# valida-xyz/valida

Measured on AMD Instinct MI355X. Metric: proofs/sec, 2^20-row Fibonacci trace, higher is better.
Workload: dtype u32; 1 GPU; C2: Fibonacci 2^20 cpu rows (mem 2^22), 14 chips, one proof per GPU; field=BabyBear / Ext5, mmcs=Keccak-256, fri_blowup=2, log_blowup=1, num_queries=40, pow_bits=8, parallelism=single GPU, proofs_in_flight_per_gpu=3, comm_stuck=False

## Files before the change

valida_amd/csrc/field.hpp:

```cpp
#pragma once
#include <cstdint>

#if defined(__HIPCC__)
#include <hip/hip_runtime.h>
#define VG_HD __host__ __device__ __forceinline__
#else
#define VG_HD inline
#endif

namespace vg {

constexpr uint32_t P = 0x78000001u;
constexpr uint32_t P_INV_NEG = 0x77ffffffu;
constexpr uint32_t R_MOD_P = 268435454u;
constexpr uint32_t R2_MOD_P = 1172168163u;
constexpr uint32_t GENERATOR = 31;
constexpr uint32_t TWO_ADIC_ROOT_27 = 0x1a427a41u;

#ifndef VG_MULHI_NOP
#define VG_MULHI_NOP 0
#endif
VG_HD uint32_t mul_lo_pinv(uint32_t lo) {
#if defined(__HIP_DEVICE_COMPILE__) && VG_MULHI_NOP == 2
    uint32_t o;
    asm("v_mul_lo_u32 %0, %1, %2\n\ts_nop 0" : "=v"(o) : "v"(lo), "v"(0x88000001u));
    return o;
#else
    return lo * 0x88000001u;
#endif
}
VG_HD uint32_t mul_hi_u32(uint32_t a, uint32_t b) {
#if defined(__HIP_DEVICE_COMPILE__) && VG_MULHI_NOP
    uint32_t o;
    asm("v_mul_hi_u32 %0, %1, %2\n\ts_nop 0" : "=v"(o) : "v"(a), "v"(b));
    return o;
#elif defined(__HIP_DEVICE_COMPILE__)
    return __umulhi(a, b);
#else
    return (uint32_t)(((uint64_t)a * b) >> 32);
#endif
}

#ifndef VG_CARRY_REDUCE
#define VG_CARRY_REDUCE 1
#endif
#if defined(__HIP_DEVICE_COMPILE__) && VG_CARRY_REDUCE == 2
VG_HD uint32_t reduce_once(uint32_t s) {
    uint32_t t, r;
    asm("v_subrev_co_u32_e32 %0, vcc, %3, %2\n\tv_cndmask_b32_e32 %1, %0, %2, vcc" : "=&v"(t), "=v"(r) : "v"(s), "v"(P) : "vcc");
    return r;
}
VG_HD uint32_t sub_mod(uint32_t a, uint32_t b) {
    uint32_t d, t, r;
    asm("v_sub_co_u32_e32 %0, vcc, %3, %4\n\tv_add_u32_e32 %1, %5, %0\n\tv_cndmask_b32_e32 %2, %0, %1, vcc" : "=&v"(d), "=&v"(t), "=v"(r) : "v"(a), "v"(b), "v"(P) : "vcc");
    return r;
}
#elif defined(__HIP_DEVICE_COMPILE__) && VG_CARRY_REDUCE
VG_HD uint32_t reduce_once(uint32_t s) {
    uint32_t t, r;
    unsigned long long borrow;
    asm("v_subrev_co_u32_e64 %0, %1, %4, %3\n\tv_cndmask_b32_e64 %2, %0, %3, %1" : "=&v"(t), "=&s"(borrow), "=v"(r) : "v"(s), "v"(P));
    return r;
}
VG_HD uint32_t sub_mod(uint32_t a, uint32_t b) {
    uint32_t d, t, r;
    unsigned long long borrow;
    asm("v_sub_co_u32_e64 %0, %1, %4, %5\n\tv_add_u32_e32 %2, %6, %0\n\tv_cndmask_b32_e64 %3, %0, %2, %1" : "=&v"(d), "=&s"(borrow), "=&v"(t), "=v"(r) : "v"(a), "v"(b), "v"(P));
    return r;
}
#else
VG_HD uint32_t reduce_once(uint32_t s) { uint32_t t = s - P; return s < t ? s : t; }
VG_HD uint32_t sub_mod(uint32_t a, uint32_t b) { uint32_t d = a - b, t = d + P; return d < t ? d : t; }
#endif

#ifndef VG_MONTY_ADD
#define VG_MONTY_ADD 0
#endif
VG_HD uint32_t monty_reduce(uint64_t t) {
#if VG_MONTY_ADD == 1
    const uint32_t m = (uint32_t)t * P_INV_NEG;
    return reduce_once((uint32_t)((t + (uint64_t)m * P) >> 32));
#else
    uint32_t lo = (uint32_t)t, hi = (uint32_t)(t >> 32);
    uint32_t m = mul_lo_pinv(lo);
    uint32_t u = mul_hi_u32(m, P);
    return sub_mod(hi, u);
#endif
}

VG_HD uint32_t monty_reduce_wide(uint64_t t) {
    uint32_t lo = (uint32_t)t, hi = reduce_once((uint32_t)(t >> 32));
    uint32_t m = mul_lo_pinv(lo);
    uint32_t u = mul_hi_u32(m, P);
    return sub_mod(hi, u);
}

struct Fp {
    uint32_t v;
    VG_HD static Fp raw(uint32_t m) { Fp r; r.v = m; return r; }
    VG_HD static Fp zero() { return raw(0); }
    VG_HD static Fp one() { return raw(R_MOD_P); }
    VG_HD static Fp from_canonical(uint32_t x) { return raw(monty_reduce((uint64_t)x * R2_MOD_P)); }
    VG_HD uint32_t canonical() const { return monty_reduce((uint64_t)v); }
    VG_HD bool is_zero() const { return v == 0; }
    VG_HD bool operator==(const Fp& o) const { return v == o.v; }
    VG_HD bool operator!=(const Fp& o) const { return v != o.v; }
    VG_HD Fp operator+(const Fp& o) const { return raw(reduce_once(v + o.v)); }
    VG_HD Fp operator-(const Fp& o) const { return raw(sub_mod(v, o.v)); }
    VG_HD Fp operator-() const { return raw(v ? P - v : 0); }
#if VG_MONTY_ADD == 2 && defined(__HIP_DEVICE_COMPILE__)
    VG_HD Fp operator*(const Fp& o) const {
        uint32_t lo, hi;
        asm("v_mul_lo_u32 %0, %2, %3\n\tv_mul_hi_u32 %1, %2, %3" : "=&v"(lo), "=v"(hi) : "v"(v), "v"(o.v));
        return raw(sub_mod(hi, mul_hi_u32(lo * 0x88000001u, P)));
    }
#else
    VG_HD Fp operator*(const Fp& o) const { return raw(monty_reduce((uint64_t)v * o.v)); }
#endif
    VG_HD Fp& operator+=(const Fp& o) { *this = *this + o; return *this; }
    VG_HD Fp& operator-=(const Fp& o) { *this = *this - o; return *this; }
    VG_HD Fp& operator*=(const Fp& o) { *this = *this * o; return *this; }
    VG_HD Fp square() const { return *this * *this; }
    VG_HD Fp pow(uint64_t e) const {
        Fp r = one(), b = *this;
        while (e) { if (e & 1) r *= b; b *= b; e >>= 1; }
        return r;
    }
    VG_HD Fp exp_power_of_2(unsigned k) const { Fp r = *this; for (unsigned i = 0; i < k; i++) r *= r; return r; }
    VG_HD Fp inv() const {
        const Fp x = *this;
        const Fp x3 = x.square() * x, x7 = x3.square() * x;
        const Fp a6 = x7.exp_power_of_2(3) * x7;
        const Fp a12 = a6.exp_power_of_2(6) * a6;
        const Fp a24 = a12.exp_power_of_2(12) * a12;
        const Fp t = a24.exp_power_of_2(3) * x7;
        const Fp w = t * x, w2 = w.square(), w4 = w2.square(), w8 = w4.square();
        return t * (w8 * w4 * w2);
    }
    VG_HD Fp halve() const { return raw((v & 1) ? (uint32_t)(((uint64_t)v + P) >> 1) : v >> 1); }
};

VG_HD Fp two_adic_generator(unsigned bits) {
    return Fp::from_canonical(TWO_ADIC_ROOT_27).exp_power_of_2(27 - bits);
}

struct Ext5 {
    Fp c[5];
    VG_HD static Ext5 zero() { Ext5 r; for (int i = 0; i < 5; i++) r.c[i] = Fp::zero(); return r; }
    VG_HD static Ext5 one() { Ext5 r = zero(); r.c[0] = Fp::one(); return r; }
    VG_HD static Ext5 from_base(Fp b) { Ext5 r = zero(); r.c[0] = b; return r; }
    VG_HD bool is_zero() const { return (c[0].v | c[1].v | c[2].v | c[3].v | c[4].v) == 0; }
    VG_HD bool operator==(const Ext5& o) const { for (int i = 0; i < 5; i++) if (c[i].v != o.c[i].v) return false; return true; }
    VG_HD bool operator!=(const Ext5& o) const { return !(*this == o); }
    VG_HD Ext5 operator+(const Ext5& o) const { Ext5 r; for (int i = 0; i < 5; i++) r.c[i] = c[i] + o.c[i]; return r; }
    VG_HD Ext5 operator-(const Ext5& o) const { Ext5 r; for (int i = 0; i < 5; i++) r.c[i] = c[i] - o.c[i]; return r; }
    VG_HD Ext5 operator-() const { Ext5 r; for (int i = 0; i < 5; i++) r.c[i] = -c[i]; return r; }
    VG_HD Ext5 operator*(const Fp& s) const { Ext5 r; for (int i = 0; i < 5; i++) r.c[i] = c[i] * s; return r; }
    VG_HD Ext5 operator+(const Fp& s) const { Ext5 r = *this; r.c[0] += s; return r; }
    VG_HD Ext5 operator-(const Fp& s) const { Ext5 r = *this; r.c[0] -= s; return r; }
    VG_HD Ext5 operator*(const Ext5& o) const {
        Fp d[5];
#pragma unroll
        for (int j = 0; j < 5; j++) d[j] = o.c[j] + o.c[j];
        Ext5 r;
#pragma unroll
        for (int k = 0; k < 5; k++) {
            uint32_t bb[5];
#pragma unroll
            for (int i = 0; i < 5; i++) bb[i] = i <= k ? o.c[k - i].v : d[k + 5 - i].v;
            uint64_t t0123 = (uint64_t)c[0].v * bb[0] + (uint64_t)c[1].v * bb[1] + (uint64_t)c[2].v * bb[2] + (uint64_t)c[3].v * bb[3];
            uint64_t t4 = (uint64_t)c[4].v * bb[4];
            r.c[k] = Fp::raw(monty_reduce_wide(t0123)) + Fp::raw(monty_reduce(t4));
        }
        return r;
    }
    VG_HD Ext5& operator+=(const Ext5& o) { *this = *this + o; return *this; }
    VG_HD Ext5& operator-=(const Ext5& o) { *this = *this - o; return *this; }
    VG_HD Ext5& operator*=(const Ext5& o) { *this = *this * o; return *this; }
    VG_HD Ext5 square() const { return *this * *this; }
    VG_HD Ext5 pow(uint64_t e) const {
        Ext5 r = one(), b = *this;
        while (e) { if (e & 1) r *= b; b *= b; e >>= 1; }
        return r;
    }
    VG_HD Ext5 exp_power_of_2(unsigned k) const { Ext5 r = *this; for (unsigned i = 0; i < k; i++) r *= r; return r; }
    template <int K> VG_HD Ext5 frobenius_k() const {
        constexpr uint32_t Z[5] = {0, 1079828539u, 847078768u, 1597816133u, 233372948u};
        Ext5 r;
        r.c[0] = c[0];
        r.c[1] = c[1] * Fp::raw(Z[(1 * K) % 5]);
        r.c[2] = c[2] * Fp::raw(Z[(2 * K) % 5]);
        r.c[3] = c[3] * Fp::raw(Z[(3 * K) % 5]);
        r.c[4] = c[4] * Fp::raw(Z[(4 * K) % 5]);
        return r;
    }
    VG_HD Ext5 frobenius() const { return frobenius_k<1>(); }
    VG_HD Ext5 inv() const {
        Ext5 f1 = frobenius_k<1>(), f2 = frobenius_k<2>(), f3 = frobenius_k<3>(), f4 = frobenius_k<4>();
        Ext5 prod = (f1 * f2) * (f3 * f4);
        Fp hi = c[1] * prod.c[4] + c[2] * prod.c[3] + c[3] * prod.c[2] + c[4] * prod.c[1];
        Fp norm = c[0] * prod.c[0] + hi + hi;
        return prod * norm.inv();
    }
};

VG_HD uint32_t reverse_bits_len(uint32_t x, unsigned bits) {
#if defined(__HIP_DEVICE_COMPILE__)
    return bits ? (__brev(x) >> (32 - bits)) : 0;
#else
    uint32_t r = 0;
    for (unsigned i = 0; i < bits; i++) r |= ((x >> i) & 1u) << (bits - 1 - i);
    return r;
#endif
}

inline unsigned log2_strict_u64(uint64_t n) { unsigned k = 0; while ((1ull << k) < n) k++; return k; }

}
```

valida_amd/csrc/host/prover.cpp:

```cpp
#include "prover.hpp"
#include "poseidon_opt.hpp"

namespace vhost {

using Clock = std::chrono::steady_clock;
static double ms_since(Clock::time_point t0) { return std::chrono::duration<double, std::milli>(Clock::now() - t0).count(); }

static Ext5 ext_from_canonical(const uint32_t* w) { Ext5 e; for (int k = 0; k < 5; k++) e.c[k] = Fp::from_canonical(w[k]); return e; }
static void ext_to_canonical(const Ext5& e, uint32_t* w) { for (int k = 0; k < 5; k++) w[k] = e.c[k].canonical(); }

Prover::Prover(int device, const MachineDesc& machine, const uint32_t* poseidon_rc480, const FriParams& fri)
    : ctx_(new DeviceCtx(device)), machine_(machine), fri_(fri), perm16_(poseidon_rc480) {
    for (auto& a : machine_.airs) {
        if (a.log_quotient_degree < 1 || a.log_quotient_degree > 3) throw std::invalid_argument("chip " + a.name + ": log_quotient_degree must be 1..3");
        if (a.native_chip != -2 && (a.native_chip < 0 || a.native_chip >= 14)) throw std::invalid_argument("chip " + a.name + ": native_chip must be a BasicMachine chip id (0..13) or -2 (captured AIR)");
        if (a.log_quotient_degree != 1 && a.native_chip >= 0) throw std::invalid_argument("chip " + a.name + ": the compiled chip kernels assume log_quotient_degree = 1");
        if (fri_.log_blowup < a.log_quotient_degree)
            throw std::invalid_argument("chip " + a.name + ": log_blowup must be >= log_quotient_degree (the quotient domain must lie inside the committed LDE)");
        std::vector<uint32_t> pw(a.program.instrs.size() * 2 + 2, 0);
        if (!a.program.instrs.empty()) memcpy(pw.data(), a.program.instrs.data(), a.program.instrs.size() * 8);
        prog_dev_.emplace_back(ctx_.get(), pw);
        iw_dev_.emplace_back(ctx_.get(), a.interaction_words);
    }
    bool sparse = false;
// ... 467 lines not shown
    ch.observe_digest(perm_pd->tree.root);
    read_cumulative_sums();
    perm_nat.clear();
    main_own.clear();
    tm.commit_perm = ms_since(t0);

    t0 = Clock::now();
    const Ext5 alpha = ch.sample_ext();
    std::vector<DMat> quot(NC);
    std::vector<char> quot_is_natural(NC, 0);
    std::vector<Fp> quot_shifts(NC);
    {
        std::vector<uint32_t> pool;
        std::vector<size_t> off(NC);
        std::vector<uint32_t> Ks(NC);
        uint32_t maxK = 0;
        for (size_t i = 0; i < NC; i++) maxK = std::max<uint32_t>(maxK, machine_.airs[i].program.num_asserts + (uint32_t)machine_.airs[i].interactions.size() + 3);
        std::vector<Ext5> apow_all(maxK);
        { Ext5 p = Ext5::one(); for (auto& e : apow_all) { e = p; p *= alpha; } }
        for (size_t i = 0; i < NC; i++) {
            auto& air = machine_.airs[i];
            uint32_t M = (uint32_t)air.interactions.size(), K = air.program.num_asserts + M + 3;
            Ks[i] = K;
            off[i] = pool.size();
            for (uint32_t k = 0; k < K; k++) put_ext(pool, apow_all[K - 1 - k]);
            for (auto& e : bus_alphas[i]) put_ext(pool, e);
            for (auto& e : betas[i]) put_ext(pool, e);
            put_ext(pool, cumulative_sums[i]);
        }
        DBuf pool_dev(&c, pool);
        Section quotient_section(&c);
        for (size_t i = 0; i < NC; i++) {
            auto& air = machine_.airs[i];
            vk::QuotientArgs a{};
            fill_quotient_args(a, (int)i, main_pd->ldes[i].view(), perm_pd->ldes[i].view(),
                               prep_slot[i] >= 0 ? prep_pd->ldes[prep_slot[i]].view() : vk::DMatView{nullptr, 0, 0, 0}, log_deg[i], pool_dev.data + off[i]);
            a.K = Ks[i];
            quot[i] = DMat(&c, 1ull << log_deg[i], 5ull << air.log_quotient_degree);
            a.out = quot[i].view();
            a.out_natural = air.log_quotient_degree == 1 ? 1 : 0;
            quot_is_natural[i] = a.out_natural != 0;
            vk::launch_quotient(c.stream_for(i, 1ull << log_deg[i]), a, c.tables);
            quot_shifts[i] = s.exp_power_of_2(air.log_quotient_degree);
        }
        quotient_section.join();
        c.check_launch("quotient");
    }
    tm.quotient = ms_since(t0);
    if (dbg && dbg->keep_matrices) {
        dbg->quotient_chunks.resize(NC);
        for (size_t i = 0; i < NC; i++) {
            auto& q = quot[i];
            DMat nat(&c, q.height, q.width);
            if (q.height > 1 && !quot_is_natural[i]) vk::launch_bitrev_rows(c.stream, q.view(), nat.view());
            else VG_HIP_CHECK(hipMemcpyAsync(nat.data, q.data, q.height * q.width * 4, hipMemcpyDeviceToDevice, c.stream));
            DBuf tmp(&c, (size_t)(q.height * q.width));
            vk::launch_export_rows(c.stream, nat.view(), 0, q.height, tmp.data);
            dbg->quotient_chunks[i].resize(q.height * q.width);
            c.download(dbg->quotient_chunks[i].data(), tmp.data, dbg->quotient_chunks[i].size() * 4);
        }
    }
    t0 = Clock::now();
    std::unique_ptr<ProverData> quot_pd;
    {
        std::vector<CommitInput> in;
        for (size_t i = 0; i < quot.size(); i++) in.push_back({&quot[i], !quot_is_natural[i], !quot_is_natural[i]});
        quot_pd = commit_batches(&c, in, &quot_shifts, fri_);
    }
    ch.observe_digest(quot_pd->tree.root);
    quot.clear();
    tm.commit_quotient = ms_since(t0);

    const Ext5 zeta = ch.sample_ext();
    std::vector<OpenRound> rounds(3);
    rounds[0].pd = main_pd.get(); rounds[1].pd = perm_pd.get(); rounds[2].pd = quot_pd.get();
    for (size_t i = 0; i < NC; i++) {
        Fp g = vg::two_adic_generator(log_deg[i]);
        rounds[0].points.push_back({zeta, zeta * g});
        rounds[1].points.push_back({zeta, zeta * g});
        rounds[2].points.push_back({zeta.exp_power_of_2(machine_.airs[i].log_quotient_degree)});
    }
    PcsOpening opening = open_multi_batches(rounds, ch);
    tm.open_values = opening.ms_values; tm.open_reduce = opening.ms_reduce; tm.fri = opening.ms_fri;
    t0 = Clock::now();
    const auto& opened = opening.opened;

    std::vector<uint32_t> pw;
    {
        size_t chip_words = 26;
        for (size_t i = 0; i < NC; i++) chip_words += 11 + 5 * (2 * machine_.airs[i].width + 10 * (machine_.airs[i].interactions.size() + 1) + 10);
        pw.reserve(chip_words + opening.proof_words.size());
    }
    pw.push_back(PROOF_MAGIC);
    pw.push_back((uint32_t)NC);
    for (int k = 0; k < 8; k++) pw.push_back(main_pd->tree.root[k]);
    for (int k = 0; k < 8; k++) pw.push_back(perm_pd->tree.root[k]);
    for (int k = 0; k < 8; k++) pw.push_back(quot_pd->tree.root[k]);
    auto put_vec = [&](const std::vector<Ext5>& v) {
        pw.push_back((uint32_t)v.size());
        for (auto& e : v) { uint32_t w5[5]; ext_to_canonical(e, w5); pw.insert(pw.end(), w5, w5 + 5); }
    };
    for (size_t i = 0; i < NC; i++) {
        pw.push_back(log_deg[i]);
        put_vec(opened[0][i][0]); put_vec(opened[0][i][1]);
        put_vec(opened[1][i][0]); put_vec(opened[1][i][1]);
        put_vec(opened[2][i][0]);
        uint32_t w5[5]; ext_to_canonical(cumulative_sums[i], w5); pw.insert(pw.end(), w5, w5 + 5);
    }
    pw.insert(pw.end(), opening.proof_words.begin(), opening.proof_words.end());
    tm.queries = opening.ms_queries + ms_since(t0);
    c.profiler.collect();
    tm.total = ms_since(t_total);
    if (times) *times = tm;
    if (dbg) {
        if (prep_pd) memcpy(dbg->prep_root, prep_pd->tree.root, 32); else memset(dbg->prep_root, 0, 32);
        for (int i = 0; i < 3; i++) ext_to_canonical(rnd[i], dbg->perm_challenges + 5 * i);
        ext_to_canonical(alpha, dbg->alpha);
        ext_to_canonical(zeta, dbg->zeta);
    }
    return pw;
}

void put_min_poly(std::vector<uint32_t>& w, const Ext5& z) {
    Ext5 g[5] = {Ext5::one(), Ext5::zero(), Ext5::zero(), Ext5::zero(), Ext5::zero()};
    Ext5 conj = z;
    for (int i = 1; i <= 4; i++) {
        conj = conj.frobenius();
        for (int k = i; k >= 1; k--) g[k] = g[k - 1] - conj * g[k];
        g[0] = Ext5::zero() - conj * g[0];
    }
    Ext5 m[5];
    for (int k = 0; k < 5; k++) m[k] = (k ? g[k - 1] : Ext5::zero()) - z * g[k];
    for (int k = 0; k < 5; k++) {
        for (int l = 1; l < 5; l++) if (!m[k].c[l].is_zero()) throw std::logic_error("open: minimal polynomial coefficient outside the base field");
        w.push_back(m[k].c[0].v);
    }
    for (int k = 0; k < 4; k++) put_ext(w, g[k]);
}

PcsOpening Prover::open_multi_batches(const std::vector<OpenRound>& rounds, Challenger& ch) {
    DeviceCtx& c = *ctx_;
    c.activate();
    const Fp s = Fp::from_canonical(vg::GENERATOR);
    const unsigned lb = fri_.log_blowup;
    const size_t NR = rounds.size();
    if (!NR) throw std::invalid_argument("open: no rounds");
    for (auto& r : rounds) {
        if (!r.pd || r.pd->ldes.empty()) throw std::invalid_argument("open: empty round");
        if (r.points.size() != r.pd->ldes.size()) throw std::invalid_argument("open: one point list per committed matrix is required");
    }
    PcsOpening res;
    auto t0 = Clock::now();
    const Ext5 alpha_b = ch.sample_ext();
    struct MatEntry { const DMat* lde; std::vector<std::tuple<uint32_t, Ext5, Ext5>> pts; size_t r, i; };
    struct Group { std::vector<Ext5> zs; std::map<PointKey, uint32_t> slot; std::vector<MatEntry> mats; uint64_t num_reduced = 0; Ext5 offset = Ext5::one(); };
    std::map<unsigned, Group> groups;
    std::vector<Ext5> apow;
    auto prepare_groups = [&]() {
        size_t max_width = 0;
        for (auto& r : rounds) for (auto& l : r.pd->ldes) max_width = std::max<size_t>(max_width, l.width);
        apow.resize(max_width);
        { Ext5 p = Ext5::one(); for (auto& a : apow) { a = p; p *= alpha_b; } }
        for (size_t r = 0; r < NR; r++)
            for (size_t i = 0; i < rounds[r].pd->ldes.size(); i++) {
                const DMat& lde = rounds[r].pd->ldes[i];
                unsigned lh = vg::log2_strict_u64(lde.height);
                Group& g = groups[lh];
                MatEntry me{&lde, {}, r, i};
                for (size_t p = 0; p < rounds[r].points[i].size(); p++) {
                    const Ext5& z = rounds[r].points[i][p];
                    auto key = key_of(z);
                    auto it = g.slot.find(key);
                    uint32_t slot;
                    if (it == g.slot.end()) { slot = (uint32_t)g.zs.size(); g.slot[key] = slot; g.zs.push_back(z); } else slot = it->second;
                    me.pts.emplace_back(slot, g.offset, Ext5::zero());
                    g.num_reduced += lde.width;
                    if (lde.width) g.offset *= apow[lde.width - 1] * alpha_b;
                }
                g.mats.push_back(std::move(me));
            }
    };

    res.opened.resize(NR);
    struct Job { size_t r, i; int p0, np; uint64_t c0, cw; size_t w[2]; size_t scale_off, out_off; };
    std::vector<Job> jobs;
    size_t out_words = 0;
    struct RLaunch { unsigned lh; size_t off; bool accumulate; uint64_t total_width; int n_points; bool vec_ok; };
    std::vector<RLaunch> launches;
    DBuf reduce_pool_dev;
    size_t apw_at = 0, ydesc_at = 0, yoff_at = 0, n_y_slots = 0;
    DBuf out_dev;
    uint32_t* out_host = nullptr;
    {
        std::map<std::pair<unsigned, PointKey>, size_t> wkey;
        std::map<unsigned, Fp> den_inv;
        std::map<PointKey, std::vector<Ext5>> zpow2;
        struct WEntry { unsigned log_n; Ext5 z; size_t pool_off; DBuf buf; };
        std::vector<WEntry> wlist;
        std::vector<uint32_t> pool;
        for (size_t r = 0; r < NR; r++) {
            res.opened[r].resize(rounds[r].pd->ldes.size());
            for (size_t i = 0; i < rounds[r].pd->ldes.size(); i++) {
                const DMat& lde = rounds[r].pd->ldes[i];
                const unsigned ln = vg::log2_strict_u64(lde.height) - lb;
                const uint64_t n = 1ull << ln;
                const auto& pts = rounds[r].points[i];
                res.opened[r][i].assign(pts.size(), std::vector<Ext5>(lde.width));
                for (size_t p0 = 0; p0 < pts.size(); p0 += 2) {
                    const int np = (int)std::min<size_t>(2, pts.size() - p0);
                    size_t widx[2] = {0, 0};
                    const size_t scale_off = pool.size();
                    for (int p = 0; p < np; p++) {
                        const Ext5& z = pts[p0 + p];
                        auto dit = den_inv.find(ln);
                        if (dit == den_inv.end()) dit = den_inv.emplace(ln, (Fp::from_canonical((uint32_t)(n % vg::P)) * s.pow(n - 1)).inv()).first;
                        std::vector<Ext5>& zp = zpow2[key_of(z)];
                        if (zp.empty()) zp.push_back(z);
                        while (zp.size() <= ln) zp.push_back(zp.back().square());
                        Ext5 zer = zp[ln] - s.exp_power_of_2(ln);
                        put_ext(pool, zer * dit->second);
                    }
                    for (int p = 0; p < np; p++) {
                        const Ext5& z = pts[p0 + p];
                        auto key = std::make_pair(ln, key_of(z));
                        auto it = wkey.find(key);
                        if (it == wkey.end()) { wkey[key] = wlist.size(); widx[p] = wlist.size(); wlist.push_back(WEntry{ln, z, 0, DBuf()}); }
                        else widx[p] = it->second;
                    }
                    const uint64_t max_cols = vk::col_dot_max_columns(np);
                    for (uint64_t c0 = 0; c0 < lde.width; c0 += max_cols) {
                        const uint64_t cw = std::min<uint64_t>(max_cols, lde.width - c0);
                        jobs.push_back(Job{r, i, (int)p0, np, c0, cw, {widx[0], widx[np - 1]}, scale_off, out_words});
                        out_words += cw * np * 5;
                    }
                }
            }
        }
        for (auto& w : wlist) { w.pool_off = pool.size(); put_min_poly(pool, w.z); }
        pool.push_back(0);
        DBuf pool_dev(&c, pool);
        {
            std::vector<uint32_t> jobs;
            uint32_t blocks = 0;
            double rows = 0;
            for (auto& w : wlist) {
                const uint64_t n = 1ull << w.log_n;
                w.buf = DBuf(&c, (size_t)vk::bary_buffer_words(n));
                jobs.push_back(blocks); jobs.push_back(0);
                put_u64(jobs, n);
                put_ptr(jobs, pool_dev.data + w.pool_off);
                put_ptr(jobs, w.buf.data);
                put_ptr(jobs, vk::bary_weights_has_image(n) ? w.buf.data + 5 * n : nullptr);
                blocks += vk::bary_weights_blocks(n);
                rows += (double)n;
            }
            if (!wlist.empty()) {
                DBuf jobs_dev(&c, jobs);
                vk::launch_bary_weights_batch(c.stream, jobs_dev.data, (uint32_t)wlist.size(), blocks, rows, s, c.tables);
            }
        }
        prepare_groups();
        {
            struct YSlot { size_t pool_off, r, i, p; };
            std::vector<YSlot> y_slots;
            std::vector<uint32_t> pool;
            for (auto& kv : groups) {
                Group& g = kv.second;
                for (uint32_t s0 = 0; s0 < g.zs.size() || s0 == 0; s0 += vk::MAX_OPEN_POINTS_PER_LAUNCH) {
                    const uint32_t s1 = std::min<uint32_t>((uint32_t)g.zs.size(), s0 + vk::MAX_OPEN_POINTS_PER_LAUNCH);
                    std::vector<const MatEntry*> live;
                    size_t max_w = 0;
                    uint64_t total_width = 0;
                    bool vec_ok = true;
                    for (auto& me : g.mats) {
                        bool any = false;
                        for (auto& t : me.pts) any |= std::get<0>(t) >= s0 && std::get<0>(t) < s1;
                        if (any) { live.push_back(&me); max_w = std::max<size_t>(max_w, me.lde->width); total_width += me.lde->width; vec_ok &= vk::reduce_vec_ok(me.lde->data, me.lde->height); }
                    }
                    launches.push_back({kv.first, pool.size(), s0 != 0, total_width, (int)(s1 - s0), vec_ok});
                    pool.push_back((uint32_t)live.size());
                    pool.push_back(s1 - s0);
                    pool.push_back((uint32_t)max_w);
                    for (uint32_t q = s0; q < s1; q++) put_min_poly(pool, g.zs[q]);
                    for (size_t col = 0; col < max_w; col++) put_ext(pool, apow[col]);
                    for (auto* me : live) {
                        put_ptr(pool, me->lde->data);
                        put_u64(pool, me->lde->height);
                        pool.push_back((uint32_t)me->lde->width);
                        uint32_t cnt = 0;
                        for (auto& t : me->pts) cnt += std::get<0>(t) >= s0 && std::get<0>(t) < s1;
                        pool.push_back(cnt);
                        for (size_t pi = 0; pi < me->pts.size(); pi++) {
                            auto& t = me->pts[pi];
                            if (std::get<0>(t) >= s0 && std::get<0>(t) < s1) {
                                pool.push_back(std::get<0>(t) - s0);
                                put_ext(pool, std::get<1>(t));
                                y_slots.push_back({pool.size(), me->r, me->i, pi});
                                put_ext(pool, Ext5::zero());
                            }
                        }
                    }
                    if (g.zs.size() <= s1) break;
                }
            }
            apw_at = pool.size();
            for (auto& a : apow) put_ext(pool, a);
            std::vector<uint32_t> ydesc, yoff;
            for (auto& ys : y_slots) {
                yoff.push_back((uint32_t)ydesc.size());
                ydesc.push_back((uint32_t)ys.pool_off);
                const size_t n_seg_at = ydesc.size();
                ydesc.push_back(0);
                for (auto& j : jobs)
                    if (j.r == ys.r && j.i == ys.i && (size_t)j.p0 <= ys.p && ys.p < (size_t)(j.p0 + j.np)) {
                        ydesc.push_back((uint32_t)j.out_off); ydesc.push_back((uint32_t)j.np); ydesc.push_back((uint32_t)(ys.p - (size_t)j.p0));
                        ydesc.push_back((uint32_t)j.c0); ydesc.push_back((uint32_t)j.cw);
                        ydesc[n_seg_at]++;
                    }
            }
            ydesc_at = pool.size();
            pool.insert(pool.end(), ydesc.begin(), ydesc.end());
            yoff_at = pool.size();
            pool.insert(pool.end(), yoff.begin(), yoff.end());
            pool.push_back(0);
            n_y_slots = y_slots.size();
            reduce_pool_dev = DBuf(&c, pool);
        }
        out_dev = DBuf(&c, out_words + 4);
        std::vector<DBuf> partials;
        std::vector<uint32_t> fin_jobs;
        uint32_t fin_blocks = 0;
        for (auto& j : jobs) {
            const DMat& lde = rounds[j.r].pd->ldes[j.i];
            const uint64_t n = lde.height >> lb;
            partials.emplace_back(&c, (size_t)(vk::col_dot_slots(n) * j.cw * j.np * 5));
            fin_blocks = vk::col_dot_finish_job(fin_jobs, fin_blocks, n, j.cw, j.np, partials.back().data, pool_dev.data + j.scale_off, out_dev.data + j.out_off);
        }
        DBuf fin_dev;
        if (!fin_jobs.empty()) fin_dev = DBuf(&c, fin_jobs);
        Section open_section(&c);
        size_t job_idx = 0;
        for (auto& j : jobs) {
            const DMat& lde = rounds[j.r].pd->ldes[j.i];
            const uint64_t n = lde.height >> lb;
            vk::DMatView sub{lde.data + j.c0 * lde.height, lde.height, j.cw, lde.height};
            vk::launch_col_dot(c.stream_for(job_idx, n), sub, n, j.np, wlist[j.w[0]].buf.data, wlist[j.w[1]].buf.data, partials[job_idx].data,
                               pool_dev.data + j.scale_off, out_dev.data + j.out_off, false);
            job_idx++;
        }
        open_section.join();
        if (!fin_jobs.empty()) vk::launch_col_dot_finish_batch(c.stream, fin_dev.data, (uint32_t)jobs.size(), fin_blocks);
        c.check_launch("opened values");
        {
            std::lock_guard<std::recursive_mutex> lk(c.host_mu);
            if (open_pinned_words_ < out_words + 4) {
                if (open_pinned_) { VG_HIP_CHECK(hipStreamSynchronize(c.stream)); VG_HIP_CHECK(hipHostFree(open_pinned_)); open_pinned_ = nullptr; open_pinned_words_ = 0; }
                VG_HIP_CHECK(hipHostMalloc((void**)&open_pinned_, (out_words + 4) * 4));
                open_pinned_words_ = out_words + 4;
            }
            out_host = open_pinned_;
        }
    }
    res.ms_values = ms_since(t0);

    t0 = Clock::now();
    std::map<unsigned, DBuf> ro;
    unsigned log_max = 0;
    {
        DBuf& pool_dev = reduce_pool_dev;
        vk::launch_open_y(c.stream, out_dev.data, pool_dev.data + apw_at, pool_dev.data + ydesc_at, pool_dev.data + yoff_at, (uint32_t)n_y_slots, pool_dev.data);
        for (auto& kv : groups) { ro[kv.first] = DBuf(&c, (size_t)(5ull << kv.first)); log_max = std::max(log_max, kv.first); }
        Section reduce_section(&c);
        std::map<unsigned, hipStream_t> stream_of;
        size_t grp_idx = 0;
        for (auto& l : launches) {
            const uint64_t L = 1ull << l.lh;
            if (!stream_of.count(l.lh)) stream_of[l.lh] = c.stream_for(grp_idx++, L);
            vk::launch_reduce_openings(stream_of[l.lh], pool_dev.data + l.off, L, s, c.tables, ro[l.lh].data, l.total_width, l.accumulate, l.n_points, l.vec_ok);
        }
        reduce_section.join();
        c.check_launch("reduce openings");
        if (out_words) VG_HIP_CHECK(hipMemcpyAsync(out_host, out_dev.data, out_words * 4, hipMemcpyDeviceToHost, c.stream));
    }
    res.ms_reduce = ms_since(t0);
    if (log_max < lb + 0u) throw std::invalid_argument("open: nothing to open");

    t0 = Clock::now();
    std::vector<DBuf> layer_bufs;
    std::vector<DeviceTree> layer_trees;
    std::vector<std::array<uint32_t, 8>> commit_phase_commits;
    DBuf cur = std::move(ro[log_max]);
    ro.erase(log_max);
    const unsigned n_layers = log_max - lb;
    std::vector<uint32_t> chw(vk::DEV_CHALLENGER_WORDS, 0);
    for (int i = 0; i < 16; i++) chw[i] = ch.state[i].v;
    for (size_t i = 0; i < ch.in.size(); i++) chw[16 + i] = ch.in[i].v;
    chw[32] = (uint32_t)ch.in.size();
    for (size_t i = 0; i < ch.out.size(); i++) chw[33 + i] = ch.out[i].v;
    chw[49] = (uint32_t)ch.out.size();
    DBuf ch_dev(&c, chw), betas_dev(&c, (size_t)(5 * n_layers + 8)), commits_dev(&c, (size_t)(8 * n_layers + 8));
    unsigned li = 0;
    for (unsigned lf = log_max; lf-- > lb; li++) {
        uint64_t L = 2ull << lf, half = L >> 1;
        layer_trees.emplace_back();
        layer_trees.back().drop_bottom = true;
        const DeviceTree::TopChallenger step{pow_pos_.data, ch_dev.data, betas_dev.data + 5 * li, commits_dev.data + 8 * li};
        layer_trees.back().build(&c, {vk::DMatView{cur.data, half, 10, half}}, false, nullptr, &step);
        DBuf next(&c, (size_t)(5 * half));
        auto it = ro.find(lf);
        vk::launch_fri_fold(c.stream, cur.data, L, betas_dev.data + 5 * li, it != ro.end() ? it->second.data : nullptr, c.tables, next.data);
        if (it != ro.end()) ro.erase(it);
        layer_bufs.push_back(std::move(cur));
        cur = std::move(next);
    }
    c.check_launch("fri fold");
    const size_t NQ = fri_.num_queries, NL = layer_trees.size();
    if (NQ > 256) throw std::invalid_argument("open: at most 256 queries");
    std::vector<uint32_t> templ, bottom_jobs;
    std::vector<std::pair<uint32_t, uint32_t>> fix;
    size_t fix_roots_at = 0, fix_final_at = 0;
    uint32_t tail_pos = 0;
    {
        size_t n_desc = 0, n_fix = 8 * NL + 16;
        for (size_t l = 0; l < NL; l++) n_desc += 1 + layer_trees[l].log_max_height;
        for (size_t r = 0; r < NR; r++) n_desc += rounds[r].pd->ldes.size() + rounds[r].pd->tree.log_max_height;
        n_desc *= NQ;
        n_fix += NQ * (2 + 2 * NL + NR * 2);
        for (size_t r = 0; r < NR; r++) n_fix += NQ * rounds[r].pd->ldes.size();
        templ.reserve(8 * n_desc + 8);
        fix.reserve(n_fix);
        uint32_t& pos = tail_pos;
        auto host_word = [&](uint32_t v) { fix.emplace_back(pos++, v); };
        auto gather = [&](const uint32_t* base, uint64_t stride, uint32_t count, uint32_t kind, size_t q, uint32_t mode, uint32_t shift, uint32_t aux) {
            const uint64_t pv = (uint64_t)base;
            const uint32_t d8[8] = {(uint32_t)pv, (uint32_t)(pv >> 32), (uint32_t)stride, (uint32_t)(stride >> 32), count | (kind << 28), pos, (uint32_t)q | (mode << 8) | (shift << 16), aux};
            templ.insert(templ.end(), d8, d8 + 8);
            pos += count;
        };
        auto gather_path = [&](const DeviceTree& t, size_t q, uint32_t shift0) {
            host_word(t.log_max_height);
            for (unsigned l = 0; l < t.log_max_height; l++) {
                if (l < t.dropped) {
                    const uint64_t pv = (uint64_t)t.leaf_ptr;
                    const uint32_t j8[8] = {(uint32_t)pv, (uint32_t)(pv >> 32), (uint32_t)t.leaf_stride, (uint32_t)(t.leaf_stride >> 32), (uint32_t)t.leaf_elems, pos, (uint32_t)q | (l << 8) | (shift0 << 16), 0};
                    bottom_jobs.insert(bottom_jobs.end(), j8, j8 + 8);
                    pos += 8;
                } else gather(t.layers[l].data, 1, 8, 1, q, 1, shift0 + l, 0);
            }
        };
        host_word((uint32_t)NL);
        fix_roots_at = fix.size();
        for (size_t l = 0; l < NL; l++) for (int w = 0; w < 8; w++) host_word(0);
        host_word((uint32_t)NQ);
        for (size_t q = 0; q < NQ; q++) {
            host_word((uint32_t)NL);
            for (size_t l = 0; l < NL; l++) {
                const uint64_t half = 1ull << (log_max - 1 - l);
                gather(layer_bufs[l].data, half, 5, 0, q, 2, (uint32_t)l, (uint32_t)(5 * half));
                gather_path(layer_trees[l], q, (uint32_t)l + 1);
            }
        }
        fix_final_at = fix.size();
        for (int k = 0; k < 6; k++) host_word(0);
        host_word((uint32_t)NQ);
        for (size_t q = 0; q < NQ; q++) {
            host_word((uint32_t)NR);
            for (size_t r = 0; r < NR; r++) {
                const DeviceTree& t = rounds[r].pd->tree;
                const uint32_t shift_r = log_max - t.log_max_height;
                host_word((uint32_t)rounds[r].pd->ldes.size());
                for (auto& lde : rounds[r].pd->ldes) {
// ... 77 lines not shown
```

valida_amd/csrc/host/sharded_prover.cpp:

```cpp
#include "sharded_prover.hpp"
#include <algorithm>
#include <array>
#include <tuple>

namespace vhost {

namespace {

Ext5 sp_ext_from_canonical(const uint32_t* w) { Ext5 e; for (int k = 0; k < 5; k++) e.c[k] = Fp::from_canonical(w[k]); return e; }
void sp_ext_to_canonical(const Ext5& e, uint32_t* w) { for (int k = 0; k < 5; k++) w[k] = e.c[k].canonical(); }

struct SpPointKey {
    uint32_t w[5];
    bool operator<(const SpPointKey& o) const { return memcmp(w, o.w, 20) < 0; }
};
SpPointKey sp_key_of(const Ext5& e) { SpPointKey k; for (int i = 0; i < 5; i++) k.w[i] = e.c[i].v; return k; }

int owner_of(uint64_t global_col, int W) { return (int)(global_col % (uint64_t)W); }

struct ShTree {
    bool sharded = false;
    DeviceTree tree;
    std::vector<std::vector<uint32_t>> top;
    unsigned log_total = 0, log_local = 0;
// ... 667 lines not shown
        std::vector<uint32_t> out;
        Ext5 alpha_b;
        std::map<unsigned, DBuf> ro;
        std::vector<FriLayer> layers;
        std::vector<std::array<uint32_t, 8>> commits;
        DBuf cur;
        bool cur_sharded = false;
        uint32_t fpw[5];
        uint32_t pow_witness = 0;
        std::vector<uint32_t> tail;
    };
    std::vector<Opening> op((size_t)NH);
    std::vector<std::vector<std::vector<std::vector<Ext5>>>> points((size_t)NH);
    for (int k = 0; k < NH; k++) {
        Rank& R = rk[k];
        const Ext5 zeta = R.ch->sample_ext();
        points[k].resize(NR);
        for (size_t i = 0; i < NC; i++) {
            const Fp g = vg::two_adic_generator(log_deg[i]);
            points[k][0].push_back({zeta, zeta * g});
            points[k][1].push_back({zeta, zeta * g});
            points[k][2].push_back({zeta.exp_power_of_2(1)});
        }
    }
    auto round_of = [&](Rank& R, size_t r) -> ShRound& { return r == 0 ? R.main_rs : r == 1 ? R.perm_rs : R.quot_rs; };

    struct Job { size_t r, i; int p0, np; uint64_t c0, cw; size_t w[2]; size_t scale_off, out_off; bool big; };
    std::vector<Job> jobs0;
    size_t out_words = 0;
    for (int k = 0; k < NH; k++) {
        Rank& R = rk[k];
        DeviceCtx& c = *R.c;
        c.activate();
        Opening& O = op[k];
        O.opened.resize(NR);
        struct WEntry { bool big; unsigned logL; uint64_t rows; Fp shift; Ext5 z; size_t pool_off; DBuf buf; };
        std::map<std::tuple<int, unsigned, SpPointKey>, size_t> wkey;
        std::vector<WEntry> wlist;
        std::vector<uint32_t> pool;
        std::vector<Job> jobs;
        size_t ow = 0;
        for (size_t r = 0; r < NR; r++) {
            ShRound& rs = round_of(R, r);
            O.opened[r].resize(rs.mats.size());
            for (size_t i = 0; i < rs.mats.size(); i++) {
                const ShMat& m = rs.mats[i];
                const unsigned logL = vg::log2_strict_u64(m.L), ln = logL - lb;
                const uint64_t n = 1ull << ln;
                const auto& pts = points[k][r][i];
                O.opened[r][i].assign(pts.size(), std::vector<Ext5>(m.width));
                const Fp rho = m.big ? rho_of(R, logL) : Fp::one();
                for (size_t p0 = 0; p0 < pts.size(); p0 += 2) {
                    const int np = (int)std::min<size_t>(2, pts.size() - p0);
                    size_t widx[2] = {0, 0};
                    const size_t scale_off = pool.size();
                    for (int p = 0; p < np; p++) {
                        const Ext5& z = pts[p0 + p];
                        if (m.big) {
                            Ext5 zer = z.exp_power_of_2(logL) - s.exp_power_of_2(logL);
                            Fp den = Fp::from_canonical((uint32_t)(m.L % vg::P)) * s.pow(m.L - 1);
                            put_ext(pool, zer * (den.inv() * rho));
                        } else {
                            Ext5 zer = z.exp_power_of_2(ln) - s.exp_power_of_2(ln);
                            Fp den = Fp::from_canonical((uint32_t)(n % vg::P)) * s.pow(n - 1);
                            put_ext(pool, zer * den.inv());
                        }
                    }
                    for (int p = 0; p < np; p++) {
                        const Ext5& z = pts[p0 + p];
                        auto key = std::make_tuple(m.big ? 1 : 0, m.big ? logL : ln, sp_key_of(z));
                        auto it = wkey.find(key);
                        if (it == wkey.end()) {
                            wkey[key] = wlist.size(); widx[p] = wlist.size();
                            wlist.push_back(WEntry{m.big, logL, m.big ? m.L / W : n, m.big ? s * rho : s, z, 0, DBuf()});
                        } else widx[p] = it->second;
                    }
                    const uint64_t max_cols = vk::col_dot_max_columns(np);
                    for (uint64_t c0 = 0; c0 < m.width; c0 += max_cols) {
                        const uint64_t cw = std::min<uint64_t>(max_cols, m.width - c0);
                        jobs.push_back(Job{r, i, (int)p0, np, c0, cw, {widx[0], widx[np - 1]}, scale_off, ow, m.big});
                        ow += cw * np * 5;
                    }
                }
            }
        }
        for (auto& w : wlist) { w.pool_off = pool.size(); put_min_poly(pool, w.z); }
        pool.push_back(0);
        DBuf pool_dev(&c, pool);
        {
            std::vector<uint32_t> bj;
            uint32_t blocks = 0;
            double rows = 0;
            auto put64 = [&](uint64_t v) { bj.push_back((uint32_t)v); bj.push_back((uint32_t)(v >> 32)); };
            for (auto& w : wlist) {
                w.buf = DBuf(&c, (size_t)vk::bary_buffer_words(w.rows));
                bj.push_back(blocks); bj.push_back(w.shift.v);
                put64(w.rows);
                put64((uint64_t)(pool_dev.data + w.pool_off));
                put64((uint64_t)w.buf.data);
                put64((uint64_t)(vk::bary_weights_has_image(w.rows) ? w.buf.data + 5 * w.rows : nullptr));
                blocks += vk::bary_weights_blocks(w.rows);
                rows += (double)w.rows;
            }
            if (!wlist.empty()) {
                DBuf jobs_dev(&c, bj);
                vk::launch_bary_weights_batch(c.stream, jobs_dev.data, (uint32_t)wlist.size(), blocks, rows, s, c.tables);
            }
        }
        DBuf out_dev(&c, ow + 4);
        std::vector<DBuf> partials;
        for (auto& j : jobs) {
            const ShMat& m = round_of(R, j.r).mats[j.i];
            const DMat& lde = m.big ? m.shard : m.lde;
            const uint64_t rows = m.big ? lde.height : (lde.height >> lb);
            partials.emplace_back(&c, (size_t)(vk::col_dot_slots(rows) * j.cw * j.np * 5));
            vk::DMatView sub{lde.data + j.c0 * lde.height, lde.height, j.cw, lde.height};
            vk::launch_col_dot(c.stream, sub, rows, j.np, wlist[j.w[0]].buf.data, wlist[j.w[1]].buf.data, partials.back().data, pool_dev.data + j.scale_off, out_dev.data + j.out_off);
        }
        c.check_launch("opened values");
        O.out.assign(ow, 0);
        if (ow) c.download_small(O.out.data(), out_dev.data, ow * 4); else c.sync();
        if (k == 0) { jobs0 = jobs; out_words = ow; }
        else if (ow != out_words) throw std::logic_error("sharded open: ranks disagree on the layout of the opened values");
    }
    {
        std::vector<const uint32_t*> contrib;
        for (auto& O : op) contrib.push_back(O.out.data());
        std::vector<uint32_t> all;
        f.all_gather(contrib, out_words, all);
        for (int k = 0; k < NH; k++) {
            Opening& O = op[k];
            for (auto& j : jobs0)
                for (uint64_t col = 0; col < j.cw; col++)
                    for (int p = 0; p < j.np; p++) {
                        const size_t at = j.out_off + (col * j.np + p) * 5;
                        Ext5 v;
                        if (j.big) {
                            v = Ext5::zero();
                            for (int r = 0; r < W; r++) v += sp_ext_from_canonical(&all[(size_t)r * out_words + at]);
                        } else v = sp_ext_from_canonical(&O.out[at]);
                        O.opened[j.r][j.i][j.p0 + p][j.c0 + col] = v;
                    }
        }
    }

    unsigned log_max = 0;
    for (int k = 0; k < NH; k++) {
        Rank& R = rk[k];
        DeviceCtx& c = *R.c;
        c.activate();
        Opening& O = op[k];
        O.alpha_b = R.ch->sample_ext();
        const Ext5& alpha_b = O.alpha_b;
        struct MatEntry { const uint32_t* data; uint64_t stride; uint64_t width; std::vector<std::tuple<uint32_t, Ext5, Ext5>> pts; };
        struct Group { std::vector<Ext5> zs; std::map<SpPointKey, uint32_t> slot; std::vector<MatEntry> mats; uint64_t num_reduced = 0; Ext5 offset = Ext5::one(); };
        std::map<unsigned, Group> groups;
        size_t max_width = 0;
        for (size_t r = 0; r < NR; r++) for (auto& m : round_of(R, r).mats) max_width = std::max<size_t>(max_width, m.width);
        std::vector<Ext5> apow(max_width);
        { Ext5 pw = Ext5::one(); for (auto& a : apow) { a = pw; pw *= alpha_b; } }
        for (size_t r = 0; r < NR; r++) {
            ShRound& rs = round_of(R, r);
            for (size_t i = 0; i < rs.mats.size(); i++) {
                const ShMat& m = rs.mats[i];
                const unsigned lh = vg::log2_strict_u64(m.L);
                Group& g = groups[lh];
                MatEntry me{m.big ? m.shard.data : m.lde.data, m.big ? m.shard.height : m.lde.height, m.width, {}};
                for (size_t p = 0; p < points[k][r][i].size(); p++) {
                    const Ext5& z = points[k][r][i][p];
                    auto key = sp_key_of(z);
                    auto it = g.slot.find(key);
                    uint32_t slot;
                    if (it == g.slot.end()) { slot = (uint32_t)g.zs.size(); g.slot[key] = slot; g.zs.push_back(z); } else slot = it->second;
                    Ext5 Y = Ext5::zero();
                    auto& ys = O.opened[r][i][p];
                    for (size_t col = 0; col < ys.size(); col++) Y += apow[col] * ys[col];
                    me.pts.emplace_back(slot, g.offset, Y);
                    g.num_reduced += m.width;
                    if (m.width) g.offset *= apow[m.width - 1] * alpha_b;
                }
                g.mats.push_back(std::move(me));
            }
        }
        struct Launch { unsigned lh; size_t off; bool accumulate; uint64_t total_width; int n_points; bool vec_ok; };
        std::vector<Launch> launches;
        std::vector<uint32_t> pool;
        for (auto& kv : groups) {
            Group& g = kv.second;
            for (uint32_t s0 = 0; s0 < g.zs.size() || s0 == 0; s0 += vk::MAX_OPEN_POINTS_PER_LAUNCH) {
                const uint32_t s1 = std::min<uint32_t>((uint32_t)g.zs.size(), s0 + vk::MAX_OPEN_POINTS_PER_LAUNCH);
                std::vector<const MatEntry*> live;
                size_t max_w = 0;
                uint64_t total_width = 0;
                bool vec_ok = true;
                for (auto& me : g.mats) {
                    bool any = false;
                    for (auto& t : me.pts) any |= std::get<0>(t) >= s0 && std::get<0>(t) < s1;
                    if (any) { live.push_back(&me); max_w = std::max<size_t>(max_w, me.width); total_width += me.width; vec_ok &= vk::reduce_vec_ok(me.data, me.stride); }
                }
                launches.push_back({kv.first, pool.size(), s0 != 0, total_width, (int)(s1 - s0), vec_ok});
                pool.push_back((uint32_t)live.size());
                pool.push_back(s1 - s0);
                pool.push_back((uint32_t)max_w);
                for (uint32_t q = s0; q < s1; q++) put_min_poly(pool, g.zs[q]);
                for (size_t col = 0; col < max_w; col++) put_ext(pool, apow[col]);
                for (auto* me : live) {
                    put_ptr(pool, me->data);
                    put_u64(pool, me->stride);
                    pool.push_back((uint32_t)me->width);
                    uint32_t cnt = 0;
                    for (auto& t : me->pts) cnt += std::get<0>(t) >= s0 && std::get<0>(t) < s1;
                    pool.push_back(cnt);
                    for (auto& t : me->pts)
                        if (std::get<0>(t) >= s0 && std::get<0>(t) < s1) { pool.push_back(std::get<0>(t) - s0); put_ext(pool, std::get<1>(t)); put_ext(pool, std::get<2>(t)); }
                }
                if (g.zs.size() <= s1) break;
            }
        }
        DBuf pool_dev(&c, pool);
        for (auto& kv : groups) {
            const uint64_t L = 1ull << kv.first, rows = L >= min_big ? L / W : L;
            O.ro[kv.first] = DBuf(&c, (size_t)(5 * rows));
            log_max = std::max(log_max, kv.first);
        }
        for (auto& l : launches) {
            const uint64_t L = 1ull << l.lh;
            const bool big = L >= min_big;
            vk::launch_reduce_openings(c.stream, pool_dev.data + l.off, big ? L / W : L, big ? s * rho_of(R, l.lh) : s, c.tables, O.ro[l.lh].data, l.total_width, l.accumulate, l.n_points, l.vec_ok);
        }
        c.check_launch("reduce openings");
    }
    if (log_max < lb) throw std::invalid_argument("sharded open: nothing to open");

    const bool multi = W > 1;
    for (auto& O : op) {
        O.cur = std::move(O.ro[log_max]);
        O.ro.erase(log_max);
        O.cur_sharded = multi && (1ull << log_max) >= min_big;
    }
    struct DevFri { bool on = false; unsigned count = 0; size_t first_layer = 0; DBuf ch_dev, betas_dev, commits_dev; };
    std::vector<DevFri> dev((size_t)NH);
    for (unsigned lf = log_max; lf-- > lb;) {
        const uint64_t len = 2ull << lf, half = len >> 1;
        const bool sharded = multi && len >= min_big, next_sharded = multi && half >= min_big;
        if (!sharded) {
            for (int k = 0; k < NH; k++) {
                Rank& R = rk[k];
                DeviceCtx& c = *R.c;
                c.activate();
                Opening& O = op[k];
                DevFri& D = dev[(size_t)k];
                if (O.cur_sharded) throw std::logic_error("sharded fri: layer state out of step");
                if (!D.on) {
                    const unsigned remaining = lf - lb + 1;
                    std::vector<uint32_t> chw(vk::DEV_CHALLENGER_WORDS, 0);
                    const Challenger& ch = *R.ch;
                    for (int i = 0; i < 16; i++) chw[i] = ch.state[i].v;
                    for (size_t i = 0; i < ch.in.size(); i++) chw[16 + i] = ch.in[i].v;
                    chw[32] = (uint32_t)ch.in.size();
                    for (size_t i = 0; i < ch.out.size(); i++) chw[33 + i] = ch.out[i].v;
                    chw[49] = (uint32_t)ch.out.size();
                    D.ch_dev = DBuf(&c, chw);
                    D.betas_dev = DBuf(&c, (size_t)(5 * remaining + 8));
                    D.commits_dev = DBuf(&c, (size_t)(8 * remaining + 8));
                    D.first_layer = O.layers.size();
                    D.on = true;
                }
                O.layers.emplace_back();
                FriLayer& ly = O.layers.back();
                ly.sharded = false; ly.len = len;
                ly.t.sharded = false;
                ly.t.log_total = ly.t.log_local = vg::log2_strict_u64(half);
                const DeviceTree::TopChallenger step{R.p->pow_pos_.data, D.ch_dev.data, D.betas_dev.data + 5 * D.count, D.commits_dev.data + 8 * D.count};
                ly.t.tree.build(&c, {vk::DMatView{O.cur.data, half, 10, half}}, false, nullptr, &step);
                DBuf next(&c, (size_t)(5 * half));
                auto it = O.ro.find(lf);
                vk::launch_fri_fold(c.stream, O.cur.data, len, D.betas_dev.data + 5 * D.count, it != O.ro.end() ? it->second.data : nullptr, c.tables, next.data);
                c.check_launch("fri fold");
                D.count++;
                ly.buf = std::move(O.cur);
                O.cur = std::move(next);
                O.cur_sharded = false;
            }
            continue;
        }
        for (int k = 0; k < NH; k++) {
            Rank& R = rk[k];
            DeviceCtx& c = *R.c;
            c.activate();
            Opening& O = op[k];
            if (O.cur_sharded != sharded) throw std::logic_error("sharded fri: layer state out of step");
            O.layers.emplace_back();
            FriLayer& ly = O.layers.back();
            ly.sharded = sharded; ly.len = len;
            const uint64_t prow = sharded ? half / W : half;
            ly.t.sharded = sharded;
            ly.t.log_total = vg::log2_strict_u64(half);
            ly.t.log_local = vg::log2_strict_u64(prow);
            ly.t.tree.build(&c, {vk::DMatView{O.cur.data, prow, 10, prow}}, true);
            if (!sharded) memcpy(ly.t.root, ly.t.tree.root, 32);
        }
        if (sharded) {
            std::vector<ShTree*> trees;
            for (auto& O : op) trees.push_back(&O.layers.back().t);
            std::vector<uint32_t> roots;
            gather_subtree_roots(trees, roots);
            for (int k = 0; k < NH; k++) finish_top(rk[k], op[k].layers.back().t, roots, nullptr);
        }
        std::vector<std::vector<uint32_t>> next_host((size_t)NH);
        for (int k = 0; k < NH; k++) {
            Rank& R = rk[k];
            DeviceCtx& c = *R.c;
            c.activate();
            Opening& O = op[k];
            FriLayer& ly = O.layers.back();
            R.ch->observe_digest(ly.t.root);
            std::array<uint32_t, 8> root;
            memcpy(root.data(), ly.t.root, 32);
            O.commits.push_back(root);
            Ext5 beta = R.ch->sample_ext();
            if (sharded) beta = beta * rho_of(R, lf + 1).inv();
            std::vector<uint32_t> bw;
            put_ext(bw, beta);
            bw.resize(8, 0);
            DBuf beta_dev(&c, bw);
            const uint64_t my_len = sharded ? len / W : len;
            DBuf next(&c, (size_t)(5 * (my_len / 2)));
            auto it = O.ro.find(lf);
            const uint32_t* add = (it != O.ro.end() && sharded == next_sharded) ? it->second.data : nullptr;
            vk::launch_fri_fold(c.stream, O.cur.data, my_len, beta_dev.data, add, c.tables, next.data);
            c.check_launch("fri fold");
            if (sharded && !next_sharded) {
                next_host[k].resize((size_t)(5 * (my_len / 2)));
                c.download(next_host[k].data(), next.data, next_host[k].size() * 4);
            } else c.sync();
            ly.buf = std::move(O.cur);
            O.cur = std::move(next);
            O.cur_sharded = next_sharded;
        }
        if (sharded && !next_sharded) {
            const uint64_t my_half = half / W, qloc = my_half / 2, q = half / 2;
            std::vector<const uint32_t*> contrib;
            for (auto& v : next_host) contrib.push_back(v.data());
            std::vector<uint32_t> all;
            f.all_gather(contrib, (size_t)(10 * qloc), all);
            for (int k = 0; k < NH; k++) {
                Rank& R = rk[k];
                DeviceCtx& c = *R.c;
                c.activate();
                Opening& O = op[k];
                std::vector<uint32_t> full((size_t)(10 * q));
                for (int r = 0; r < W; r++)
                    for (uint64_t col = 0; col < 10; col++)
                        memcpy(&full[(size_t)(col * q + (uint64_t)r * qloc)], &all[(size_t)r * 10 * qloc + (size_t)(col * qloc)], (size_t)qloc * 4);
                auto it = O.ro.find(lf);
                if (it != O.ro.end()) {
                    std::vector<uint32_t> add((size_t)(10 * q));
                    c.download(add.data(), it->second.data, add.size() * 4);
                    for (size_t x = 0; x < full.size(); x++) full[x] = (Fp::raw(full[x]) + Fp::raw(add[x])).v;
                }
                O.cur = DBuf(&c, full);
            }
        }
    }
    for (int k = 0; k < NH; k++) {
        DevFri& D = dev[(size_t)k];
        if (!D.on) continue;
// ... 179 lines not shown
```

valida_amd/csrc/kernels/launch.hpp:

```cpp
#pragma once
#include <vector>
#include "device_common.hpp"
#include "profiler.hpp"
#include "../air/symbolic.hpp"
#include "verify_args.hpp"

namespace vk {

struct QuotientArgs {
    DMatView main_lde, perm_lde, prep_lde;
    int log_n;
    const vair::Instr* prog;
    uint32_t n_instrs, n_regs, n_air_asserts;
    const uint32_t* iw;
    const uint32_t* consts;
    uint32_t K;
    uint32_t coset_shift, coset_shift_inv;
    int lqd;
    uint32_t zh_inv[8];
    uint32_t zh[8];
    uint32_t g_inv;
    DMatView out;
    int out_natural;
    static constexpr int INTERPRET = -2;
    int native_chip;
    const uint32_t* main_nx;
    const uint32_t* perm_nx;
    const uint32_t* prep_nx;
    uint32_t next_step_p1;
    QuotientArgs normalised() const {
        QuotientArgs b = *this;
        if (!b.main_nx) b.main_nx = b.main_lde.data;
        if (!b.perm_nx) b.perm_nx = b.perm_lde.data;
        if (!b.prep_nx) b.prep_nx = b.prep_lde.data;
        if (!b.next_step_p1) b.next_step_p1 = 1u + (1u << (b.lqd > 0 ? b.lqd : 1));
        return b;
    }
};


void launch_ingest(hipStream_t st, const uint32_t* src_dev, DMatView dst, bool bitrev);
void launch_bitrev_rows(hipStream_t st, DMatView src, DMatView dst);
void launch_clock_probe(hipStream_t st, uint64_t* out3, uint32_t iters);
void launch_interleave_blocks(hipStream_t st, const uint32_t* src, uint32_t* dst, uint64_t rows, uint32_t log_wq, uint64_t n_cols);
void launch_export_rows(hipStream_t st, DMatView src, uint64_t row0, uint64_t nrows, uint32_t* dst_dev);
void launch_intt(hipStream_t st, DMatView m, const DeviceTables& tb);
void launch_coset_ntt(hipStream_t st, DMatView coeffs, DMatView dst, uint64_t dst_row0, Fp shift, const DeviceTables& tb);
void launch_lde_natural(hipStream_t st, DMatView nat, DMatView lde, int log_blowup, const DeviceTables& tb, const LdeTables& lt, DMatView s1, DMatView s2);
void launch_verify_chunk(hipStream_t st, const VerifyChunkArgs& a);
void launch_keccak_leaves(hipStream_t st, const uint32_t* const* cols_dev, int n_elems, uint64_t n_rows, uint32_t* digests);
void launch_keccak_leaves_strided(hipStream_t st, const uint32_t* base, uint64_t stride, int n_elems, uint64_t n_rows, uint32_t* digests);
void launch_keccak_compress(hipStream_t st, const uint32_t* prev, const uint32_t* const* cols_dev, int n_elems, uint64_t n_out, uint32_t* next);
void launch_keccak_bottom_q(hipStream_t st, const uint32_t* jobs_dev, uint32_t n_jobs, const uint32_t* indices_dev, uint32_t* dst);
void launch_poseidon_bottom_q(hipStream_t st, const uint32_t* pos_dev, bool sparse, const uint32_t* jobs_dev, uint32_t n_jobs, const uint32_t* indices_dev, uint32_t* dst);
constexpr int KECCAK_TOP_MAX_LEVELS = 11;
struct KeccakTopArgs {
    const uint32_t* prev;
    uint64_t first_len;
    int levels;
    uint32_t* out[KECCAK_TOP_MAX_LEVELS];
    const uint32_t* const* cols[KECCAK_TOP_MAX_LEVELS];
    int n_elems[KECCAK_TOP_MAX_LEVELS];
    const uint32_t* leaf_base = nullptr;
    uint64_t leaf_stride = 0;
    int leaf_elems = 0;
    uint64_t leaf_rows = 0;
    uint64_t block_len = 0;
    const uint32_t* ch_pos = nullptr;
    uint32_t* ch_state = nullptr;
    uint32_t* ch_beta5 = nullptr;
    uint32_t* ch_commit8 = nullptr;
};
void launch_keccak_top(hipStream_t st, const KeccakTopArgs& a);
constexpr uint64_t KECCAK_LEVELS_BLOCK_LEN = 64;
void launch_keccak_levels(hipStream_t st, const KeccakTopArgs& a);
bool keccak_levels_fused(uint64_t len);
bool keccak_levels_take_leaves(uint64_t n_rows);
bool keccak_top_takes_leaves(uint64_t n_rows);
void launch_poseidon_leaves(hipStream_t st, const uint32_t* pos_dev, bool sparse, const uint32_t* const* cols_dev, int n_elems, uint64_t n_rows, uint32_t* digests);
void launch_poseidon_leaves_strided(hipStream_t st, const uint32_t* pos_dev, bool sparse, const uint32_t* base, uint64_t stride, int n_elems, uint64_t n_rows, uint32_t* digests);
void launch_poseidon_compress(hipStream_t st, const uint32_t* pos_dev, bool sparse, const uint32_t* prev, const uint32_t* const* cols_dev, int n_elems, uint64_t n_out, uint32_t* next);
bool poseidon_levels_take(uint64_t parents);
int poseidon_levels_group(uint64_t parents);
void launch_poseidon_levels(hipStream_t st, const uint32_t* pos_dev, bool sparse, const KeccakTopArgs& a);
void launch_poseidon_top(hipStream_t st, const uint32_t* pos_dev, bool sparse, const KeccakTopArgs& a);
uint64_t perm_scratch_words(uint64_t n);
void launch_add_ext_const(hipStream_t st, uint32_t* data, uint64_t stride, uint64_t n, const uint32_t* off5_dev);
void launch_perm_trace(hipStream_t st, DMatView main, DMatView prep, const uint32_t* iw_dev, const uint32_t* chal_dev, uint32_t M, DMatView perm,
                       uint32_t* scratch, int native_chip = -2);
void launch_quotient(hipStream_t st, const QuotientArgs& a, const DeviceTables& tb);
void launch_check_constraints(hipStream_t st, const QuotientArgs& a, unsigned long long* first_bad_dev);
struct TgCpuOp { uint32_t pc, fp, opcode; int32_t operands[5]; uint32_t kind, has_imm, imm, mem_first; };
struct TgMemOp { uint32_t clk, addr, value, is_write; };
struct TgAluOp { uint32_t opcode, a, b, c; };
struct TgOutOp { uint32_t clk, byte; };
enum { TG_CPU_STORE32 = 0, TG_CPU_LOAD32, TG_CPU_JAL, TG_CPU_JALV, TG_CPU_BEQ, TG_CPU_BNE, TG_CPU_IMM32, TG_CPU_BUS, TG_CPU_BUS_LEFT_IMM, TG_CPU_STOP,
       TG_CPU_LOADFP, TG_CPU_LOAD_U8, TG_CPU_LOAD_S8, TG_CPU_STORE_U8, TG_CPU_READ_ADVICE };
void launch_tracegen_cpu(hipStream_t st, const TgCpuOp* ops, uint64_t n, const TgMemOp* mem, uint64_t n_mem, DMatView t);
size_t tracegen_mem_sort_scratch_bytes(uint64_t n);
hipError_t launch_tracegen_mem(hipStream_t st, const TgMemOp* mem, uint64_t n, const uint32_t* static_cells, uint64_t n_static, uint32_t* keys2, uint32_t* idx2,
                               void* sort_tmp, size_t sort_tmp_bytes, DMatView t);
void launch_tracegen_alu(hipStream_t st, int chip, const TgAluOp* ops, uint64_t n, DMatView t);
void launch_tracegen_idle(hipStream_t st, int mode, const uint32_t* static_cells, uint64_t n_static, DMatView t);
hipError_t launch_tracegen_range(hipStream_t st, const TgCpuOp* ops, uint64_t n, const TgMemOp* mem, uint64_t n_mem, uint32_t* counts, DMatView t);
void launch_tracegen_alu2(hipStream_t st, int chip, const TgAluOp* ops, uint64_t n, DMatView t);
void launch_tracegen_output(hipStream_t st, const TgOutOp* vals, const uint32_t* row0, uint64_t n, uint64_t n_rows, DMatView t);
hipError_t launch_tracegen_program(hipStream_t st, const TgCpuOp* ops, uint64_t n, uint64_t padded_n, uint32_t rom_len, uint32_t* counts, DMatView t);
void launch_bary_weights(hipStream_t st, uint64_t n, const uint32_t* min_poly_dev, Fp shift, const DeviceTables& tb, uint32_t* w);
void launch_bary_weights_batch(hipStream_t st, const uint32_t* jobs_dev, uint32_t n_jobs, uint32_t total_blocks, double total_rows, Fp shift, const DeviceTables& tb);
uint32_t bary_weights_blocks(uint64_t n);
bool bary_weights_has_image(uint64_t n);
uint64_t col_dot_slots(uint64_t n);
uint64_t bary_buffer_words(uint64_t n);
uint64_t col_dot_max_columns(int np);
void launch_col_dot(hipStream_t st, DMatView m, uint64_t n, int np, const uint32_t* w0, const uint32_t* w1, uint32_t* partial,
                    const uint32_t* scale5_dev, uint32_t* out_dev, bool finish = true);
uint32_t col_dot_finish_job(std::vector<uint32_t>& jobs, uint32_t first_block, uint64_t n, uint64_t width, int np, const uint32_t* partial, const uint32_t* scale5_dev, uint32_t* out_dev);
void launch_col_dot_finish_batch(hipStream_t st, const uint32_t* jobs_dev, uint32_t n_jobs, uint32_t total_blocks);
constexpr int MAX_OPEN_POINTS_PER_LAUNCH = 4;
void launch_open_y(hipStream_t st, const uint32_t* vals_dev, const uint32_t* apow_dev, const uint32_t* desc_dev, const uint32_t* entry_off_dev, uint32_t n_entries, uint32_t* pool_dev);
inline bool reduce_vec_ok(const void* col0, uint64_t stride_words) { return ((uintptr_t)col0 & 15) == 0 && (stride_words & 3) == 0; }
void launch_reduce_openings(hipStream_t st, const uint32_t* desc_dev, uint64_t L, Fp shift, const DeviceTables& tb, uint32_t* out, uint64_t total_width,
                            bool accumulate, int n_points, bool vec_ok);
void launch_fri_fold(hipStream_t st, const uint32_t* in, uint64_t L, const uint32_t* beta5_dev, const uint32_t* add, const DeviceTables& tb, uint32_t* out);
constexpr int DEV_CHALLENGER_WORDS = 50;
void launch_fri_challenge(hipStream_t st, const uint32_t* pos_dev, uint32_t* ch_dev, const uint32_t* digest8_dev, uint32_t* beta5_dev, uint32_t* commit8_dev);
void launch_pow_grind(hipStream_t st, const uint32_t* pos_dev, bool sparse, uint32_t k_pending, uint32_t first, uint32_t count, uint32_t bits, uint32_t* best_dev);
void launch_gather(hipStream_t st, const uint32_t* desc_dev, uint64_t n_desc, uint32_t* dst);
void launch_gather_q(hipStream_t st, const uint32_t* templ_dev, uint64_t n_desc, const uint32_t* indices_dev, uint32_t* dst);

}
```

valida_amd/csrc/kernels/merkle.hip:

```cpp
#include "launch.hpp"
#include "keccak.hpp"
#include "keccak_pair.hpp"
#include "challenger_dev.hpp"
#include <cstdlib>
#include <stdexcept>

namespace vk {

__device__ __forceinline__ uint32_t wrap_mod_p(uint32_t w) {
    if (w >= vg::P) w -= vg::P;
    if (w >= vg::P) w -= vg::P;
    return w;
}

__device__ __forceinline__ void squeeze_digest(const KState& a, uint32_t (&out)[8]) {
#pragma unroll
    for (int i = 0; i < 4; i++) { out[2 * i] = wrap_mod_p(a.lo[i]); out[2 * i + 1] = wrap_mod_p(a.hi[i]); }
}

struct PtrCols {
    const uint32_t* const* p;
    __device__ __forceinline__ const uint32_t* operator[](int k) const { return p[k]; }
};
struct StridedCols {
    const uint32_t* base;
    uint64_t stride;
    __device__ __forceinline__ const uint32_t* operator[](int k) const { return base + (uint64_t)k * stride; }
};
template <class Cols>
__device__ __forceinline__ void hash_row(const Cols cols, int n_elems, uint64_t r, uint32_t (&out)[8]) {
    KState a;
    kstate_zero(a);
    int base = 0;
    for (; base + 34 <= n_elems; base += 34) {
#pragma unroll
        for (int k = 0; k < 34; k++) absorb_word(a, k, Fp::raw(cols[base + k][r]).canonical());
        keccak_f1600<false>(a);
    }
    const int rem = n_elems - base;
#pragma unroll
    for (int k = 0; k < 34; k++) {
        if (k < rem) absorb_word(a, k, Fp::raw(cols[base + k][r]).canonical());
        if (k == rem) absorb_word(a, k, 0x01u);
    }
    absorb_word(a, 33, 0x80000000u);
    keccak_f1600<true>(a);
    squeeze_digest(a, out);
}

__device__ __forceinline__ void compress2(const uint32_t (&l)[8], const uint32_t (&r)[8], uint32_t (&out)[8]) {
    KState a;
    kstate_zero(a);
#pragma unroll
    for (int i = 0; i < 4; i++) { a.lo[i] = l[2 * i]; a.hi[i] = l[2 * i + 1]; a.lo[4 + i] = r[2 * i]; a.hi[4 + i] = r[2 * i + 1]; }
    a.lo[8] = 0x01u;
    a.hi[16] = 0x80000000u;
    keccak_f1600<true>(a);
    squeeze_digest(a, out);
}

__device__ __forceinline__ void load_digest(const uint32_t* p, uint32_t (&d)[8]) {
    const uint4* q = reinterpret_cast<const uint4*>(p);
    uint4 lo = q[0], hi = q[1];
    d[0] = lo.x; d[1] = lo.y; d[2] = lo.z; d[3] = lo.w; d[4] = hi.x; d[5] = hi.y; d[6] = hi.z; d[7] = hi.w;
}
__device__ __forceinline__ void store_digest(uint32_t* p, const uint32_t (&d)[8]) {
    uint4* q = reinterpret_cast<uint4*>(p);
    q[0] = make_uint4(d[0], d[1], d[2], d[3]);
    q[1] = make_uint4(d[4], d[5], d[6], d[7]);
}

template <class Cols>
__global__ void __launch_bounds__(256) k_keccak_leaves(const Cols cols, int n_elems, uint64_t n_rows, uint32_t* __restrict__ digests) {
    uint64_t r = (uint64_t)blockIdx.x * blockDim.x + threadIdx.x;
    if (r >= n_rows) return;
    uint32_t d[8];
    hash_row(cols, n_elems, r, d);
    store_digest(digests + 8 * r, d);
}

__global__ void __launch_bounds__(256) k_keccak_compress(const uint32_t* __restrict__ prev, const uint32_t* const* __restrict__ cols, int n_elems, uint64_t n_out,
                                  uint32_t* __restrict__ next) {
    uint64_t i = (uint64_t)blockIdx.x * blockDim.x + threadIdx.x;
    if (i >= n_out) return;
    uint32_t l[8], r[8], d[8];
    load_digest(prev + 16 * i, l);
    load_digest(prev + 16 * i + 8, r);
    compress2(l, r, d);
    if (n_elems > 0) {
        uint32_t h[8], d2[8];
        hash_row(PtrCols{cols}, n_elems, i, h);
        compress2(d, h, d2);
        store_digest(next + 8 * i, d2);
    } else {
        store_digest(next + 8 * i, d);
    }
}

template <class Cols>
__device__ __forceinline__ void hash_row_pair(const Cols cols, int n_elems, uint64_t r, int h, uint32_t (&out)[4]) {
    KHalf a;
#pragma unroll
    for (int i = 0; i < 25; i++) a.s[i] = 0;
    int base = 0;
    for (; base + 34 <= n_elems; base += 34) {
#pragma unroll
        for (int l = 0; l < 17; l++) a.s[l] ^= Fp::raw(cols[base + 2 * l + h][r]).canonical();
        keccak_f1600_pair<false>(a, h);
    }
    const int rem = n_elems - base;
#pragma unroll
    for (int l = 0; l < 17; l++) {
        const int k = 2 * l + h;
        if (k < rem) a.s[l] ^= Fp::raw(cols[base + k][r]).canonical();
        if (k == rem) a.s[l] ^= 0x01u;
    }
    if (h) a.s[16] ^= 0x80000000u;
    keccak_f1600_pair<true>(a, h);
#pragma unroll
    for (int i = 0; i < 4; i++) out[i] = wrap_mod_p(a.s[i]);
}
__device__ __forceinline__ void compress2_pair(const uint32_t (&l)[4], const uint32_t (&r)[4], int h, uint32_t (&out)[4]) {
    KHalf a;
#pragma unroll
    for (int i = 0; i < 25; i++) a.s[i] = 0;
#pragma unroll
    for (int i = 0; i < 4; i++) { a.s[i] = l[i]; a.s[4 + i] = r[i]; }
    if (!h) a.s[8] = 0x01u;
    else a.s[16] = 0x80000000u;
    keccak_f1600_pair<true>(a, h);
#pragma unroll
    for (int i = 0; i < 4; i++) out[i] = wrap_mod_p(a.s[i]);
}
__device__ __forceinline__ void load_digest_half(const uint32_t* p, int h, uint32_t (&d)[4]) {
#pragma unroll
    for (int i = 0; i < 4; i++) d[i] = p[2 * i + h];
}
__device__ __forceinline__ void store_digest_half(uint32_t* p, int h, const uint32_t (&d)[4]) {
#pragma unroll
    for (int i = 0; i < 4; i++) p[2 * i + h] = d[i];
}
__device__ __forceinline__ void node_pair(const uint32_t* prev, const uint32_t* const* cols, int n_elems, uint64_t i, int h, uint32_t* out) {
    uint32_t l[4], r[4], d[4];
    load_digest_half(prev + 16 * i, h, l);
    load_digest_half(prev + 16 * i + 8, h, r);
    compress2_pair(l, r, h, d);
    if (n_elems > 0) {
        uint32_t hr[4], d2[4];
        hash_row_pair(PtrCols{cols}, n_elems, i, h, hr);
        compress2_pair(d, hr, h, d2);
        store_digest_half(out + 8 * i, h, d2);
    } else {
        store_digest_half(out + 8 * i, h, d);
    }
}
template <class Cols>
__global__ void __launch_bounds__(256) k_keccak_leaves_pair(const Cols cols, int n_elems, uint64_t n_rows, uint32_t* __restrict__ digests) {
    const uint64_t t = (uint64_t)blockIdx.x * blockDim.x + threadIdx.x, r = t >> 1;
    if (r >= n_rows) return;
    uint32_t d[4];
    hash_row_pair(cols, n_elems, r, (int)(t & 1), d);
    store_digest_half(digests + 8 * r, (int)(t & 1), d);
}
__global__ void __launch_bounds__(256) k_keccak_compress_pair(const uint32_t* __restrict__ prev, const uint32_t* const* __restrict__ cols, int n_elems, uint64_t n_out,
                                                             uint32_t* __restrict__ next) {
    const uint64_t t = (uint64_t)blockIdx.x * blockDim.x + threadIdx.x, i = t >> 1;
    if (i >= n_out) return;
    node_pair(prev, cols, n_elems, i, (int)(t & 1), next);
}
__global__ void __launch_bounds__(1024) k_keccak_top_pair(KeccakTopArgs a) {
    const uint32_t* prev = a.prev;
    if (a.leaf_rows) {
        if ((threadIdx.x >> 1) < a.leaf_rows) {
            uint32_t d[4];
            hash_row_pair(StridedCols{a.leaf_base, a.leaf_stride}, a.leaf_elems, threadIdx.x >> 1, (int)(threadIdx.x & 1), d);
            store_digest_half(const_cast<uint32_t*>(a.prev) + 8 * (threadIdx.x >> 1), (int)(threadIdx.x & 1), d);
        }
        __threadfence_block();
        __syncthreads();
    }
    for (int l = 0; l < a.levels; l++) {
        const uint64_t len = a.first_len >> l;
        if ((threadIdx.x >> 1) < len) node_pair(prev, a.cols[l], a.n_elems[l], threadIdx.x >> 1, (int)(threadIdx.x & 1), a.out[l]);
        __threadfence_block();
        __syncthreads();
        prev = a.out[l];
    }
    if (a.ch_pos && threadIdx.x < 64) fri_challenge_step((int)threadIdx.x, a.ch_pos, a.ch_state, prev, a.ch_beta5, a.ch_commit8);
}

constexpr int LEVELS_LDS_X = 512, LEVELS_LDS_Y = 256;
__device__ __forceinline__ void lds_barrier() {
#ifdef __HIPCC__
    asm volatile("s_waitcnt lgkmcnt(0)\n\ts_barrier" ::: "memory");
#else
    __syncthreads();
#endif
}
__global__ void __launch_bounds__(1024) k_keccak_levels_pair(KeccakTopArgs a) {
    __shared__ uint32_t lds[(LEVELS_LDS_X + LEVELS_LDS_Y) * 8];
    const int h = (int)(threadIdx.x & 1);
    const uint32_t t = threadIdx.x >> 1;
    const uint64_t b0 = a.block_len, first = (uint64_t)blockIdx.x * b0;
    bool in_lds = false;
    if (a.leaf_rows) {
        if (t < 2 * b0) {
            uint32_t d[4];
            const uint64_t row = 2 * first + t;
            hash_row_pair(StridedCols{a.leaf_base, a.leaf_stride}, a.leaf_elems, row, h, d);
            store_digest_half(const_cast<uint32_t*>(a.prev) + 8 * row, h, d);
            store_digest_half(lds + 8 * t, h, d);
        }
        lds_barrier();
        in_lds = true;
    }
    for (int l = 0; l < a.levels; l++) {
        const uint32_t* in = lds + ((l & 1) ? LEVELS_LDS_X * 8 : 0);
        uint32_t* out = lds + ((l & 1) ? 0 : LEVELS_LDS_X * 8);
        if (t < (b0 >> l)) {
            const uint64_t i = (first >> l) + t;
            uint32_t lf[4], rg[4], d[4];
            if (in_lds) { load_digest_half(in + 16 * t, h, lf); load_digest_half(in + 16 * t + 8, h, rg); }
            else { load_digest_half(a.prev + 16 * i, h, lf); load_digest_half(a.prev + 16 * i + 8, h, rg); }
            compress2_pair(lf, rg, h, d);
            if (a.n_elems[l] > 0) {
                uint32_t hr[4], d2[4];
                hash_row_pair(PtrCols{a.cols[l]}, a.n_elems[l], i, h, hr);
                compress2_pair(d, hr, h, d2);
#pragma unroll
                for (int k = 0; k < 4; k++) d[k] = d2[k];
            }
            store_digest_half(a.out[l] + 8 * i, h, d);
            store_digest_half(out + 8 * t, h, d);
        }
        in_lds = true;
        if (l + 1 < a.levels) lds_barrier();
    }
    if (a.ch_pos) {
        __threadfence_block();
        __syncthreads();
        if (threadIdx.x < 64) fri_challenge_step((int)threadIdx.x, a.ch_pos, a.ch_state, a.out[a.levels - 1], a.ch_beta5, a.ch_commit8);
    }
}

__global__ void __launch_bounds__(1024) k_keccak_top(KeccakTopArgs a) {
    const uint32_t* prev = a.prev;
    for (int l = 0; l < a.levels; l++) {
        const uint64_t len = a.first_len >> l;
        if (threadIdx.x < len) {
            const uint64_t i = threadIdx.x;
            uint32_t lft[8], rgt[8], d[8];
            load_digest(prev + 16 * i, lft);
            load_digest(prev + 16 * i + 8, rgt);
            compress2(lft, rgt, d);
            if (a.n_elems[l] > 0) {
                uint32_t h[8], d2[8];
                hash_row(PtrCols{a.cols[l]}, a.n_elems[l], i, h);
                compress2(d, h, d2);
                store_digest(a.out[l] + 8 * i, d2);
            } else {
                store_digest(a.out[l] + 8 * i, d);
            }
        }
        __threadfence_block();
        __syncthreads();
        prev = a.out[l];
    }
    if (a.ch_pos && threadIdx.x < 64) fri_challenge_step((int)threadIdx.x, a.ch_pos, a.ch_state, prev, a.ch_beta5, a.ch_commit8);
}

constexpr double KECCAK_VALU_PER_PERM = 23 * 178.0 + 58.0;
constexpr uint64_t KECCAK_PAIR_MAX_NODES = 32768;
static bool keccak_pairs_enabled() {
    static const bool on = [] { const char* e = getenv("VGPU_KECCAK_PAIRS"); return !(e && e[0] == '0'); }();
    return on;
}
static double row_perms(int n_elems) { return (double)(n_elems / 34 + 1); }
static double node_perms(int n_inject) { return n_inject > 0 ? 2.0 + row_perms(n_inject) : 1.0; }

bool keccak_top_takes_leaves(uint64_t n_rows) { return keccak_pairs_enabled() && n_rows >= 2 && n_rows <= 512; }
static bool keccak_levels_enabled() {
    static const bool on = [] { const char* e = getenv("VGPU_KECCAK_LEVELS"); return !(e && e[0] == '0'); }();
    return on && keccak_pairs_enabled();
}
bool keccak_levels_fused(uint64_t len) { return keccak_levels_enabled() && len >= KECCAK_LEVELS_BLOCK_LEN && len <= KECCAK_PAIR_MAX_NODES; }
bool keccak_levels_take_leaves(uint64_t n_rows) { return n_rows >= 2 * KECCAK_LEVELS_BLOCK_LEN && keccak_levels_fused(n_rows / 2); }

void launch_keccak_levels(hipStream_t st, const KeccakTopArgs& a0) {
    KeccakTopArgs a = a0;
    if (!a.block_len) a.block_len = a.first_len;
    const uint64_t b0 = a.block_len;
    if (!keccak_levels_enabled() || !b0 || (b0 & (b0 - 1)) || b0 > (uint64_t)LEVELS_LDS_Y || a.first_len % b0 || a.levels < 1 || a.levels > KECCAK_TOP_MAX_LEVELS ||
        (b0 >> (a.levels - 1)) == 0 || (a.leaf_rows && a.leaf_rows != 2 * a.first_len) || (a.ch_pos && a.first_len != b0))
        throw std::logic_error("keccak levels: a launch this kernel does not fit");
    double bytes = 0, perms = 0;
    for (int l = 0; l < a.levels; l++) {
        bytes += (double)(a.first_len >> l) * (96.0 + 4.0 * a.n_elems[l]);
        perms += (double)(a.first_len >> l) * node_perms(a.n_elems[l]);
    }
    if (a.leaf_rows) {
        bytes += (double)a.leaf_rows * (4.0 * a.leaf_elems + 32.0);
        perms += (double)a.leaf_rows * row_perms(a.leaf_elems);
    }
    unsigned threads = (unsigned)((a.leaf_rows ? 4 : 2) * b0);
    if (threads < 64) threads = 64;
    ProfScope ps("k_keccak_levels_pair", st, bytes, perms * KECCAK_VALU_PER_PERM / 64.0);
    VK_LAUNCH(k_keccak_levels_pair, dim3((unsigned)(a.first_len / b0)), dim3(threads), 0, st, a);
}

void launch_keccak_top(hipStream_t st, const KeccakTopArgs& a) {
    double bytes = 0, perms = 0;
    for (int l = 0; l < a.levels; l++) {
        bytes += (double)(a.first_len >> l) * (96.0 + 4.0 * a.n_elems[l]);
        perms += (double)(a.first_len >> l) * node_perms(a.n_elems[l]);
    }
    const bool pairs = keccak_pairs_enabled() && a.first_len <= 512;
    if (a.leaf_rows) {
        if (!pairs || a.leaf_rows != 2 * a.first_len || !keccak_top_takes_leaves(a.leaf_rows)) throw std::logic_error("keccak top: leaf prologue on a tree it does not fit");
        bytes += (double)a.leaf_rows * (4.0 * a.leaf_elems + 32.0);
        perms += (double)a.leaf_rows * row_perms(a.leaf_elems);
    }
    if (pairs && keccak_levels_enabled() && a.first_len <= (uint64_t)LEVELS_LDS_Y) { launch_keccak_levels(st, a); return; }
    ProfScope ps(pairs ? "k_keccak_top_pair" : "k_keccak_top", st, bytes, perms * KECCAK_VALU_PER_PERM / 64.0);
    if (pairs) { VK_LAUNCH(k_keccak_top_pair, dim3(1), dim3(1024), 0, st, a); return; }
    VK_LAUNCH(k_keccak_top, dim3(1), dim3(1024), 0, st, a);
}

template <class Cols> __device__ __forceinline__ void bottom_digest_quad(const Cols cols, int n_elems, uint64_t node, uint32_t level, int pair, int h, uint32_t (&d)[4]) {
    uint32_t own[4];
    hash_row_pair(cols, n_elems, level ? 2 * node + (uint64_t)pair : node, h, own);
    if (level == 0) {
#pragma unroll
        for (int i = 0; i < 4; i++) d[i] = own[i];
        return;
    }
    uint32_t right[4];
#pragma unroll
    for (int i = 0; i < 4; i++) right[i] = (uint32_t)__builtin_amdgcn_update_dpp(0, (int)own[i], 0xEE, 0xF, 0xF, true);
    compress2_pair(own, right, h, d);
}
__global__ void __launch_bounds__(256) k_keccak_bottom_q(const uint32_t* __restrict__ jobs, uint32_t n_jobs, const uint32_t* __restrict__ indices, uint32_t* __restrict__ dst) {
    const uint32_t t = blockIdx.x * blockDim.x + threadIdx.x, j = t >> 2;
    if (j >= n_jobs) return;
    const int pair = (int)((t >> 1) & 1u), h = (int)(t & 1u);
    const uint32_t* e = jobs + 8 * j;
    const uint64_t ptr = ((uint64_t)e[1] << 32) | e[0], stride = ((uint64_t)e[3] << 32) | e[2];
    const uint32_t q = e[6] & 0xffu, level = (e[6] >> 8) & 0xffu, shift = e[6] >> 16;
    const uint64_t node = (((uint64_t)indices[q] >> shift) >> level) ^ 1u;
    uint32_t d[4];
    if (stride) bottom_digest_quad(StridedCols{reinterpret_cast<const uint32_t*>(ptr), stride}, (int)e[4], node, level, pair, h, d);
    else bottom_digest_quad(PtrCols{reinterpret_cast<const uint32_t* const*>(ptr)}, (int)e[4], node, level, pair, h, d);
    if (pair == 0) store_digest_half(dst + e[5], h, d);
}
void launch_keccak_bottom_q(hipStream_t st, const uint32_t* jobs_dev, uint32_t n_jobs, const uint32_t* indices_dev, uint32_t* dst) {
    if (!n_jobs) return;
    ProfScope ps("k_gather", st, 0.0);
    VK_LAUNCH(k_keccak_bottom_q, dim3((4 * n_jobs + 255) / 256), dim3(256), 0, st, jobs_dev, n_jobs, indices_dev, dst);
}

void launch_keccak_leaves(hipStream_t st, const uint32_t* const* cols_dev, int n_elems, uint64_t n_rows, uint32_t* digests) {
    unsigned blocks = (unsigned)((n_rows + 255) / 256);
    const bool pairs = keccak_pairs_enabled() && n_rows <= KECCAK_PAIR_MAX_NODES;
    ProfScope ps(pairs ? "k_keccak_leaves_pair" : "k_keccak_leaves", st, (double)n_rows * (4.0 * n_elems + 32.0), (double)n_rows * row_perms(n_elems) * KECCAK_VALU_PER_PERM / 64.0);
    if (pairs) {
        VK_LAUNCH(k_keccak_leaves_pair<PtrCols>, dim3((unsigned)((2 * n_rows + 255) / 256)), dim3(256), 0, st, PtrCols{cols_dev}, n_elems, n_rows, digests);
        return;
    }
    VK_LAUNCH(k_keccak_leaves<PtrCols>, dim3(blocks), dim3(256), 0, st, PtrCols{cols_dev}, n_elems, n_rows, digests);
}
void launch_keccak_leaves_strided(hipStream_t st, const uint32_t* base, uint64_t stride, int n_elems, uint64_t n_rows, uint32_t* digests) {
    unsigned blocks = (unsigned)((n_rows + 255) / 256);
    const bool pairs = keccak_pairs_enabled() && n_rows <= KECCAK_PAIR_MAX_NODES;
    ProfScope ps(pairs ? "k_keccak_leaves_pair" : "k_keccak_leaves", st, (double)n_rows * (4.0 * n_elems + 32.0), (double)n_rows * row_perms(n_elems) * KECCAK_VALU_PER_PERM / 64.0);
    if (pairs) {
        VK_LAUNCH(k_keccak_leaves_pair<StridedCols>, dim3((unsigned)((2 * n_rows + 255) / 256)), dim3(256), 0, st, StridedCols{base, stride}, n_elems, n_rows, digests);
        return;
    }
    VK_LAUNCH(k_keccak_leaves<StridedCols>, dim3(blocks), dim3(256), 0, st, StridedCols{base, stride}, n_elems, n_rows, digests);
}
void launch_keccak_compress(hipStream_t st, const uint32_t* prev, const uint32_t* const* cols_dev, int n_elems, uint64_t n_out, uint32_t* next) {
    unsigned blocks = (unsigned)((n_out + 255) / 256);
    const bool pairs = keccak_pairs_enabled() && n_out <= KECCAK_PAIR_MAX_NODES;
    ProfScope ps(pairs ? "k_keccak_compress_pair" : "k_keccak_compress", st, (double)n_out * (96.0 + 4.0 * n_elems), (double)n_out * node_perms(n_elems) * KECCAK_VALU_PER_PERM / 64.0);
    if (pairs) {
        VK_LAUNCH(k_keccak_compress_pair, dim3((unsigned)((2 * n_out + 255) / 256)), dim3(256), 0, st, prev, cols_dev, n_elems, n_out, next);
        return;
    }
    VK_LAUNCH(k_keccak_compress, dim3(blocks), dim3(256), 0, st, prev, cols_dev, n_elems, n_out, next);
}

}
```

valida_amd/csrc/kernels/ntt.hip:

```cpp
#include "launch.hpp"
#include "butterfly.hpp"

namespace vk {

template <bool PAD> __device__ __forceinline__ int tile_addr(int i, int c, int LD) { return PAD ? i + (i >> 4) : i * LD + c; }

template <int R>
__device__ __forceinline__ void load_round_twiddles(Fp (&held)[(1 << R) - 1], const uint32_t* tw, int low, int lowbits) {
#pragma unroll
    for (int st = 0; st < R; st++) {
        const uint32_t* t = tw + ((1 << (lowbits + st)) - 1) + low;
#pragma unroll
        for (int k = 0; k < (1 << st); k++) held[(1 << st) - 1 + k] = Fp::raw(t[k << lowbits]);
    }
}

template <int R, bool DIT, bool PAD, int LB>
__device__ __forceinline__ void ntt_round(uint32_t* buf, const uint32_t* tw, int logn, int s_lo, int logT, int LD) {
    constexpr int G = 1 << R;
    const int n_items = (1 << (logn - R)) << logT;
    const int maskT = (1 << logT) - 1, lowbits = LB >= 0 ? LB : s_lo - 1, lowmask = (1 << lowbits) - 1;
    const bool linear = !PAD || lowbits >= 4 || lowbits + R <= 4;
    const int gs = PAD ? (lowbits >= 4 ? (1 << lowbits) + (1 << (lowbits - 4)) : (1 << lowbits)) : (LD << lowbits);
    for (int w = threadIdx.x; w < n_items; w += blockDim.x) {
        const int c = w & maskT, q = w >> logT;
        const int low = q & lowmask, base = ((q >> lowbits) << (lowbits + R)) | low;
        uint32_t* p0 = buf + tile_addr<PAD>(base, c, LD);
        Fp x[G];
        if (linear) {
#pragma unroll
            for (int g = 0; g < G; g++) x[g] = Fp::raw(p0[g * gs]);
        } else {
#pragma unroll
            for (int g = 0; g < G; g++) x[g] = Fp::raw(buf[tile_addr<PAD>(base | (g << lowbits), c, LD)]);
        }
        butterflies<R, DIT, LB == 0>(x, tw, low, lowbits);
        if (linear) {
#pragma unroll
            for (int g = 0; g < G; g++) p0[g * gs] = x[g].v;
        } else {
#pragma unroll
            for (int g = 0; g < G; g++) buf[tile_addr<PAD>(base | (g << lowbits), c, LD)] = x[g].v;
        }
    }
    __syncthreads();
}

template <bool DIT, bool PAD>
__device__ __forceinline__ void ntt_round_dispatch(int R, uint32_t* buf, const uint32_t* tw, int logn, int s_lo, int logT, int LD) {
    if (s_lo == 1) {
        switch (R) {
            case 1: ntt_round<1, DIT, PAD, 0>(buf, tw, logn, 1, logT, LD); break;
            case 2: ntt_round<2, DIT, PAD, 0>(buf, tw, logn, 1, logT, LD); break;
            case 3: ntt_round<3, DIT, PAD, 0>(buf, tw, logn, 1, logT, LD); break;
            default: ntt_round<4, DIT, PAD, 0>(buf, tw, logn, 1, logT, LD); break;
        }
        return;
    }
    switch (R) {
        case 1: ntt_round<1, DIT, PAD, -1>(buf, tw, logn, s_lo, logT, LD); break;
        case 2: ntt_round<2, DIT, PAD, -1>(buf, tw, logn, s_lo, logT, LD); break;
        case 3: ntt_round<3, DIT, PAD, -1>(buf, tw, logn, s_lo, logT, LD); break;
        default: ntt_round<4, DIT, PAD, -1>(buf, tw, logn, s_lo, logT, LD); break;
    }
}

template <bool DIT, bool PAD>
__device__ __forceinline__ void tile_transform(uint32_t* buf, const uint32_t* tw, int logn, int logT, int LD) {
    if (logn == 0) return;
    if (PAD && logn == 12) {
        if (DIT) {
            ntt_round<4, true, PAD, 0>(buf, tw, 12, 1, 0, LD);
            ntt_round<4, true, PAD, 4>(buf, tw, 12, 5, 0, LD);
            ntt_round<4, true, PAD, 8>(buf, tw, 12, 9, 0, LD);
        } else {
            ntt_round<4, false, PAD, 8>(buf, tw, 12, 9, 0, LD);
            ntt_round<4, false, PAD, 4>(buf, tw, 12, 5, 0, LD);
            ntt_round<4, false, PAD, 0>(buf, tw, 12, 1, 0, LD);
        }
        return;
    }
    if (PAD && logn == 14) {
        if (DIT) {
            ntt_round<4, true, PAD, 0>(buf, tw, 14, 1, 0, LD);
            ntt_round<4, true, PAD, 4>(buf, tw, 14, 5, 0, LD);
            ntt_round<4, true, PAD, 8>(buf, tw, 14, 9, 0, LD);
            ntt_round<2, true, PAD, 12>(buf, tw, 14, 13, 0, LD);
        } else {
            ntt_round<2, false, PAD, 12>(buf, tw, 14, 13, 0, LD);
            ntt_round<4, false, PAD, 8>(buf, tw, 14, 9, 0, LD);
            ntt_round<4, false, PAD, 4>(buf, tw, 14, 5, 0, LD);
            ntt_round<4, false, PAD, 0>(buf, tw, 14, 1, 0, LD);
        }
        return;
    }
    const int rounds = (logn + 3) >> 2, small = logn / rounds, extra = logn - small * rounds;
    if (DIT) {
        int s_lo = 1;
        for (int i = 0; i < rounds; i++) { int R = small + (i < extra ? 1 : 0); ntt_round_dispatch<true, PAD>(R, buf, tw, logn, s_lo, logT, LD); s_lo += R; }
    } else {
        int s_top = logn;
        for (int i = 0; i < rounds; i++) { int R = small + (i < extra ? 1 : 0); ntt_round_dispatch<false, PAD>(R, buf, tw, logn, s_top - R + 1, logT, LD); s_top -= R; }
    }
}

template <int R, bool DIT, int LB, int LOGT>
__device__ __forceinline__ void ntt_round_strided(uint32_t* buf, const uint32_t* tw, int logn) {
    constexpr int G = 1 << R, T = 1 << LOGT, LD = T + 1, gs = LD << LB;
    const int n_items = (1 << (logn - R)) << LOGT;
    for (int w = threadIdx.x; w < n_items; w += blockDim.x) {
        const int c = w & (T - 1), q = w >> LOGT;
        const int low = q & ((1 << LB) - 1), base = ((q >> LB) << (LB + R)) | low;
        uint32_t* p0 = buf + base * LD + c;
        Fp x[G];
#pragma unroll
        for (int g = 0; g < G; g++) x[g] = Fp::raw(p0[g * gs]);
        butterflies<R, DIT, LB == 0>(x, tw, low, LB);
#pragma unroll
        for (int g = 0; g < G; g++) p0[g * gs] = x[g].v;
    }
    __syncthreads();
}
template <bool DIT, int K_HI, int LOGT>
__device__ __forceinline__ void strided_transform(uint32_t* buf, const uint32_t* tw) {
    static_assert(K_HI == 8 || K_HI == 10, "hot shapes only");
    if (DIT) {
        ntt_round_strided<4, true, 0, LOGT>(buf, tw, K_HI);
        ntt_round_strided<4, true, 4, LOGT>(buf, tw, K_HI);
        if (K_HI == 10) ntt_round_strided<2, true, 8, LOGT>(buf, tw, K_HI);
    } else {
        if (K_HI == 10) ntt_round_strided<2, false, 8, LOGT>(buf, tw, K_HI);
        ntt_round_strided<4, false, 4, LOGT>(buf, tw, K_HI);
        ntt_round_strided<4, false, 0, LOGT>(buf, tw, K_HI);
    }
}
#ifndef VGPU_STRIDED_FIXED
#define VGPU_STRIDED_FIXED 1
#endif
template <bool DIT>
__device__ __forceinline__ void strided_tile_transform(uint32_t* buf, const uint32_t* tw, int k_hi, int logT, int LD) {
    if (VGPU_STRIDED_FIXED && k_hi == 8 && logT == 6) strided_transform<DIT, 8, 6>(buf, tw);
    else if (VGPU_STRIDED_FIXED && k_hi == 10 && logT == 4) strided_transform<DIT, 10, 4>(buf, tw);
    else tile_transform<DIT, false>(buf, tw, k_hi, logT, LD);
}

__device__ __forceinline__ void stage_twiddles(uint32_t* dst, const uint32_t* __restrict__ compact, int logn) {
    const int count = (1 << logn) - 1;
    for (int i = threadIdx.x; i < count; i += blockDim.x) dst[i] = compact[i];
}

__device__ __forceinline__ Fp root_pow(const DeviceTables& tb, int m, uint32_t x) { return domain_point(tb, m ? __brev(x) >> (32 - m) : 0u); }
__device__ __forceinline__ Fp inv_root_pow(const DeviceTables& tb, int m, uint32_t x) { return inv_domain_point(tb, m ? __brev(x) >> (32 - m) : 0u); }

__host__ __device__ inline int padded_words(int n) { return n + (n >> 4); }

constexpr int CONTIG_MAX_PER_THREAD = 16;
__device__ __forceinline__ void prefetch_tile(uint32_t (&pre)[CONTIG_MAX_PER_THREAD], const uint32_t* __restrict__ src, int n_lo) {
#pragma unroll
    for (int u = 0; u < CONTIG_MAX_PER_THREAD; u++) {
        const int i = threadIdx.x + u * blockDim.x;
        if (i < n_lo) pre[u] = src[i];
    }
}
__device__ __forceinline__ void commit_tile(const uint32_t (&pre)[CONTIG_MAX_PER_THREAD], uint32_t* lds, int n_lo) {
#pragma unroll
    for (int u = 0; u < CONTIG_MAX_PER_THREAD; u++) {
        const int i = threadIdx.x + u * blockDim.x;
        if (i < n_lo) lds[tile_addr<true>(i, 0, 0)] = pre[u];
    }
}

__global__ void k_intt_contig(DMatView m, int k, int k_lo, DeviceTables tb, uint32_t n_inv_mont) {
    extern __shared__ uint32_t lds[];
    const int n_lo = 1 << k_lo, k_hi = k - k_lo;
    const uint32_t* tw = tb.itwc;
    const uint64_t tiles_per_col = m.height >> k_lo, total = tiles_per_col * m.width;
    auto tile_ptr = [&](uint64_t t) { const uint64_t cidx = t >> k_hi; return m.col(cidx) + (t & (tiles_per_col - 1)) * n_lo; };
    uint32_t pre[CONTIG_MAX_PER_THREAD];
    if (blockIdx.x < total) prefetch_tile(pre, tile_ptr(blockIdx.x), n_lo);
    for (uint64_t t = blockIdx.x; t < total; t += gridDim.x) {
        const uint64_t h = t & (tiles_per_col - 1);
        uint32_t* col = tile_ptr(t);
        commit_tile(pre, lds, n_lo);
        __syncthreads();
        if (t + gridDim.x < total) prefetch_tile(pre, tile_ptr(t + gridDim.x), n_lo);
        tile_transform<true, true>(lds, tw, k_lo, 0, 0);
        if (k_hi > 0) {
            const uint32_t e = __brev((uint32_t)h) >> (32 - k_hi), nmask = (1u << k) - 1u;
            Fp step = inv_root_pow(tb, k, (e * blockDim.x) & nmask), cur = inv_root_pow(tb, k, (e * threadIdx.x) & nmask);
            for (int i = threadIdx.x; i < n_lo; i += blockDim.x) { col[i] = (Fp::raw(lds[tile_addr<true>(i, 0, 0)]) * cur).v; cur *= step; }
        } else {
            Fp ninv = Fp::raw(n_inv_mont);
            for (int i = threadIdx.x; i < n_lo; i += blockDim.x) col[i] = (Fp::raw(lds[tile_addr<true>(i, 0, 0)]) * ninv).v;
        }
        __syncthreads();
    }
}

__device__ __forceinline__ unsigned strided_tile_of_block(unsigned x, unsigned n_tiles) {
    if (n_tiles & 15u) return x;
    return (x & ~15u) | ((x & 7u) << 1) | ((x >> 3) & 1u);
}

__global__ void k_intt_strided(DMatView m, int k, int k_lo, int logT, DeviceTables tb, uint32_t n_inv_mont) {
    extern __shared__ uint32_t lds[];
    const int k_hi = k - k_lo, n_hi = 1 << k_hi, T = 1 << logT, LD = T + 1;
    const uint64_t n_lo = 1ull << k_lo;
    uint32_t* tw = lds + n_hi * LD;
    uint32_t* col = m.col(blockIdx.y) + (uint64_t)strided_tile_of_block(blockIdx.x, gridDim.x) * T;
    const int total = n_hi << logT;
    {
        int e = threadIdx.x;
        for (; e + 7 * (int)blockDim.x < total; e += 8 * blockDim.x) {
            uint32_t v[8];
#pragma unroll
            for (int u = 0; u < 8; u++) { const int eu = e + u * (int)blockDim.x; v[u] = col[(uint64_t)(eu >> logT) * n_lo + (eu & (T - 1))]; }
#pragma unroll
            for (int u = 0; u < 8; u++) { const int eu = e + u * (int)blockDim.x; lds[(eu >> logT) * LD + (eu & (T - 1))] = v[u]; }
        }
        for (; e < total; e += blockDim.x) { int c = e & (T - 1), h = e >> logT; lds[h * LD + c] = col[h * n_lo + c]; }
    }
    stage_twiddles(tw, tb.itwc, k_hi);
    __syncthreads();
    strided_tile_transform<true>(lds, tw, k_hi, logT, LD);
    Fp ninv = Fp::raw(n_inv_mont);
    for (int e = threadIdx.x; e < total; e += blockDim.x) { int c = e & (T - 1), h = e >> logT; col[h * n_lo + c] = (Fp::raw(lds[h * LD + c]) * ninv).v; }
}

struct CosetPowers { uint32_t lo[64], hi[256], hp[128], step; };

__global__ void k_ntt_strided(DMatView src, DMatView dst, uint64_t dst_row0, int k, int k_lo, int logT, DeviceTables tb, CosetPowers cp) {
    extern __shared__ uint32_t lds[];
    const int k_hi = k - k_lo, n_hi = 1 << k_hi, T = 1 << logT, LD = T + 1;
    const uint64_t n_lo = 1ull << k_lo, r0 = (uint64_t)strided_tile_of_block(blockIdx.x, gridDim.x) * T;
    uint32_t* tw = lds + n_hi * LD;
    const uint32_t* in = src.col(blockIdx.y) + r0;
    uint32_t* out = dst.col(blockIdx.y) + dst_row0 + r0;
    const int total = n_hi << logT;
    {
        int c = threadIdx.x & (T - 1), h0 = threadIdx.x >> logT, hstep = blockDim.x >> logT;
        const uint32_t r = (uint32_t)r0 + c;
        Fp cur = Fp::raw(cp.lo[r & 63]) * Fp::raw(cp.hi[r >> 6]) * Fp::raw(cp.hp[h0]), step = Fp::raw(cp.step);
        int h = h0;
        for (; h + 7 * hstep < n_hi; h += 8 * hstep) {
            uint32_t v[8];
#pragma unroll
            for (int u = 0; u < 8; u++) v[u] = in[(uint64_t)(h + u * hstep) * n_lo + c];
#pragma unroll
            for (int u = 0; u < 8; u++) { lds[(h + u * hstep) * LD + c] = (Fp::raw(v[u]) * cur).v; cur *= step; }
        }
        for (; h < n_hi; h += hstep) { lds[h * LD + c] = (Fp::raw(in[h * n_lo + c]) * cur).v; cur *= step; }
    }
    stage_twiddles(tw, tb.twc, k_hi);
    __syncthreads();
    strided_tile_transform<false>(lds, tw, k_hi, logT, LD);
    for (int h = threadIdx.x; h < n_hi; h += blockDim.x) {
        const uint32_t e = __brev((uint32_t)h) >> (32 - k_hi);
        Fp base = root_pow(tb, k, e);
        Fp cur = root_pow(tb, k, (uint32_t)(((uint64_t)e * r0) & ((1ull << k) - 1)));
        for (int c = 0; c < T; c++) { lds[h * LD + c] = (Fp::raw(lds[h * LD + c]) * cur).v; cur *= base; }
    }
    __syncthreads();
    for (int e = threadIdx.x; e < total; e += blockDim.x) { int c = e & (T - 1), h = e >> logT; out[h * n_lo + c] = lds[h * LD + c]; }
}

__global__ void k_ntt_contig(DMatView src, DMatView dst, uint64_t dst_row0, int k, int k_lo, DeviceTables tb, uint32_t shift_mont,
                             int from_src
                             ) {
    extern __shared__ uint32_t lds[];
    const int n_lo = 1 << k_lo;
    const uint32_t* tw = tb.twc;
    const uint64_t tiles_per_col = src.height >> k_lo, total = tiles_per_col * src.width;
    auto tile_ptr = [&](uint64_t t) { const uint64_t cidx = t >> (k - k_lo); return dst.col(cidx) + dst_row0 + (t & (tiles_per_col - 1)) * n_lo; };
    Fp cur0 = Fp::one(), step = Fp::one();
    if (from_src) { Fp shift = Fp::raw(shift_mont); cur0 = shift.pow(threadIdx.x); step = shift.pow(blockDim.x); }
    uint32_t pre[CONTIG_MAX_PER_THREAD];
    if (!from_src && blockIdx.x < total) prefetch_tile(pre, tile_ptr(blockIdx.x), n_lo);
    for (uint64_t t = blockIdx.x; t < total; t += gridDim.x) {
        uint32_t* out = tile_ptr(t);
        if (from_src) {
            const uint32_t* in = src.col(t);
            Fp cur = cur0;
            for (int i = threadIdx.x; i < n_lo; i += blockDim.x) { lds[tile_addr<true>(i, 0, 0)] = (Fp::raw(in[i]) * cur).v; cur *= step; }
        } else {
            commit_tile(pre, lds, n_lo);
        }
        __syncthreads();
        if (!from_src && t + gridDim.x < total) prefetch_tile(pre, tile_ptr(t + gridDim.x), n_lo);
        tile_transform<false, true>(lds, tw, k_lo, 0, 0);
        for (int i = threadIdx.x; i < n_lo; i += blockDim.x) out[i] = lds[tile_addr<true>(i, 0, 0)];
        __syncthreads();
    }
}


#ifndef VGPU_STRIDED_IO
#define VGPU_STRIDED_IO 1
#endif
#if defined(__HIP_DEVICE_COMPILE__)
#define VGPU_OPAQUE_S(x) asm volatile("" : "+s"(x))
#else
#define VGPU_OPAQUE_S(x) ((void)0)
#endif
__host__ __device__ constexpr uint32_t brev_c(uint32_t x, int bits) { uint32_t r = 0; for (int i = 0; i < bits; i++) r |= ((x >> i) & 1u) << (bits - 1 - i); return r; }
template <int K_HI, int LOGT> struct StridedShape {
    static constexpr int NT = 512, T = 1 << LOGT, LD = T + 1, NH = 1 << K_HI, LH = 9 - LOGT , HSTEP = 1 << LH, U = NH >> LH;
    static_assert(U == 32 && (K_HI - LH) == 5, "512 threads x 32 elements");
};
template <int K_HI, int LOGT, bool SRC_BITREV>
__device__ __forceinline__ void strided_tile_load(const uint32_t* col0, uint32_t n_lo, uint32_t* lds) {
    using S = StridedShape<K_HI, LOGT>;
    const uint32_t tid = threadIdx.x, c = tid & (S::T - 1), h0 = tid >> LOGT;
    const uint32_t blk0 = SRC_BITREV ? (__brev(h0) >> (32 - S::LH)) << 5 : h0;
    const uint32_t voff = (blk0 * n_lo + c) * 4u;
    uint32_t* l0 = lds + h0 * S::LD + c;
    const uint32_t step = (uint32_t)S::HSTEP * n_lo * 4u;
    uint32_t run = 0;
#pragma unroll
    for (int u0 = 0; u0 < S::U; u0 += 8) {
        uint32_t v[8];
#pragma unroll
        for (int k = 0; k < 8; k++) {
            const uint32_t u = (uint32_t)(u0 + k);
            if (SRC_BITREV) v[k] = load_at(col0, voff, brev_c(u, 5) * n_lo * 4u);
            else { v[k] = load_at(col0, voff, run); run += step; VGPU_OPAQUE_S(run); }
        }
#pragma unroll
        for (int k = 0; k < 8; k++) l0[(u0 + k) * S::HSTEP * S::LD] = v[k];
    }
}
template <int K_HI, int LOGT>
__device__ __forceinline__ void strided_tile_store(uint32_t* col0, uint32_t n_lo, const uint32_t* lds) {
    using S = StridedShape<K_HI, LOGT>;
    const uint32_t tid = threadIdx.x, c = tid & (S::T - 1), h0 = tid >> LOGT;
    const uint32_t voff = (h0 * n_lo + c) * 4u;
    const uint32_t* l0 = lds + h0 * S::LD + c;
    const uint32_t step = (uint32_t)S::HSTEP * n_lo * 4u;
    uint32_t run = 0;
#pragma unroll
    for (int u = 0; u < S::U; u++) { store_at(col0, voff, run, l0[u * S::HSTEP * S::LD]); run += step; VGPU_OPAQUE_S(run); }
}
template <int K_HI, int LOGT>
__device__ __forceinline__ void strided_tile_store_transposed(uint32_t* out_col, uint32_t tile, int k_lo, const uint32_t* lds) {
    using S = StridedShape<K_HI, LOGT>;
    const uint32_t tid = threadIdx.x, kq = (uint32_t)(k_lo - LOGT);
    const uint32_t qb_tile = kq ? __brev(tile) >> (32 - kq) : 0u;
    if (K_HI == 8) {
        const uint32_t p2 = tid & 255u, c0 = tid >> 8;
        uint32_t* base = out_col + ((uint64_t)qb_tile << K_HI);
        const uint32_t voff = ((((c0 << 5) << kq) << K_HI) + p2) * 4u;
        const uint32_t* l0 = lds + p2 * S::LD + c0;
#pragma unroll
        for (int i = 0; i < 32; i++) store_at(base, voff, ((brev_c((uint32_t)i, 5) << kq) << K_HI) * 4u, l0[2 * i]);
    } else {
        uint32_t* base = out_col + ((uint64_t)qb_tile << K_HI);
        const uint32_t* l0 = lds + tid * S::LD;
#pragma unroll
        for (int i = 0; i < 32; i++) {
            const uint32_t c = (uint32_t)(i >> 1), half = (uint32_t)(i & 1);
            store_at(base, (tid + 512u * half) * 4u, ((brev_c(c, LOGT) << kq) << K_HI) * 4u, l0[512 * half * S::LD + c]);
        }
    }
}

template <int FK_HI, int FLOGT>
__global__ void __launch_bounds__(FK_HI ? 512 : 1024) k_lde_a(DMatView src, DMatView dst, int k, int k_lo, int logT_arg, DeviceTables tb) {
    extern __shared__ uint32_t lds[];
    const int k_hi = FK_HI ? FK_HI : k - k_lo, logT = FK_HI ? FLOGT : logT_arg, n_hi = 1 << k_hi, T = 1 << logT, LD = T + 1;
    const uint64_t n_lo = 1ull << k_lo, r0 = (uint64_t)strided_tile_of_block(blockIdx.x, gridDim.x) * T;
    uint32_t* tw = lds + n_hi * LD;
    const uint32_t* in = src.col(blockIdx.y) + r0;
    uint32_t* out = dst.col(blockIdx.y) + r0;
    const int total = n_hi << logT;
    if constexpr (FK_HI != 0) strided_tile_load<FK_HI, FLOGT, false>(in, (uint32_t)n_lo, lds);
    else {
        int e = threadIdx.x;
        for (; e + 7 * (int)blockDim.x < total; e += 8 * blockDim.x) {
            uint32_t v[8];
#pragma unroll
            for (int u = 0; u < 8; u++) { const int eu = e + u * (int)blockDim.x; v[u] = in[(uint64_t)(eu >> logT) * n_lo + (eu & (T - 1))]; }
#pragma unroll
            for (int u = 0; u < 8; u++) { const int eu = e + u * (int)blockDim.x; lds[(eu >> logT) * LD + (eu & (T - 1))] = v[u]; }
        }
        for (; e < total; e += blockDim.x) { int c = e & (T - 1), h = e >> logT; lds[h * LD + c] = in[(uint64_t)h * n_lo + c]; }
    }
    stage_twiddles(tw, tb.itwc, k_hi);
    __syncthreads();
    if constexpr (FK_HI != 0) strided_transform<false, FK_HI, FLOGT>(lds, tw);
    else tile_transform<false, false>(lds, tw, k_hi, logT, LD);
    for (int p = threadIdx.x; p < n_hi; p += blockDim.x) {
        const uint32_t ca = __brev((uint32_t)p) >> (32 - k_hi);
        const Fp base = inv_root_pow(tb, k, ca);
        Fp cur = inv_root_pow(tb, k, (uint32_t)(((uint64_t)ca * r0) & ((1ull << k) - 1)));
        for (int c = 0; c < T; c++) { lds[p * LD + c] = (Fp::raw(lds[p * LD + c]) * cur).v; cur *= base; }
    }
    __syncthreads();
    if constexpr (FK_HI != 0) strided_tile_store<FK_HI, FLOGT>(out, (uint32_t)n_lo, lds);
    else
        for (int e = threadIdx.x; e < total; e += blockDim.x) { int c = e & (T - 1), h = e >> logT; out[(uint64_t)h * n_lo + c] = lds[h * LD + c]; }
}

template <int MAXT>
__global__ void __launch_bounds__(MAXT) k_lde_mid(DMatView src, DMatView dst, int k, int k_lo, int lb, DeviceTables tb, LdeTables lt) {
    extern __shared__ uint32_t lds[];
    const int n_lo = 1 << k_lo, k_hi = k - k_lo, n_hi = 1 << k_hi, b = 1 << lb;
    uint32_t* A = lds;
    uint32_t* W = lds + padded_words(n_lo);
    const uint64_t N = 1ull << k, tiles_per_col = (uint64_t)n_hi, total = tiles_per_col * src.width;
    const uint32_t nmask = (uint32_t)(N - 1);
    auto tile_ptr = [&](uint64_t t) { const uint64_t cidx = t >> k_hi; return src.col(cidx) + (t & (tiles_per_col - 1)) * n_lo; };
    uint32_t pre[CONTIG_MAX_PER_THREAD];
    if (blockIdx.x < total) prefetch_tile(pre, tile_ptr(blockIdx.x), n_lo);
    for (uint64_t t = blockIdx.x; t < total; t += gridDim.x) {
        const uint64_t cidx = t >> k_hi, p = t & (tiles_per_col - 1);
        commit_tile(pre, A, n_lo);
        __syncthreads();
        if (t + gridDim.x < total) prefetch_tile(pre, tile_ptr(t + gridDim.x), n_lo);
        tile_transform<false, true>(A, tb.itwc, k_lo, 0, 0);
        const uint32_t ca = k_hi ? __brev((uint32_t)p) >> (32 - k_hi) : 0u;
        for (int tc = 0; tc < b; tc++) {
            const uint32_t* fac = lt.fac + (size_t)tc * n_lo;
            for (int i = threadIdx.x; i < n_lo; i += blockDim.x) W[tile_addr<true>(i, 0, 0)] = (Fp::raw(A[tile_addr<true>(i, 0, 0)]) * Fp::raw(fac[i])).v;
            __syncthreads();
            tile_transform<true, true>(W, tb.twc, k_lo, 0, 0);
            if (k_hi > 0) {
                uint32_t* out = dst.col(cidx) + (uint64_t)tc * N + p * n_lo;
                const Fp step = root_pow(tb, k, (ca * blockDim.x) & nmask);
                Fp cur = Fp::raw(lt.sig[(size_t)tc * n_hi + ca]) * root_pow(tb, k, (ca * threadIdx.x) & nmask);
                for (int q = threadIdx.x; q < n_lo; q += blockDim.x) { out[q] = (Fp::raw(W[tile_addr<true>(q, 0, 0)]) * cur).v; cur *= step; }
            } else {
                const uint32_t blk = lb ? __brev((uint32_t)tc) >> (32 - lb) : 0u;
                uint32_t* out = dst.col(cidx) + (uint64_t)blk * N;
                for (int j = threadIdx.x; j < n_lo; j += blockDim.x) {
                    const int q = k ? (int)(__brev((uint32_t)j) >> (32 - k)) : 0;
                    out[j] = W[tile_addr<true>(q, 0, 0)];
                }
            }
            __syncthreads();
        }
    }
}

__global__ void __launch_bounds__(256) k_lde_mid12(DMatView src, DMatView dst, int k, int lb, DeviceTables tb, LdeTables lt) {
    extern __shared__ uint32_t lds[];
    constexpr int K_LO = 12, N_LO = 1 << K_LO;
    const int k_hi = k - K_LO, n_hi = 1 << k_hi, b = 1 << lb, tid = threadIdx.x;
    const uint64_t N = 1ull << k, tiles_per_col = (uint64_t)n_hi, total = tiles_per_col * src.width;
    const uint32_t nmask = (uint32_t)(N - 1);
    auto tile_ptr = [&](uint64_t t) { const uint64_t cidx = t >> k_hi; return src.col(cidx) + (t & (tiles_per_col - 1)) * N_LO; };
    Fp tw_in[15], tw_out[15];
    load_round_twiddles<4>(tw_in, tb.itwc, tid, 8);
    load_round_twiddles<4>(tw_out, tb.twc, tid, 8);
    const Fp* const held_in = tw_in;
    const Fp* const held_out = tw_out;
    uint32_t pre[16];
    if (blockIdx.x < total) {
        const uint32_t* sp = tile_ptr(blockIdx.x);
#pragma unroll
        for (int g = 0; g < 16; g++) pre[g] = sp[tid + 256 * g];
    }
    for (uint64_t t = blockIdx.x; t < total; t += gridDim.x) {
        const uint64_t cidx = t >> k_hi, p = t & (tiles_per_col - 1);
        Fp x[16];
#pragma unroll
        for (int g = 0; g < 16; g++) x[g] = Fp::raw(pre[g]);
        if (t + gridDim.x < total) {
            const uint32_t* sp = tile_ptr(t + gridDim.x);
#pragma unroll
            for (int g = 0; g < 16; g++) pre[g] = sp[tid + 256 * g];
        }
        butterflies<4, false, false>(x, tb.itwc, tid, 8, held_in);
        {
            uint32_t* p0 = lds + tile_addr<true>(tid, 0, 0);
#pragma unroll
            for (int g = 0; g < 16; g++) p0[g * 272] = x[g].v;
        }
        __syncthreads();
        ntt_round<4, false, true, 4>(lds, tb.itwc, 12, 5, 0, 0);
        {
            const uint32_t* p0 = lds + 17 * tid;
#pragma unroll
            for (int g = 0; g < 16; g++) x[g] = Fp::raw(p0[g]);
        }
        butterflies<4, false, true>(x, tb.itwc, 0, 0);
        const uint32_t ca = __brev((uint32_t)p) >> (32 - k_hi);
        const Fp step = root_pow(tb, k, (ca * 256u) & nmask), tw0 = root_pow(tb, k, (ca * (uint32_t)tid) & nmask);
        for (int tc = 0; tc < b; tc++) {
            Fp y[16];
            {
                const uint32_t* fac = lt.fac + (size_t)tc * N_LO + 16 * tid;
#pragma unroll
                for (int g = 0; g < 16; g++) y[g] = x[g] * Fp::raw(fac[g]);
            }
            butterflies<4, true, true>(y, tb.twc, 0, 0);
            {
                uint32_t* p0 = lds + 17 * tid;
#pragma unroll
                for (int g = 0; g < 16; g++) p0[g] = y[g].v;
            }
            __syncthreads();
            ntt_round<4, true, true, 4>(lds, tb.twc, 12, 5, 0, 0);
            {
                const uint32_t* p0 = lds + tile_addr<true>(tid, 0, 0);
#pragma unroll
                for (int g = 0; g < 16; g++) y[g] = Fp::raw(p0[g * 272]);
            }
            butterflies<4, true, false>(y, tb.twc, tid, 8, held_out);
            uint32_t* out = dst.col(cidx) + (uint64_t)tc * N + p * N_LO + tid;
            Fp cur = Fp::raw(lt.sig[(size_t)tc * n_hi + ca]) * tw0;
#pragma unroll
            for (int g = 0; g < 16; g++) { out[256 * g] = (y[g] * cur).v; cur *= step; }
            __syncthreads();
        }
    }
}

__global__ void __launch_bounds__(1024) k_lde_mid14(DMatView src, DMatView dst, int k, int lb, DeviceTables tb, LdeTables lt) {
    extern __shared__ uint32_t lds[];
    constexpr int K_LO = 14, N_LO = 1 << K_LO, NT = 1024;
    uint32_t* const coef = lds + (N_LO + (N_LO >> 4));
    const int k_hi = k - K_LO, n_hi = 1 << k_hi, b = 1 << lb, tid = threadIdx.x;
    const uint64_t N = 1ull << k, tiles_per_col = (uint64_t)n_hi, total = tiles_per_col * src.width;
    const uint32_t nmask = (uint32_t)(N - 1);
    for (uint64_t t = blockIdx.x; t < total; t += gridDim.x) {
        const uint64_t cidx = t >> k_hi, p = t & (tiles_per_col - 1);
        const uint32_t* sp = src.col(cidx) + p * N_LO;
#pragma unroll
        for (int j = 0; j < 4; j++) {
            const int w = tid + NT * j;
            Fp x4[4];
#pragma unroll
            for (int g = 0; g < 4; g++) x4[g] = Fp::raw(sp[w + 4096 * g]);
            butterflies<2, false, false>(x4, tb.itwc, w, 12);
#pragma unroll
            for (int g = 0; g < 4; g++) lds[tile_addr<true>(w + 4096 * g, 0, 0)] = x4[g].v;
        }
        __syncthreads();
        ntt_round<4, false, true, 8>(lds, tb.itwc, 14, 9, 0, 0);
        ntt_round<4, false, true, 4>(lds, tb.itwc, 14, 5, 0, 0);
        {
            Fp x[16];
            const uint32_t* p0 = lds + 17 * tid;
#pragma unroll
            for (int g = 0; g < 16; g++) x[g] = Fp::raw(p0[g]);
            butterflies<4, false, true>(x, tb.itwc, 0, 0);
            uint32_t* c0 = coef + 17 * tid;
#pragma unroll
            for (int g = 0; g < 16; g++) c0[g] = x[g].v;
        }
        const uint32_t ca = k_hi ? __brev((uint32_t)p) >> (32 - k_hi) : 0u;
        const Fp step = root_pow(tb, k, (ca * 4096u) & nmask);
        for (int tc = 0; tc < b; tc++) {
            Fp y[16];
            {
                const uint32_t* fac = lt.fac + (size_t)tc * N_LO + 16 * tid;
                const uint32_t* c0 = coef + 17 * tid;
#pragma unroll
                for (int g = 0; g < 16; g++) y[g] = Fp::raw(c0[g]) * Fp::raw(fac[g]);
            }
            butterflies<4, true, true>(y, tb.twc, 0, 0);
            {
                uint32_t* p0 = lds + 17 * tid;
#pragma unroll
                for (int g = 0; g < 16; g++) p0[g] = y[g].v;
            }
            __syncthreads();
            ntt_round<4, true, true, 4>(lds, tb.twc, 14, 5, 0, 0);
            ntt_round<4, true, true, 8>(lds, tb.twc, 14, 9, 0, 0);
            uint32_t* out = dst.col(cidx) + (uint64_t)tc * N + p * N_LO;
            const Fp sg = Fp::raw(lt.sig[(size_t)tc * n_hi + ca]);
#pragma unroll 1
            for (int j = 0; j < 4; j++) {
                const int w = tid + NT * j;
                Fp y4[4];
#pragma unroll
                for (int g = 0; g < 4; g++) y4[g] = Fp::raw(lds[tile_addr<true>(w + 4096 * g, 0, 0)]);
                butterflies<2, true, false>(y4, tb.twc, w, 12);
                Fp cur = sg * root_pow(tb, k, (ca * (uint32_t)w) & nmask);
#pragma unroll
                for (int g = 0; g < 4; g++) { out[w + 4096 * g] = (y4[g] * cur).v; cur *= step; }
            }
            __syncthreads();
        }
    }
}

template <int FK_HI, int FLOGT>
__global__ void __launch_bounds__(FK_HI ? 512 : 1024) k_lde_c(DMatView src, DMatView dst, int k, int k_lo, int lb, int logT_arg, DeviceTables tb
                        ) {
    extern __shared__ uint32_t lds[];
    const int k_hi = FK_HI ? FK_HI : k - k_lo, logT = FK_HI ? FLOGT : logT_arg, n_hi = 1 << k_hi, T = 1 << logT, LD = T + 1;
    const uint64_t n_lo = 1ull << k_lo, N = 1ull << k, q0 = (uint64_t)strided_tile_of_block(blockIdx.x, gridDim.x) * T;
    const uint32_t tc = blockIdx.z, blk = lb ? __brev(tc) >> (32 - lb) : 0u;
    uint32_t* tw = lds + n_hi * LD;
    const uint32_t* in = src.col(blockIdx.y) + (uint64_t)tc * N + q0;
    uint32_t* out = dst.col(blockIdx.y) + (uint64_t)blk * N;
    const int total = n_hi << logT;
    if constexpr (FK_HI != 0) strided_tile_load<FK_HI, FLOGT, true>(in, (uint32_t)n_lo, lds);
    else {
        int e = threadIdx.x;
        for (; e + 7 * (int)blockDim.x < total; e += 8 * blockDim.x) {
            uint32_t v[8];
#pragma unroll
            for (int u = 0; u < 8; u++) {
                const int eu = e + u * (int)blockDim.x;
                const uint32_t h = (uint32_t)(eu >> logT), pb = __brev(h) >> (32 - k_hi);
                v[u] = in[(uint64_t)pb * n_lo + (eu & (T - 1))];
            }
#pragma unroll
            for (int u = 0; u < 8; u++) { const int eu = e + u * (int)blockDim.x; lds[(eu >> logT) * LD + (eu & (T - 1))] = v[u]; }
        }
        for (; e < total; e += blockDim.x) {
            const int c = e & (T - 1);
            const uint32_t h = (uint32_t)(e >> logT), pb = __brev(h) >> (32 - k_hi);
            lds[h * LD + c] = in[(uint64_t)pb * n_lo + c];
        }
    }
    stage_twiddles(tw, tb.twc, k_hi);
    __syncthreads();
    if constexpr (FK_HI != 0) strided_transform<false, FK_HI, FLOGT>(lds, tw);
    else tile_transform<false, false>(lds, tw, k_hi, logT, LD);
    const uint32_t tile = strided_tile_of_block(blockIdx.x, gridDim.x);
    if constexpr (FK_HI != 0) strided_tile_store_transposed<FK_HI, FLOGT>(out, tile, k_lo, lds);
    else
    for (int e = threadIdx.x; e < total; e += blockDim.x) {
        const int p2 = e & (n_hi - 1), c = e >> k_hi;
        const uint32_t qb = __brev((uint32_t)(q0 + c)) >> (32 - k_lo);
        out[(uint64_t)qb * n_hi + p2] = lds[p2 * LD + c];
    }
}

struct NttPlan { int k, k_lo, k_hi, logT; unsigned threads_contig, threads_strided; size_t lds_contig, lds_strided; };
static NttPlan make_plan(int k) {
    NttPlan p;
    p.k = k; p.k_lo = k < 12 ? k : (k >= 23 ? 14 : 12); p.k_hi = k - p.k_lo;
    int t = 16384 >> p.k_hi; if (t > 64) t = 64; if (t < 8) t = 8;
    if ((1 << p.k_lo) < t) t = 1 << p.k_lo;
    p.logT = 0; while ((1 << p.logT) < t) p.logT++;
    unsigned n_lo = 1u << p.k_lo;
    p.threads_contig = n_lo / 16 < 64 ? 64 : (n_lo / 16 > 1024 ? 1024 : n_lo / 16);
    unsigned tile = (1u << p.k_hi) << p.logT;
    p.threads_strided = tile / 32 < 64 ? 64 : (tile / 32 > 1024 ? 1024 : tile / 32);
    if (p.threads_strided < (1u << p.logT)) p.threads_strided = 1u << p.logT;
    p.lds_contig = (size_t)padded_words((int)n_lo) * 4;
    p.lds_strided = ((size_t)(1u << p.k_hi) * ((1u << p.logT) + 1) + (1u << p.k_hi)) * 4;
    return p;
}

static void set_lds_limit() {
    static bool done = false;
    if (done) return;
    const int lim = 160 * 1024;
    (void)hipFuncSetAttribute((const void*)k_intt_strided, hipFuncAttributeMaxDynamicSharedMemorySize, lim);
    (void)hipFuncSetAttribute((const void*)k_ntt_strided, hipFuncAttributeMaxDynamicSharedMemorySize, lim);
    (void)hipFuncSetAttribute((const void*)k_intt_contig, hipFuncAttributeMaxDynamicSharedMemorySize, lim);
    (void)hipFuncSetAttribute((const void*)k_ntt_contig, hipFuncAttributeMaxDynamicSharedMemorySize, lim);
    (void)hipFuncSetAttribute((const void*)k_lde_a<0, 0>, hipFuncAttributeMaxDynamicSharedMemorySize, lim);
    (void)hipFuncSetAttribute((const void*)k_lde_a<8, 6>, hipFuncAttributeMaxDynamicSharedMemorySize, lim);
    (void)hipFuncSetAttribute((const void*)k_lde_a<10, 4>, hipFuncAttributeMaxDynamicSharedMemorySize, lim);
    (void)hipFuncSetAttribute((const void*)k_lde_mid<256>, hipFuncAttributeMaxDynamicSharedMemorySize, lim);
    (void)hipFuncSetAttribute((const void*)k_lde_mid<1024>, hipFuncAttributeMaxDynamicSharedMemorySize, lim);
    (void)hipFuncSetAttribute((const void*)k_lde_c<0, 0>, hipFuncAttributeMaxDynamicSharedMemorySize, lim);
    (void)hipFuncSetAttribute((const void*)k_lde_c<8, 6>, hipFuncAttributeMaxDynamicSharedMemorySize, lim);
    (void)hipFuncSetAttribute((const void*)k_lde_c<10, 4>, hipFuncAttributeMaxDynamicSharedMemorySize, lim);
    (void)hipFuncSetAttribute((const void*)k_lde_mid12, hipFuncAttributeMaxDynamicSharedMemorySize, lim);
    (void)hipFuncSetAttribute((const void*)k_lde_mid14, hipFuncAttributeMaxDynamicSharedMemorySize, lim);
    done = true;
}

void launch_intt(hipStream_t st, DMatView m, const DeviceTables& tb) {
    set_lds_limit();
    int k = (int)vg::log2_strict_u64(m.height);
    NttPlan p = make_plan(k);
    uint32_t ninv = Fp::from_canonical((uint32_t)(m.height % vg::P)).inv().v;
    const uint64_t tiles_c = (m.height >> p.k_lo) * m.width;
    dim3 gc((unsigned)(tiles_c < 4096 ? tiles_c : 4096));
    const double pass_bytes = 8.0 * m.height * m.width;
    {
        ProfScope ps("k_intt_contig", st, pass_bytes);
        VK_LAUNCH(k_intt_contig, gc, dim3(p.threads_contig), p.lds_contig, st, m, k, p.k_lo, tb, ninv);
    }
    if (p.k_hi > 0) {
        dim3 gs((unsigned)((1u << p.k_lo) >> p.logT), (unsigned)m.width);
        ProfScope ps("k_intt_strided", st, pass_bytes);
        VK_LAUNCH(k_intt_strided, gs, dim3(p.threads_strided), p.lds_strided, st, m, k, p.k_lo, p.logT, tb, ninv);
    }
}

void launch_coset_ntt(hipStream_t st, DMatView coeffs, DMatView dst, uint64_t dst_row0, Fp shift, const DeviceTables& tb) {
    set_lds_limit();
    int k = (int)vg::log2_strict_u64(coeffs.height);
    NttPlan p = make_plan(k);
    const uint64_t tiles_c = (coeffs.height >> p.k_lo) * coeffs.width;
    dim3 gc((unsigned)(tiles_c < 4096 ? tiles_c : 4096));
    const double pass_bytes = 8.0 * coeffs.height * coeffs.width;
    if (p.k_hi > 0) {
        dim3 gs((unsigned)((1u << p.k_lo) >> p.logT), (unsigned)coeffs.width);
        {
            CosetPowers cp;
            const unsigned hstep = p.threads_strided >> p.logT;
            Fp a = Fp::one(), s64 = shift.pow(64), sn = shift.pow(1ull << p.k_lo);
            for (int i = 0; i < 64; i++) { cp.lo[i] = a.v; a *= shift; }
            a = Fp::one();
            for (int i = 0; i < 256; i++) { cp.hi[i] = a.v; a *= s64; }
            a = Fp::one();
            cp.step = 0;
            for (unsigned i = 0; i < 128; i++) { cp.hp[i] = a.v; a *= sn; if (i + 1 == hstep) cp.step = a.v; }
            ProfScope ps("k_ntt_strided", st, pass_bytes);
            VK_LAUNCH(k_ntt_strided, gs, dim3(p.threads_strided), p.lds_strided, st, coeffs, dst, dst_row0, k, p.k_lo, p.logT, tb, cp);
        }
        ProfScope ps("k_ntt_contig", st, pass_bytes);
        VK_LAUNCH(k_ntt_contig, gc, dim3(p.threads_contig), p.lds_contig, st, coeffs, dst, dst_row0, k, p.k_lo, tb, shift.v, 0);
    } else {
        ProfScope ps("k_ntt_contig", st, pass_bytes);
        VK_LAUNCH(k_ntt_contig, gc, dim3(p.threads_contig), p.lds_contig, st, coeffs, dst, dst_row0, k, p.k_lo, tb, shift.v, 1);
    }
}

void launch_lde_natural(hipStream_t st, DMatView nat, DMatView lde, int log_blowup, const DeviceTables& tb, const LdeTables& lt, DMatView s1, DMatView s2) {
    set_lds_limit();
    const int k = (int)vg::log2_strict_u64(nat.height);
    NttPlan p = make_plan(k);
    const uint64_t tiles = ((uint64_t)1 << p.k_hi) * nat.width;
    dim3 gm((unsigned)(tiles < 4096 ? tiles : 4096));
    const size_t lds_mid = 2 * (size_t)padded_words(1 << p.k_lo) * 4;
    const double nw = 4.0 * nat.height * nat.width, b = (double)(1u << log_blowup);
    if (p.k_hi == 0) {
        ProfScope ps("k_lde_mid", st, nw * (1.0 + b));
        VK_LAUNCH(k_lde_mid<256>, gm, dim3(p.threads_contig), lds_mid, st, nat, lde, k, p.k_lo, log_blowup, tb, lt);
        return;
    }
    dim3 gs((unsigned)((1u << p.k_lo) >> p.logT), (unsigned)nat.width);
    {
        ProfScope ps("k_lde_a", st, 2.0 * nw);
        const int shape = VGPU_STRIDED_IO && VGPU_STRIDED_FIXED && p.threads_strided == 512 ? (p.k_hi == 8 && p.logT == 6 ? 8 : (p.k_hi == 10 && p.logT == 4 ? 10 : 0)) : 0;
        if (shape == 8) VK_LAUNCH((k_lde_a<8, 6>), gs, dim3(512), p.lds_strided, st, nat, s1, k, p.k_lo, p.logT, tb);
        else if (shape == 10) VK_LAUNCH((k_lde_a<10, 4>), gs, dim3(512), p.lds_strided, st, nat, s1, k, p.k_lo, p.logT, tb);
        else VK_LAUNCH((k_lde_a<0, 0>), gs, dim3(p.threads_strided), p.lds_strided, st, nat, s1, k, p.k_lo, p.logT, tb);
    }
    if (p.k_lo == 12) {
        if (gm.x > 4096u) gm.x = 4096u;
        ProfScope ps("k_lde_mid12", st, nw * (1.0 + b));
        VK_LAUNCH(k_lde_mid12, gm, dim3(256), (size_t)padded_words(4096) * 4, st, s1, s2, k, log_blowup, tb, lt);
    } else if (p.k_lo == 14) {
        ProfScope ps("k_lde_mid14", st, nw * (1.0 + b));
        VK_LAUNCH(k_lde_mid14, gm, dim3(1024), 2 * (size_t)padded_words(16384) * 4, st, s1, s2, k, log_blowup, tb, lt);
    } else {
        ProfScope ps("k_lde_mid", st, nw * (1.0 + b));
        if (p.threads_contig <= 256) VK_LAUNCH(k_lde_mid<256>, gm, dim3(p.threads_contig), lds_mid, st, s1, s2, k, p.k_lo, log_blowup, tb, lt);
        else VK_LAUNCH(k_lde_mid<1024>, gm, dim3(p.threads_contig), lds_mid, st, s1, s2, k, p.k_lo, log_blowup, tb, lt);
    }
    dim3 gc((unsigned)((1u << p.k_lo) >> p.logT), (unsigned)nat.width, 1u << log_blowup);
    ProfScope ps("k_lde_c", st, 2.0 * nw * b);
    const int shape_c = VGPU_STRIDED_IO && VGPU_STRIDED_FIXED && p.threads_strided == 512 ? (p.k_hi == 8 && p.logT == 6 ? 8 : (p.k_hi == 10 && p.logT == 4 ? 10 : 0)) : 0;
#define VG_LDE_C(A, B, THREADS) VK_LAUNCH((k_lde_c<A, B>), gc, dim3(THREADS), p.lds_strided, st, s2, lde, k, p.k_lo, log_blowup, p.logT, tb)
    if (shape_c == 8) VG_LDE_C(8, 6, 512);
    else if (shape_c == 10) VG_LDE_C(10, 4, 512);
    else VG_LDE_C(0, 0, p.threads_strided);
#undef VG_LDE_C
}

}
```

valida_amd/csrc/kernels/open.hip:

```cpp
#include <cstdlib>
#include <stdexcept>
#include <type_traits>
#include <vector>
#include <string>
#include "launch.hpp"
#include "poseidon_perm.hpp"
#include "challenger_dev.hpp"

namespace vk {

constexpr int BARY_ROWS = 4;
__device__ __forceinline__ void bary_weights_block(uint64_t block, uint64_t n, const uint32_t* __restrict__ mg, uint32_t shift, const DeviceTables& tb, uint32_t* __restrict__ w,
                                                   uint32_t* __restrict__ img) {
    const uint64_t j0 = (block * blockDim.x + threadIdx.x) * BARY_ROWS;
    if (j0 >= n) return;
    const uint32_t* g = mg + 5;
    Fp r[BARY_ROWS], mx[BARY_ROWS], pre[BARY_ROWS];
    Ext5 gx[BARY_ROWS];
    Fp run = Fp::one();
#pragma unroll
    for (int q = 0; q < BARY_ROWS; q++) {
        const bool live = j0 + q < n;
        r[q] = live ? domain_point(tb, (uint32_t)(j0 + q)) : Fp::one();
        const Fp x = Fp::raw(shift) * r[q], x2 = x * x, x3 = x2 * x, x4 = x2 * x2, x5 = x4 * x;
        const uint64_t tm = (uint64_t)mg[1] * x.v + (uint64_t)mg[2] * x2.v + (uint64_t)mg[3] * x3.v + (uint64_t)mg[4] * x4.v;
        mx[q] = Fp::raw(vg::monty_reduce_wide(tm)) + Fp::raw(mg[0]) + x5;
#pragma unroll
        for (int k = 0; k < 5; k++) {
            const uint64_t tg = (uint64_t)g[5 + k] * x.v + (uint64_t)g[10 + k] * x2.v + (uint64_t)g[15 + k] * x3.v;
            gx[q].c[k] = Fp::raw(vg::monty_reduce_wide(tg)) + Fp::raw(g[k]);
        }
        gx[q].c[0] += x4;
        pre[q] = run;
        run = run * mx[q];
    }
    Fp inv = run.inv();
    Ext5 res[BARY_ROWS];
#pragma unroll
    for (int q = BARY_ROWS - 1; q >= 0; q--) {
        const Fp minv = inv * pre[q];
        inv = inv * mx[q];
        res[q] = gx[q] * (-(minv * r[q]));
    }
    if (img) {
        const uint64_t slab = j0 >> 6, gg = (j0 >> 4) & 3, qq = (j0 >> 2) & 3;
#pragma unroll
        for (int k = 0; k < 5; k++)
#pragma unroll
            for (int a = 0; a < 5; a++) {
                uint32_t word = 0;
#pragma unroll
                for (int q = 0; q < BARY_ROWS; q++) word |= ((res[q].c[k].v >> (7 * a)) & 0x7fu) << (8 * q);
                img[((((slab * 5 + a) * 4 + gg) * 5 + k) << 2) + qq] = word;
            }
    }
    if (j0 + BARY_ROWS <= n) {
#pragma unroll
        for (int k = 0; k < 5; k++) *reinterpret_cast<uint4*>(w + (uint64_t)k * n + j0) = make_uint4(res[0].c[k].v, res[1].c[k].v, res[2].c[k].v, res[3].c[k].v);
    } else {
#pragma unroll
        for (int q = 0; q < BARY_ROWS; q++) if (j0 + q < n) store_ext(w, n, j0 + q, res[q]);
    }
}

__global__ void __launch_bounds__(256) k_bary_weights(uint64_t n, const uint32_t* __restrict__ mg, uint32_t shift, DeviceTables tb, uint32_t* __restrict__ w,
                                                      uint32_t* __restrict__ img) {
    bary_weights_block(blockIdx.x, n, mg, shift, tb, w, img);
}
struct BaryJob { uint32_t first_block, shift; uint64_t n; const uint32_t* mg; uint32_t* w; uint32_t* img; };
__global__ void __launch_bounds__(256) k_bary_weights_batch(const BaryJob* __restrict__ jobs, uint32_t n_jobs, uint32_t shift, DeviceTables tb) {
    uint32_t lo = 0, hi = n_jobs - 1;
    while (lo < hi) { const uint32_t mid = (lo + hi + 1) >> 1; if (jobs[mid].first_block <= blockIdx.x) lo = mid; else hi = mid - 1; }
    const BaryJob j = jobs[lo];
    bary_weights_block(blockIdx.x - j.first_block, j.n, j.mg, j.shift ? j.shift : shift, tb, j.w, j.img);
}

constexpr int DOT_THREADS = 256, DOT_TR = 128, DOT_TRP = DOT_TR + 4, DOT_MAX_PASSES = 4, DOT_MAX_BLOCKS = 1024;

__device__ __forceinline__ Fp wave_sum(Fp v) {
#pragma unroll
    for (int off = 32; off >= 1; off >>= 1) v += Fp::raw((uint32_t)__shfl_xor((int)v.v, off, 64));
    return v;
}

struct Acc96 {
    uint32_t lo, mid, hi;
    __device__ __forceinline__ void add(uint64_t t) {
        const uint64_t s = (uint64_t)lo + (uint32_t)t;
        lo = (uint32_t)s;
        const uint64_t m = (uint64_t)mid + (uint32_t)(t >> 32) + (uint32_t)(s >> 32);
        mid = (uint32_t)m;
        hi += (uint32_t)(m >> 32);
    }
    __device__ __forceinline__ Fp reduce() const {
        uint32_t m = mid;
        if (m >= vg::P) m -= vg::P;
        if (m >= vg::P) m -= vg::P;
        return Fp::raw(vg::monty_reduce((uint64_t)lo)) + Fp::raw(m) + Fp::from_canonical(hi);
    }
};

template <int NP>
__global__ void __launch_bounds__(DOT_THREADS) k_col_dot(DMatView m, uint64_t n, const uint32_t* __restrict__ w0, const uint32_t* __restrict__ w1, uint32_t* __restrict__ partial) {
    extern __shared__ uint32_t lds[];
    constexpr int PK = NP * 5;
    const int C = (int)m.width, n_out = C * PK;
    uint32_t* Mt = lds;
    uint32_t* Wt = lds + C * DOT_TRP;
    Acc96 acc[DOT_MAX_PASSES];
#pragma unroll
    for (int q = 0; q < DOT_MAX_PASSES; q++) acc[q] = Acc96{0, 0, 0};
    const uint64_t n_tiles = (n + DOT_TR - 1) / DOT_TR;
    for (uint64_t t = blockIdx.x; t < n_tiles; t += gridDim.x) {
        const uint64_t row0 = t * DOT_TR;
        const int rows = (int)((n - row0) < (uint64_t)DOT_TR ? (n - row0) : (uint64_t)DOT_TR);
        {
            const int r = threadIdx.x & (DOT_TR - 1);
            const uint32_t* src = m.data + row0 + r;
            uint32_t* dstp = Mt + r;
            const bool live = r < rows;
            int c = threadIdx.x / DOT_TR;
            for (; c + 6 < C; c += 8) {
                uint32_t v[4];
#pragma unroll
                for (int u = 0; u < 4; u++) v[u] = live ? src[(uint64_t)(c + 2 * u) * m.stride] : 0u;
#pragma unroll
                for (int u = 0; u < 4; u++) dstp[(c + 2 * u) * DOT_TRP] = v[u];
            }
            for (; c < C; c += 2) dstp[c * DOT_TRP] = live ? src[(uint64_t)c * m.stride] : 0u;
        }
        {
            const int r = threadIdx.x & (DOT_TR - 1);
            const bool live = r < rows;
            uint32_t v[(PK + 1) / 2];
#pragma unroll
            for (int u = 0; u < (PK + 1) / 2; u++) {
                const int pk = (int)(threadIdx.x / DOT_TR) + 2 * u;
                const uint32_t* w = pk < 5 ? w0 : w1;
                v[u] = (live && pk < PK) ? w[(uint64_t)(pk < 5 ? pk : pk - 5) * n + row0 + r] : 0u;
            }
#pragma unroll
            for (int u = 0; u < (PK + 1) / 2; u++) {
                const int pk = (int)(threadIdx.x / DOT_TR) + 2 * u;
                if (pk < PK) Wt[pk * DOT_TRP + r] = v[u];
            }
        }
        __syncthreads();
#pragma unroll
        for (int q = 0; q < DOT_MAX_PASSES; q++) {
            int idx = q * DOT_THREADS + threadIdx.x;
            if (idx < n_out) {
                int c = idx / PK, pk = idx - c * PK;
                const uint4* mp = reinterpret_cast<const uint4*>(Mt + c * DOT_TRP);
                const uint4* wp = reinterpret_cast<const uint4*>(Wt + pk * DOT_TRP);
                Acc96 a = acc[q];
#pragma unroll 4
                for (int r = 0; r < DOT_TR / 4; r++) {
                    const uint4 mv = mp[r], wv = wp[r];
                    uint64_t t4 = (uint64_t)mv.x * wv.x;
                    t4 += (uint64_t)mv.y * wv.y;
                    t4 += (uint64_t)mv.z * wv.z;
                    t4 += (uint64_t)mv.w * wv.w;
                    a.add(t4);
                }
                acc[q] = a;
            }
        }
        __syncthreads();
    }
#pragma unroll
    for (int q = 0; q < DOT_MAX_PASSES; q++) {
        int idx = q * DOT_THREADS + threadIdx.x;
        if (idx < n_out) partial[(uint64_t)blockIdx.x * n_out + idx] = acc[q].reduce().v;
    }
}

typedef int v4i __attribute__((ext_vector_type(4)));
constexpr uint64_t MFMA_DOT_MIN_ROWS = 1024, MFMA_DOT_MAX_CHUNK = 16384;
__host__ __device__ inline uint64_t mfma_dot_chunk_rows(uint64_t n) {
    uint64_t c = n / 2048;
    return c < 64 ? 64 : (c > MFMA_DOT_MAX_CHUNK ? MFMA_DOT_MAX_CHUNK : c);
}

template <int NP>
__global__ void __launch_bounds__(256) k_col_dot_mfma(DMatView m, uint64_t n, const uint32_t* __restrict__ img0, const uint32_t* __restrict__ img1, uint64_t chunk_rows,
                                                      uint32_t* __restrict__ partial) {
    constexpr int PK = NP * 5;
    const int lane = threadIdx.x & 63, wave = threadIdx.x >> 6, j = lane & 15, g = lane >> 4;
    const uint64_t C = m.width, n_groups = (C + 15) / 16, n_chunks = n / chunk_rows;
    const uint64_t item = (uint64_t)blockIdx.x * 4 + wave;
    if (item >= n_groups * n_chunks) return;
    const uint64_t group = item % n_groups, chunk = item / n_groups;
    const uint64_t c = group * 16 + j;
    const bool col_live = c < C;
    const uint32_t* img = (j < 5 || NP == 1) ? img0 : img1;
    const int limb = j % 5;
    const uint32_t* colp = m.data + (col_live ? c : 0) * m.stride + 16 * g;
    v4i acc[9];
#pragma unroll
    for (int s = 0; s < 9; s++) acc[s] = v4i{0, 0, 0, 0};
    const uint64_t slab0 = chunk * chunk_rows / 64, slab1 = slab0 + chunk_rows / 64;
    v4i A[5], An[5];
    uint4 v[4], vn[4];
    auto fetch = [&](uint64_t slab, v4i (&a5)[5], uint4 (&v4)[4]) {
#pragma unroll
        for (int a = 0; a < 5; a++) a5[a] = *reinterpret_cast<const v4i*>(img + ((((slab * 5 + a) * 4 + g) * 5 + limb) << 2));
        const uint4* src = reinterpret_cast<const uint4*>(colp + slab * 64);
#pragma unroll
        for (int q = 0; q < 4; q++) v4[q] = src[q];
    };
    fetch(slab0, A, v);
    for (uint64_t slab = slab0; slab < slab1; slab++) {
        fetch(slab + 1 < slab1 ? slab + 1 : slab, An, vn);
        v4i B[5];
#pragma unroll
        for (int a = 0; a < 5; a++)
#pragma unroll
            for (int q = 0; q < 4; q++) {
                const uint32_t d0 = __builtin_amdgcn_ubfe(v[q].x, 7 * a, 7), d1 = __builtin_amdgcn_ubfe(v[q].y, 7 * a, 7);
                const uint32_t d2 = __builtin_amdgcn_ubfe(v[q].z, 7 * a, 7), d3 = __builtin_amdgcn_ubfe(v[q].w, 7 * a, 7);
                B[a][q] = (int)(d0 | (d1 << 8) | (d2 << 16) | (d3 << 24));
            }
#pragma unroll
        for (int a = 0; a < 5; a++)
#pragma unroll
            for (int b = 0; b < 5; b++) acc[a + b] = __builtin_amdgcn_mfma_i32_16x16x64_i8(A[a], B[b], acc[a + b], 0, 0, 0);
#pragma unroll
        for (int a = 0; a < 5; a++) A[a] = An[a];
#pragma unroll
        for (int q = 0; q < 4; q++) v[q] = vn[q];
    }
    Fp pw[9];
    pw[0] = Fp::one();
    const Fp step = Fp::from_canonical(128);
#pragma unroll
    for (int s = 1; s < 9; s++) pw[s] = pw[s - 1] * step;
    const uint64_t n_out = C * PK;
#pragma unroll
    for (int r = 0; r < 4; r++) {
        const int pk = 4 * g + r;
        if (pk < PK && col_live) {
            Fp y = Fp::zero();
#pragma unroll
            for (int s = 0; s < 9; s++) y += Fp::from_canonical((uint32_t)acc[s][r]) * pw[s];
            partial[chunk * n_out + c * PK + pk] = vg::monty_reduce((uint64_t)vg::monty_reduce((uint64_t)y.v));
        }
    }
}

__global__ void __launch_bounds__(64) k_col_dot_finish(const uint32_t* __restrict__ partial, uint64_t n_blocks, uint64_t width, int NP, const uint32_t* __restrict__ scale5 ,
                                 uint32_t* __restrict__ out) {
    const uint64_t idx = blockIdx.x;
    const uint64_t c = idx / NP;
    const int p = (int)(idx % NP);
    const uint64_t n_out = width * NP * 5;
    Ext5 acc = Ext5::zero();
    for (uint64_t b = threadIdx.x; b < n_blocks; b += 64) acc += ext_from_words(partial + b * n_out + (c * NP + p) * 5);
#pragma unroll
    for (int k = 0; k < 5; k++) acc.c[k] = wave_sum(acc.c[k]);
    if (threadIdx.x == 0) {
        acc = acc * ext_from_words(scale5 + 5 * p);
        for (int k = 0; k < 5; k++) out[idx * 5 + k] = acc.c[k].canonical();
    }
}

struct DotFinishJob { uint32_t first_block, np; const uint32_t* partial; uint64_t n_blocks, width; const uint32_t* scale5; uint32_t* out; };
__global__ void __launch_bounds__(64) k_col_dot_finish_batch(const DotFinishJob* __restrict__ jobs, uint32_t n_jobs) {
    uint32_t lo = 0, hi = n_jobs - 1;
    while (lo < hi) { const uint32_t mid = (lo + hi + 1) >> 1; if (jobs[mid].first_block <= blockIdx.x) lo = mid; else hi = mid - 1; }
    const DotFinishJob j = jobs[lo];
    const uint64_t idx = blockIdx.x - j.first_block;
    const uint64_t c = idx / j.np;
    const int p = (int)(idx % j.np);
    const uint64_t n_out = j.width * j.np * 5;
    Ext5 acc = Ext5::zero();
    for (uint64_t b = threadIdx.x; b < j.n_blocks; b += 64) acc += ext_from_words(j.partial + b * n_out + (c * j.np + p) * 5);
#pragma unroll
    for (int k = 0; k < 5; k++) acc.c[k] = wave_sum(acc.c[k]);
    if (threadIdx.x == 0) {
        acc = acc * ext_from_words(j.scale5 + 5 * p);
        for (int k = 0; k < 5; k++) j.out[idx * 5 + k] = acc.c[k].canonical();
    }
}

constexpr int MAX_OPEN_POINTS = MAX_OPEN_POINTS_PER_LAUNCH;

__global__ void __launch_bounds__(256) k_reduce_openings(const uint32_t* __restrict__ desc, uint64_t L, uint32_t shift, DeviceTables tb, uint32_t* __restrict__ out, int accumulate) {
    uint64_t j = (uint64_t)blockIdx.x * blockDim.x + threadIdx.x;
    if (j >= L) return;
    const uint32_t n_mats = desc[0], n_points = desc[1], max_w = desc[2];
    const uint32_t* mg = desc + 3;
    const uint32_t* apow = mg + 25 * n_points;
    const uint32_t* md = apow + 5 * max_w;
    Ext5 S[MAX_OPEN_POINTS];
#pragma unroll
    for (int p = 0; p < MAX_OPEN_POINTS; p++) S[p] = Ext5::zero();
    for (uint32_t mi = 0; mi < n_mats; mi++) {
        const uint32_t* colp = reinterpret_cast<const uint32_t*>(((uint64_t)md[1] << 32) | md[0]);
        const uint64_t stride = ((uint64_t)md[3] << 32) | md[2];
        const uint32_t width = md[4], npts = md[5];
        md += 6;
        Ext5 rr = Ext5::zero();
        uint32_t c = 0;
        for (; c + 16 <= width; c += 16) {
            uint32_t v[16];
#pragma unroll
            for (int u = 0; u < 16; u++) v[u] = colp[(uint64_t)(c + u) * stride + j];
#pragma unroll
            for (int g = 0; g < 16; g += 4) {
                const uint32_t* a0 = apow + 5 * (c + g);
#pragma unroll
                for (int k = 0; k < 5; k++) {
                    uint64_t t = (uint64_t)a0[k] * v[g] + (uint64_t)a0[5 + k] * v[g + 1] + (uint64_t)a0[10 + k] * v[g + 2] + (uint64_t)a0[15 + k] * v[g + 3];
                    rr.c[k] += Fp::raw(vg::monty_reduce_wide(t));
                }
            }
        }
        for (; c + 4 <= width; c += 4) {
            const uint32_t v0 = colp[(uint64_t)c * stride + j], v1 = colp[(uint64_t)(c + 1) * stride + j];
            const uint32_t v2 = colp[(uint64_t)(c + 2) * stride + j], v3 = colp[(uint64_t)(c + 3) * stride + j];
            const uint32_t* a0 = apow + 5 * c;
#pragma unroll
            for (int k = 0; k < 5; k++) {
                uint64_t t = (uint64_t)a0[k] * v0 + (uint64_t)a0[5 + k] * v1 + (uint64_t)a0[10 + k] * v2 + (uint64_t)a0[15 + k] * v3;
                rr.c[k] += Fp::raw(vg::monty_reduce_wide(t));
            }
        }
        for (; c < width; c++) rr += ext_from_words(apow + 5 * c) * Fp::raw(colp[(uint64_t)c * stride + j]);
        for (uint32_t q = 0; q < npts; q++, md += 11) {
            Ext5 t = ext_from_words(md + 1) * (ext_from_words(md + 6) - rr);
            const uint32_t slot = md[0];
#pragma unroll
            for (int p = 0; p < MAX_OPEN_POINTS; p++) if ((uint32_t)p == slot) S[p] += t;
        }
    }
    const Fp x = Fp::raw(shift) * domain_point(tb, (uint32_t)j);
    const Fp x2 = x * x, x3 = x2 * x, x4 = x2 * x2, x5 = x4 * x;
    Ext5 gx[MAX_OPEN_POINTS];
    Fp mx[MAX_OPEN_POINTS], pre[MAX_OPEN_POINTS];
    Fp run = Fp::one();
#pragma unroll
    for (int p = 0; p < MAX_OPEN_POINTS; p++)
        if ((uint32_t)p < n_points) {
            const uint32_t* q = mg + 25 * p;
            const uint64_t tm = (uint64_t)q[1] * x.v + (uint64_t)q[2] * x2.v + (uint64_t)q[3] * x3.v + (uint64_t)q[4] * x4.v;
            mx[p] = Fp::raw(vg::monty_reduce_wide(tm)) + Fp::raw(q[0]) + x5;
            const uint32_t* g = q + 5;
#pragma unroll
            for (int k = 0; k < 5; k++) {
                const uint64_t tg = (uint64_t)g[5 + k] * x.v + (uint64_t)g[10 + k] * x2.v + (uint64_t)g[15 + k] * x3.v;
                gx[p].c[k] = Fp::raw(vg::monty_reduce_wide(tg)) + Fp::raw(g[k]);
            }
            gx[p].c[0] += x4;
            pre[p] = run;
            run = run * mx[p];
        }
    Fp inv_run = run.inv();
    Ext5 ro = Ext5::zero();
#pragma unroll
    for (int p = MAX_OPEN_POINTS - 1; p >= 0; p--)
        if ((uint32_t)p < n_points) { ro -= (S[p] * gx[p]) * (inv_run * pre[p]); inv_run = inv_run * mx[p]; }
    const uint64_t half = L >> 1;
    if (accumulate) ro += load_ext(out + (j & 1) * 5 * half, half, j >> 1);
    store_ext(out + (j & 1) * 5 * half, half, j >> 1, ro);
}

template <int R> struct RowVec;
template <> struct RowVec<2> { using T = uint2; static __device__ __forceinline__ void get(const T& v, uint32_t (&e)[2]) { e[0] = v.x; e[1] = v.y; } };
template <> struct RowVec<4> { using T = uint4; static __device__ __forceinline__ void get(const T& v, uint32_t (&e)[4]) { e[0] = v.x; e[1] = v.y; e[2] = v.z; e[3] = v.w; } };
template <int NP, int R>
__global__ void __launch_bounds__(256) k_reduce_openings_rows(const uint32_t* __restrict__ desc, uint64_t L, uint32_t shift, DeviceTables tb, uint32_t* __restrict__ out, int accumulate) {
    using V = typename RowVec<R>::T;
    const uint64_t j0 = ((uint64_t)blockIdx.x * blockDim.x + threadIdx.x) * R;
    if (j0 >= L) return;
    const uint32_t n_mats = desc[0], n_points = desc[1], max_w = desc[2];
    const uint32_t* mg = desc + 3;
    const uint32_t* apow = mg + 25 * n_points;
    const uint32_t* md = apow + 5 * max_w;
    Ext5 S[NP][R];
#pragma unroll
    for (int p = 0; p < NP; p++)
#pragma unroll
        for (int r = 0; r < R; r++) S[p][r] = Ext5::zero();
    for (uint32_t mi = 0; mi < n_mats; mi++) {
        const uint32_t* colp = reinterpret_cast<const uint32_t*>(((uint64_t)md[1] << 32) | md[0]) + j0;
        const uint64_t stride = ((uint64_t)md[3] << 32) | md[2];
        const uint32_t width = md[4], npts = md[5];
        md += 6;
        Ext5 rr[R];
#pragma unroll
        for (int r = 0; r < R; r++) rr[r] = Ext5::zero();
        auto four_cols = [&](const V& v0, const V& v1, const V& v2, const V& v3, const uint32_t* a0) {
            uint32_t e0[R], e1[R], e2[R], e3[R];
            RowVec<R>::get(v0, e0); RowVec<R>::get(v1, e1); RowVec<R>::get(v2, e2); RowVec<R>::get(v3, e3);
#pragma unroll
            for (int r = 0; r < R; r++)
#pragma unroll
                for (int k = 0; k < 5; k++) {
                    const uint64_t t = (uint64_t)a0[k] * e0[r] + (uint64_t)a0[5 + k] * e1[r] + (uint64_t)a0[10 + k] * e2[r] + (uint64_t)a0[15 + k] * e3[r];
                    rr[r].c[k] += Fp::raw(vg::monty_reduce_wide(t));
                }
        };
        uint32_t c = 0;
        for (; c + 8 <= width; c += 8) {
            V v[8];
#pragma unroll
            for (int u = 0; u < 8; u++) v[u] = *reinterpret_cast<const V*>(colp + (uint64_t)(c + u) * stride);
            four_cols(v[0], v[1], v[2], v[3], apow + 5 * c);
            four_cols(v[4], v[5], v[6], v[7], apow + 5 * (c + 4));
        }
        for (; c + 4 <= width; c += 4) {
            V v[4];
#pragma unroll
            for (int u = 0; u < 4; u++) v[u] = *reinterpret_cast<const V*>(colp + (uint64_t)(c + u) * stride);
            four_cols(v[0], v[1], v[2], v[3], apow + 5 * c);
        }
        for (; c < width; c++) {
            uint32_t e[R];
            RowVec<R>::get(*reinterpret_cast<const V*>(colp + (uint64_t)c * stride), e);
            const Ext5 a = ext_from_words(apow + 5 * c);
#pragma unroll
            for (int r = 0; r < R; r++) rr[r] += a * Fp::raw(e[r]);
        }
        for (uint32_t q = 0; q < npts; q++, md += 11) {
            const Ext5 coef = ext_from_words(md + 1), Y = ext_from_words(md + 6);
            const uint32_t slot = md[0];
#pragma unroll
            for (int r = 0; r < R; r++) {
                const Ext5 t = coef * (Y - rr[r]);
#pragma unroll
                for (int p = 0; p < NP; p++) if ((uint32_t)p == slot) S[p][r] += t;
            }
        }
    }
    const Fp x = Fp::raw(shift) * domain_point(tb, (uint32_t)j0), im = domain_point(tb, 2u);
    const Fp x2 = x * x, x3 = x2 * x, x4 = x2 * x2, x5 = x4 * x;
    Fp pw[R][5];
    pw[0][0] = x; pw[0][1] = x2; pw[0][2] = x3; pw[0][3] = x4; pw[0][4] = x5;
    pw[1][0] = -x; pw[1][1] = x2; pw[1][2] = -x3; pw[1][3] = x4; pw[1][4] = -x5;
    if constexpr (R == 4) {
        const Fp ix = im * x, ix3 = im * x3, ix5 = im * x5;
        pw[2][0] = ix; pw[2][1] = -x2; pw[2][2] = -ix3; pw[2][3] = x4; pw[2][4] = ix5;
        pw[3][0] = -ix; pw[3][1] = -x2; pw[3][2] = ix3; pw[3][3] = x4; pw[3][4] = -ix5;
    }
    Fp mx[NP][R], pre[NP][R];
    Fp run = Fp::one();
#pragma unroll
    for (int p = 0; p < NP; p++)
        if ((uint32_t)p < n_points) {
            const uint32_t* q = mg + 25 * p;
#pragma unroll
            for (int r = 0; r < R; r++) {
                const uint64_t tm = (uint64_t)q[1] * pw[r][0].v + (uint64_t)q[2] * pw[r][1].v + (uint64_t)q[3] * pw[r][2].v + (uint64_t)q[4] * pw[r][3].v;
                mx[p][r] = Fp::raw(vg::monty_reduce_wide(tm)) + Fp::raw(q[0]) + pw[r][4];
                pre[p][r] = run;
                run = run * mx[p][r];
            }
        }
    Fp inv_run = run.inv();
    Ext5 ro[R];
#pragma unroll
    for (int r = 0; r < R; r++) ro[r] = Ext5::zero();
    auto point_step = [&](auto pc) {
        constexpr int p = decltype(pc)::value;
        if ((uint32_t)p < n_points) {
            const uint32_t* g = mg + 25 * p + 5;
#pragma unroll
            for (int r = R - 1; r >= 0; r--) {
                Ext5 gx;
#pragma unroll
                for (int k = 0; k < 5; k++) {
                    const uint64_t tg = (uint64_t)g[5 + k] * pw[r][0].v + (uint64_t)g[10 + k] * pw[r][1].v + (uint64_t)g[15 + k] * pw[r][2].v;
                    gx.c[k] = Fp::raw(vg::monty_reduce_wide(tg)) + Fp::raw(g[k]);
                }
                gx.c[0] += pw[r][3];
                ro[r] -= (S[p][r] * gx) * (inv_run * pre[p][r]);
                inv_run = inv_run * mx[p][r];
            }
        }
    };
    if constexpr (NP > 3) point_step(std::integral_constant<int, 3>{});
    if constexpr (NP > 2) point_step(std::integral_constant<int, 2>{});
    if constexpr (NP > 1) point_step(std::integral_constant<int, 1>{});
    point_step(std::integral_constant<int, 0>{});
    const uint64_t half = L >> 1, at = j0 >> 1;
#pragma unroll
    for (int k = 0; k < 5; k++) {
        uint32_t* pe = out + (uint64_t)k * half + at;
        uint32_t* po = out + (uint64_t)(5 + k) * half + at;
        if constexpr (R == 4) {
            Fp e0 = ro[0].c[k], e1 = ro[2].c[k], o0 = ro[1].c[k], o1 = ro[3].c[k];
            if (accumulate) { const uint2 a = *reinterpret_cast<uint2*>(pe), b = *reinterpret_cast<uint2*>(po); e0 += Fp::raw(a.x); e1 += Fp::raw(a.y); o0 += Fp::raw(b.x); o1 += Fp::raw(b.y); }
            *reinterpret_cast<uint2*>(pe) = make_uint2(e0.v, e1.v);
            *reinterpret_cast<uint2*>(po) = make_uint2(o0.v, o1.v);
        } else {
            Fp e0 = ro[0].c[k], o0 = ro[1].c[k];
            if (accumulate) { e0 += Fp::raw(*pe); o0 += Fp::raw(*po); }
            *pe = e0.v;
            *po = o0.v;
        }
    }
}

__global__ void __launch_bounds__(256) k_fri_fold(const uint32_t* __restrict__ in, uint64_t L, const uint32_t* __restrict__ beta5 ,
                           const uint32_t* __restrict__ add, DeviceTables tb, uint32_t* __restrict__ out) {
    const uint64_t half = L >> 1;
    uint64_t i = (uint64_t)blockIdx.x * blockDim.x + threadIdx.x;
    if (i >= half) return;
    Ext5 f0 = load_ext(in, half, i), f1 = load_ext(in + 5 * half, half, i);
    Ext5 beta = ext_from_words(beta5);
    Fp xinv = inv_domain_point(tb, (uint32_t)(2 * i));
    Ext5 r = (f0 + f1) + beta * ((f0 - f1) * xinv);
#pragma unroll
    for (int k = 0; k < 5; k++) r.c[k] = r.c[k].halve();
    const uint64_t q = half >> 1;
    if (q == 0) {
        if (add) r += load_ext(add, 1, 0);
        store_ext(out, 1, 0, r);
        return;
    }
    uint32_t* o = out + (i & 1) * 5 * q;
    if (add) r += load_ext(add + (i & 1) * 5 * q, q, i >> 1);
    store_ext(o, q, i >> 1, r);
}

__global__ void k_gather(const uint32_t* __restrict__ desc, uint64_t n_desc, uint32_t* __restrict__ dst) {
    uint64_t d = (uint64_t)blockIdx.x * (blockDim.x >> 5) + (threadIdx.x >> 5);
    if (d >= n_desc) return;
    const uint32_t* e = desc + 6 * d;
    const uint32_t* src = reinterpret_cast<const uint32_t*>(((uint64_t)e[1] << 32) | e[0]);
    const uint64_t stride = ((uint64_t)e[3] << 32) | e[2];
    const uint32_t count = e[4] & 0x0fffffffu, kind = e[4] >> 28;
    uint32_t* o = dst + e[5];
    for (uint32_t k = threadIdx.x & 31; k < count; k += 32) {
        uint32_t v = src[(uint64_t)k * stride];
        o[k] = kind == 0 ? Fp::raw(v).canonical() : v;
    }
}

__global__ void k_gather_q(const uint32_t* __restrict__ templ, uint64_t n_desc, const uint32_t* __restrict__ indices, uint32_t* __restrict__ dst) {
    uint64_t d = (uint64_t)blockIdx.x * (blockDim.x >> 5) + (threadIdx.x >> 5);
    if (d >= n_desc) return;
    const uint32_t* e = templ + 8 * d;
    const uint32_t* base = reinterpret_cast<const uint32_t*>(((uint64_t)e[1] << 32) | e[0]);
    const uint64_t stride = ((uint64_t)e[3] << 32) | e[2];
    const uint32_t count = e[4] & 0x0fffffffu, kind = e[4] >> 28;
    const uint32_t q = e[6] & 0xffu, mode = (e[6] >> 8) & 0xffu, shift = e[6] >> 16;
    const uint64_t index = indices[q];
    const uint32_t* src = mode == 0 ? base + (index >> shift) : mode == 1 ? base + 8 * ((index >> shift) ^ 1) : base + (index >> (shift + 1)) + (((index >> shift) & 1) ? 0u : e[7]);
    uint32_t* o = dst + e[5];
    for (uint32_t k = threadIdx.x & 31; k < count; k += 32) {
        uint32_t v = src[(uint64_t)k * stride];
        o[k] = kind == 0 ? Fp::raw(v).canonical() : v;
    }
}
void launch_gather_q(hipStream_t st, const uint32_t* templ_dev, uint64_t n_desc, const uint32_t* indices_dev, uint32_t* dst) {
    if (!n_desc) return;
    ProfScope ps("k_gather", st, 0.0);
    VK_LAUNCH(k_gather_q, dim3((unsigned)((n_desc + 7) / 8)), dim3(256), 0, st, templ_dev, n_desc, indices_dev, dst);
}

__global__ void __launch_bounds__(64) k_fri_challenge(const uint32_t* __restrict__ pos, uint32_t* __restrict__ ch, const uint32_t* __restrict__ digest8,
                                                      uint32_t* __restrict__ beta5, uint32_t* __restrict__ commit8) {
    fri_challenge_step((int)threadIdx.x, pos, ch, digest8, beta5, commit8);
}

void launch_fri_challenge(hipStream_t st, const uint32_t* pos_dev, uint32_t* ch_dev, const uint32_t* digest8_dev, uint32_t* beta5_dev, uint32_t* commit8_dev) {
    ProfScope ps("k_fri_challenge", st, 0.0);
    VK_LAUNCH(k_fri_challenge, dim3(1), dim3(64), 0, st, pos_dev, ch_dev, digest8_dev, beta5_dev, commit8_dev);
}

__global__ void __launch_bounds__(256) k_pow_grind(const uint32_t* __restrict__ pos, int sparse, uint32_t k_pending, uint32_t first, uint32_t count, uint32_t mask,
                                                   uint32_t* __restrict__ best) {
    uint32_t t = blockIdx.x * blockDim.x + threadIdx.x;
    if (t >= count) return;
    const uint32_t* base = pos + 496;
    Fp st[16];
#pragma unroll
    for (int i = 0; i < 16; i++) st[i] = Fp::raw(base[i]);
    const Fp wit = Fp::from_canonical(first + t);
#pragma unroll
    for (int i = 0; i < 16; i++) if ((uint32_t)i == k_pending) st[i] = wit;
    poseidon16_permute(st, tab_of(pos, sparse != 0));
    if ((st[15].canonical() & mask) == 0) atomicMin(best, first + t);
// ... 115 lines not shown
```

Baseline: 62.76 proofs/s.

## Fold opening Y terms into per-point constants and index alpha powers globally

Changes the batched opening reduction so alpha powers are indexed by the global running column offset, not recomputed per matrix. The opened-value terms are folded into one per-point constant K that seeds the accumulator, which drops the per-matrix Y subtraction and coefficient multiply. Matrices with one point, or two points and narrow width, now walk the columns directly with shifted power tables and skip the final Ext5 product. Separately, the Keccak Merkle row hash uses buffer loads and a cheaper additive canonicalisation. The cost is larger alpha-power tables and more column walks for two-point matrices, which also touches the sharded prover and the Y-reconstruction descriptors.

```diff
diff --git a/valida_amd/csrc/field.hpp b/valida_amd/csrc/field.hpp
--- a/valida_amd/csrc/field.hpp
+++ b/valida_amd/csrc/field.hpp
@@ -102,6 +102,7 @@
     VG_HD static Fp one() { return raw(R_MOD_P); }
     VG_HD static Fp from_canonical(uint32_t x) { return raw(monty_reduce((uint64_t)x * R2_MOD_P)); }
     VG_HD uint32_t canonical() const { return monty_reduce((uint64_t)v); }
+    VG_HD uint32_t canonical_additive() const { return mul_hi_u32(v * P_INV_NEG, P) + (v != 0 ? 1u : 0u); }
     VG_HD bool is_zero() const { return v == 0; }
     VG_HD bool operator==(const Fp& o) const { return v == o.v; }
     VG_HD bool operator!=(const Fp& o) const { return v != o.v; }
diff --git a/valida_amd/csrc/host/prover.cpp b/valida_amd/csrc/host/prover.cpp
--- a/valida_amd/csrc/host/prover.cpp
+++ b/valida_amd/csrc/host/prover.cpp
@@ -643,15 +643,11 @@
     PcsOpening res;
     auto t0 = Clock::now();
     const Ext5 alpha_b = ch.sample_ext();
-    struct MatEntry { const DMat* lde; std::vector<std::tuple<uint32_t, Ext5, Ext5>> pts; size_t r, i; };
-    struct Group { std::vector<Ext5> zs; std::map<PointKey, uint32_t> slot; std::vector<MatEntry> mats; uint64_t num_reduced = 0; Ext5 offset = Ext5::one(); };
+    struct MatEntry { const DMat* lde; std::vector<std::pair<uint32_t, uint64_t>> pts; size_t r, i; };
+    struct Group { std::vector<Ext5> zs; std::map<PointKey, uint32_t> slot; std::vector<MatEntry> mats; uint64_t num_reduced = 0; };
     std::map<unsigned, Group> groups;
     std::vector<Ext5> apow;
     auto prepare_groups = [&]() {
-        size_t max_width = 0;
-        for (auto& r : rounds) for (auto& l : r.pd->ldes) max_width = std::max<size_t>(max_width, l.width);
-        apow.resize(max_width);
-        { Ext5 p = Ext5::one(); for (auto& a : apow) { a = p; p *= alpha_b; } }
         for (size_t r = 0; r < NR; r++)
             for (size_t i = 0; i < rounds[r].pd->ldes.size(); i++) {
                 const DMat& lde = rounds[r].pd->ldes[i];
@@ -664,12 +660,15 @@
                     auto it = g.slot.find(key);
                     uint32_t slot;
                     if (it == g.slot.end()) { slot = (uint32_t)g.zs.size(); g.slot[key] = slot; g.zs.push_back(z); } else slot = it->second;
-                    me.pts.emplace_back(slot, g.offset, Ext5::zero());
+                    me.pts.emplace_back(slot, g.num_reduced);
                     g.num_reduced += lde.width;
-                    if (lde.width) g.offset *= apow[lde.width - 1] * alpha_b;
                 }
                 g.mats.push_back(std::move(me));
             }
+        size_t n_pow = 0;
+        for (auto& kv : groups) n_pow = std::max<size_t>(n_pow, kv.second.num_reduced);
+        apow.resize(n_pow);
+        { Ext5 p = Ext5::one(); for (auto& a : apow) { a = p; p *= alpha_b; } }
     };
 
     res.opened.resize(NR);
@@ -752,7 +751,7 @@
         }
         prepare_groups();
         {
-            struct YSlot { size_t pool_off, r, i, p; };
+            struct YSlot { size_t pool_off; std::vector<std::tuple<size_t, size_t, size_t, uint64_t>> parts; };
             std::vector<YSlot> y_slots;
             std::vector<uint32_t> pool;
             for (auto& kv : groups) {
@@ -760,34 +759,34 @@
                 for (uint32_t s0 = 0; s0 < g.zs.size() || s0 == 0; s0 += vk::MAX_OPEN_POINTS_PER_LAUNCH) {
                     const uint32_t s1 = std::min<uint32_t>((uint32_t)g.zs.size(), s0 + vk::MAX_OPEN_POINTS_PER_LAUNCH);
                     std::vector<const MatEntry*> live;
-                    size_t max_w = 0;
                     uint64_t total_width = 0;
                     bool vec_ok = true;
                     for (auto& me : g.mats) {
                         bool any = false;
-                        for (auto& t : me.pts) any |= std::get<0>(t) >= s0 && std::get<0>(t) < s1;
-                        if (any) { live.push_back(&me); max_w = std::max<size_t>(max_w, me.lde->width); total_width += me.lde->width; vec_ok &= vk::reduce_vec_ok(me.lde->data, me.lde->height); }
+                        for (auto& t : me.pts) any |= t.first >= s0 && t.first < s1;
+                        if (any) { live.push_back(&me); total_width += me.lde->width; vec_ok &= vk::reduce_vec_ok(me.lde->data, me.lde->height); }
                     }
                     launches.push_back({kv.first, pool.size(), s0 != 0, total_width, (int)(s1 - s0), vec_ok});
                     pool.push_back((uint32_t)live.size());
                     pool.push_back(s1 - s0);
-                    pool.push_back((uint32_t)max_w);
+                    pool.push_back((uint32_t)g.num_reduced);
                     for (uint32_t q = s0; q < s1; q++) put_min_poly(pool, g.zs[q]);
-                    for (size_t col = 0; col < max_w; col++) put_ext(pool, apow[col]);
+                    const size_t y0 = y_slots.size();
+                    for (uint32_t q = s0; q < s1; q++) { y_slots.push_back({pool.size(), {}}); put_ext(pool, Ext5::zero()); }
+                    for (size_t col = 0; col < g.num_reduced; col++) put_ext(pool, apow[col]);
                     for (auto* me : live) {
                         put_ptr(pool, me->lde->data);
                         put_u64(pool, me->lde->height);
                         pool.push_back((uint32_t)me->lde->width);
                         uint32_t cnt = 0;
-                        for (auto& t : me->pts) cnt += std::get<0>(t) >= s0 && std::get<0>(t) < s1;
-                        pool.push_back(cnt);
+                        for (auto& t : me->pts) cnt += t.first >= s0 && t.first < s1;
+                        pool.push_back(cnt | (vk::reduce_direct(me->lde->width, cnt) ? vk::REDUCE_DIRECT_FLAG : 0u));
                         for (size_t pi = 0; pi < me->pts.size(); pi++) {
                             auto& t = me->pts[pi];
-                            if (std::get<0>(t) >= s0 && std::get<0>(t) < s1) {
-                                pool.push_back(std::get<0>(t) - s0);
-                                put_ext(pool, std::get<1>(t));
-                                y_slots.push_back({pool.size(), me->r, me->i, pi});
-                                put_ext(pool, Ext5::zero());
+                            if (t.first >= s0 && t.first < s1) {
+                                pool.push_back(t.first - s0);
+                                pool.push_back((uint32_t)t.second);
+                                y_slots[y0 + (t.first - s0)].parts.emplace_back(me->r, me->i, pi, t.second);
                             }
                         }
                     }
@@ -802,12 +801,13 @@
                 ydesc.push_back((uint32_t)ys.pool_off);
                 const size_t n_seg_at = ydesc.size();
                 ydesc.push_back(0);
-                for (auto& j : jobs)
-                    if (j.r == ys.r && j.i == ys.i && (size_t)j.p0 <= ys.p && ys.p < (size_t)(j.p0 + j.np)) {
-                        ydesc.push_back((uint32_t)j.out_off); ydesc.push_back((uint32_t)j.np); ydesc.push_back((uint32_t)(ys.p - (size_t)j.p0));
-                        ydesc.push_back((uint32_t)j.c0); ydesc.push_back((uint32_t)j.cw);
-                        ydesc[n_seg_at]++;
-                    }
+                for (auto& [yr, yi, yp, yoffset] : ys.parts)
+                    for (auto& j : jobs)
+                        if (j.r == yr && j.i == yi && (size_t)j.p0 <= yp && yp < (size_t)(j.p0 + j.np)) {
+                            ydesc.push_back((uint32_t)j.out_off); ydesc.push_back((uint32_t)j.np); ydesc.push_back((uint32_t)(yp - (size_t)j.p0));
+                            ydesc.push_back((uint32_t)(yoffset + j.c0)); ydesc.push_back((uint32_t)j.cw);
+                            ydesc[n_seg_at]++;
+                        }
             }
             ydesc_at = pool.size();
             pool.insert(pool.end(), ydesc.begin(), ydesc.end());
diff --git a/valida_amd/csrc/host/sharded_prover.cpp b/valida_amd/csrc/host/sharded_prover.cpp
--- a/valida_amd/csrc/host/sharded_prover.cpp
+++ b/valida_amd/csrc/host/sharded_prover.cpp
@@ -843,36 +843,32 @@
         Opening& O = op[k];
         O.alpha_b = R.ch->sample_ext();
         const Ext5& alpha_b = O.alpha_b;
-        struct MatEntry { const uint32_t* data; uint64_t stride; uint64_t width; std::vector<std::tuple<uint32_t, Ext5, Ext5>> pts; };
-        struct Group { std::vector<Ext5> zs; std::map<SpPointKey, uint32_t> slot; std::vector<MatEntry> mats; uint64_t num_reduced = 0; Ext5 offset = Ext5::one(); };
+        struct MatEntry { const uint32_t* data; uint64_t stride; uint64_t width; std::vector<std::pair<uint32_t, uint64_t>> pts; size_t r, i; };
+        struct Group { std::vector<Ext5> zs; std::map<SpPointKey, uint32_t> slot; std::vector<MatEntry> mats; uint64_t num_reduced = 0; };
         std::map<unsigned, Group> groups;
-        size_t max_width = 0;
-        for (size_t r = 0; r < NR; r++) for (auto& m : round_of(R, r).mats) max_width = std::max<size_t>(max_width, m.width);
-        std::vector<Ext5> apow(max_width);
-        { Ext5 pw = Ext5::one(); for (auto& a : apow) { a = pw; pw *= alpha_b; } }
         for (size_t r = 0; r < NR; r++) {
             ShRound& rs = round_of(R, r);
             for (size_t i = 0; i < rs.mats.size(); i++) {
                 const ShMat& m = rs.mats[i];
                 const unsigned lh = vg::log2_strict_u64(m.L);
                 Group& g = groups[lh];
-                MatEntry me{m.big ? m.shard.data : m.lde.data, m.big ? m.shard.height : m.lde.height, m.width, {}};
+                MatEntry me{m.big ? m.shard.data : m.lde.data, m.big ? m.shard.height : m.lde.height, m.width, {}, r, i};
                 for (size_t p = 0; p < points[k][r][i].size(); p++) {
                     const Ext5& z = points[k][r][i][p];
                     auto key = sp_key_of(z);
                     auto it = g.slot.find(key);
                     uint32_t slot;
                     if (it == g.slot.end()) { slot = (uint32_t)g.zs.size(); g.slot[key] = slot; g.zs.push_back(z); } else slot = it->second;
-                    Ext5 Y = Ext5::zero();
-                    auto& ys = O.opened[r][i][p];
-                    for (size_t col = 0; col < ys.size(); col++) Y += apow[col] * ys[col];
-                    me.pts.emplace_back(slot, g.offset, Y);
+                    me.pts.emplace_back(slot, g.num_reduced);
                     g.num_reduced += m.width;
-                    if (m.width) g.offset *= apow[m.width - 1] * alpha_b;
                 }
                 g.mats.push_back(std::move(me));
             }
         }
+        size_t n_pow = 0;
+        for (auto& kv : groups) n_pow = std::max<size_t>(n_pow, kv.second.num_reduced);
+        std::vector<Ext5> apow(n_pow);
+        { Ext5 pw = Ext5::one(); for (auto& a : apow) { a = pw; pw *= alpha_b; } }
         struct Launch { unsigned lh; size_t off; bool accumulate; uint64_t total_width; int n_points; bool vec_ok; };
         std::vector<Launch> launches;
         std::vector<uint32_t> pool;
@@ -881,29 +877,36 @@
             for (uint32_t s0 = 0; s0 < g.zs.size() || s0 == 0; s0 += vk::MAX_OPEN_POINTS_PER_LAUNCH) {
                 const uint32_t s1 = std::min<uint32_t>((uint32_t)g.zs.size(), s0 + vk::MAX_OPEN_POINTS_PER_LAUNCH);
                 std::vector<const MatEntry*> live;
-                size_t max_w = 0;
                 uint64_t total_width = 0;
                 bool vec_ok = true;
+                std::vector<Ext5> K(s1 - s0, Ext5::zero());
                 for (auto& me : g.mats) {
                     bool any = false;
-                    for (auto& t : me.pts) any |= std::get<0>(t) >= s0 && std::get<0>(t) < s1;
-                    if (any) { live.push_back(&me); max_w = std::max<size_t>(max_w, me.width); total_width += me.width; vec_ok &= vk::reduce_vec_ok(me.data, me.stride); }
+                    for (size_t pi = 0; pi < me.pts.size(); pi++) {
+                        auto& t = me.pts[pi];
+                        if (t.first < s0 || t.first >= s1) continue;
+                        any = true;
+                        auto& ys = O.opened[me.r][me.i][pi];
+                        for (size_t col = 0; col < ys.size(); col++) K[t.first - s0] += apow[t.second + col] * ys[col];
+                    }
+                    if (any) { live.push_back(&me); total_width += me.width; vec_ok &= vk::reduce_vec_ok(me.data, me.stride); }
                 }
                 launches.push_back({kv.first, pool.size(), s0 != 0, total_width, (int)(s1 - s0), vec_ok});
                 pool.push_back((uint32_t)live.size());
                 pool.push_back(s1 - s0);
-                pool.push_back((uint32_t)max_w);
+                pool.push_back((uint32_t)g.num_reduced);
                 for (uint32_t q = s0; q < s1; q++) put_min_poly(pool, g.zs[q]);
-                for (size_t col = 0; col < max_w; col++) put_ext(pool, apow[col]);
+                for (auto& k5 : K) put_ext(pool, k5);
+                for (size_t col = 0; col < g.num_reduced; col++) put_ext(pool, apow[col]);
                 for (auto* me : live) {
                     put_ptr(pool, me->data);
                     put_u64(pool, me->stride);
                     pool.push_back((uint32_t)me->width);
                     uint32_t cnt = 0;
-                    for (auto& t : me->pts) cnt += std::get<0>(t) >= s0 && std::get<0>(t) < s1;
-                    pool.push_back(cnt);
+                    for (auto& t : me->pts) cnt += t.first >= s0 && t.first < s1;
+                    pool.push_back(cnt | (vk::reduce_direct(me->width, cnt) ? vk::REDUCE_DIRECT_FLAG : 0u));
                     for (auto& t : me->pts)
-                        if (std::get<0>(t) >= s0 && std::get<0>(t) < s1) { pool.push_back(std::get<0>(t) - s0); put_ext(pool, std::get<1>(t)); put_ext(pool, std::get<2>(t)); }
+                        if (t.first >= s0 && t.first < s1) { pool.push_back(t.first - s0); pool.push_back((uint32_t)t.second); }
                 }
                 if (g.zs.size() <= s1) break;
             }
diff --git a/valida_amd/csrc/kernels/launch.hpp b/valida_amd/csrc/kernels/launch.hpp
--- a/valida_amd/csrc/kernels/launch.hpp
+++ b/valida_amd/csrc/kernels/launch.hpp
@@ -118,6 +118,9 @@
 uint32_t col_dot_finish_job(std::vector<uint32_t>& jobs, uint32_t first_block, uint64_t n, uint64_t width, int np, const uint32_t* partial, const uint32_t* scale5_dev, uint32_t* out_dev);
 void launch_col_dot_finish_batch(hipStream_t st, const uint32_t* jobs_dev, uint32_t n_jobs, uint32_t total_blocks);
 constexpr int MAX_OPEN_POINTS_PER_LAUNCH = 4;
+constexpr uint32_t REDUCE_DIRECT_FLAG = 0x100;
+constexpr uint64_t REDUCE_DIRECT_MAX_WIDTH_2PT = 12;
+inline bool reduce_direct(uint64_t width, size_t n_pts) { return n_pts == 1 || (n_pts == 2 && width <= REDUCE_DIRECT_MAX_WIDTH_2PT); }
 void launch_open_y(hipStream_t st, const uint32_t* vals_dev, const uint32_t* apow_dev, const uint32_t* desc_dev, const uint32_t* entry_off_dev, uint32_t n_entries, uint32_t* pool_dev);
 inline bool reduce_vec_ok(const void* col0, uint64_t stride_words) { return ((uintptr_t)col0 & 15) == 0 && (stride_words & 3) == 0; }
 void launch_reduce_openings(hipStream_t st, const uint32_t* desc_dev, uint64_t L, Fp shift, const DeviceTables& tb, uint32_t* out, uint64_t total_width,
diff --git a/valida_amd/csrc/kernels/merkle.hip b/valida_amd/csrc/kernels/merkle.hip
--- a/valida_amd/csrc/kernels/merkle.hip
+++ b/valida_amd/csrc/kernels/merkle.hip
@@ -8,9 +8,9 @@
 namespace vk {
 
 __device__ __forceinline__ uint32_t wrap_mod_p(uint32_t w) {
-    if (w >= vg::P) w -= vg::P;
-    if (w >= vg::P) w -= vg::P;
-    return w;
+    const uint32_t a = w - vg::P, b = w - 2u * vg::P;
+    const uint32_t m = a < w ? a : w;
+    return b < m ? b : m;
 }
 
 __device__ __forceinline__ void squeeze_digest(const KState& a, uint32_t (&out)[8]) {
@@ -27,20 +27,30 @@
     uint64_t stride;
     __device__ __forceinline__ const uint32_t* operator[](int k) const { return base + (uint64_t)k * stride; }
 };
+constexpr uint64_t KECCAK_MAX_ROWS = 1ull << 30;
 template <class Cols>
-__device__ __forceinline__ void hash_row(const Cols cols, int n_elems, uint64_t r, uint32_t (&out)[8]) {
+__device__ __forceinline__ uint32_t load_elem(const Cols& cols, int k, uint32_t r) {
+#ifdef __HIPCC__
+    const __amdgpu_buffer_rsrc_t rsrc = __builtin_amdgcn_make_buffer_rsrc(const_cast<uint32_t*>(cols[k]), 0, 0xFFFFFFFF, 0x00020000);
+    return (uint32_t)__builtin_amdgcn_raw_buffer_load_b32(rsrc, (int)(r << 2), 0, 0);
+#else
+    return cols[k][r];
+#endif
+}
+template <class Cols>
+__device__ __forceinline__ void hash_row(const Cols cols, int n_elems, uint32_t r, uint32_t (&out)[8]) {
     KState a;
     kstate_zero(a);
     int base = 0;
     for (; base + 34 <= n_elems; base += 34) {
 #pragma unroll
-        for (int k = 0; k < 34; k++) absorb_word(a, k, Fp::raw(cols[base + k][r]).canonical());
+        for (int k = 0; k < 34; k++) absorb_word(a, k, Fp::raw(load_elem(cols, base + k, r)).canonical_additive());
         keccak_f1600<false>(a);
     }
     const int rem = n_elems - base;
 #pragma unroll
     for (int k = 0; k < 34; k++) {
-        if (k < rem) absorb_word(a, k, Fp::raw(cols[base + k][r]).canonical());
+        if (k < rem) absorb_word(a, k, Fp::raw(load_elem(cols, base + k, r)).canonical_additive());
         if (k == rem) absorb_word(a, k, 0x01u);
     }
     absorb_word(a, 33, 0x80000000u);
@@ -75,7 +85,7 @@
     uint64_t r = (uint64_t)blockIdx.x * blockDim.x + threadIdx.x;
     if (r >= n_rows) return;
     uint32_t d[8];
-    hash_row(cols, n_elems, r, d);
+    hash_row(cols, n_elems, (uint32_t)r, d);
     store_digest(digests + 8 * r, d);
 }
 
@@ -89,7 +99,7 @@
     compress2(l, r, d);
     if (n_elems > 0) {
         uint32_t h[8], d2[8];
-        hash_row(PtrCols{cols}, n_elems, i, h);
+        hash_row(PtrCols{cols}, n_elems, (uint32_t)i, h);
         compress2(d, h, d2);
         store_digest(next + 8 * i, d2);
     } else {
@@ -105,14 +115,14 @@
     int base = 0;
     for (; base + 34 <= n_elems; base += 34) {
 #pragma unroll
-        for (int l = 0; l < 17; l++) a.s[l] ^= Fp::raw(cols[base + 2 * l + h][r]).canonical();
+        for (int l = 0; l < 17; l++) a.s[l] ^= Fp::raw(cols[base + 2 * l + h][r]).canonical_additive();
         keccak_f1600_pair<false>(a, h);
     }
     const int rem = n_elems - base;
 #pragma unroll
     for (int l = 0; l < 17; l++) {
         const int k = 2 * l + h;
-        if (k < rem) a.s[l] ^= Fp::raw(cols[base + k][r]).canonical();
+        if (k < rem) a.s[l] ^= Fp::raw(cols[base + k][r]).canonical_additive();
         if (k == rem) a.s[l] ^= 0x01u;
     }
     if (h) a.s[16] ^= 0x80000000u;
@@ -255,7 +265,7 @@
             compress2(lft, rgt, d);
             if (a.n_elems[l] > 0) {
                 uint32_t h[8], d2[8];
-                hash_row(PtrCols{a.cols[l]}, a.n_elems[l], i, h);
+                hash_row(PtrCols{a.cols[l]}, a.n_elems[l], (uint32_t)i, h);
                 compress2(d, h, d2);
                 store_digest(a.out[l] + 8 * i, d2);
             } else {
@@ -359,6 +369,7 @@
 }
 
 void launch_keccak_leaves(hipStream_t st, const uint32_t* const* cols_dev, int n_elems, uint64_t n_rows, uint32_t* digests) {
+    if (n_rows > KECCAK_MAX_ROWS) throw std::invalid_argument("keccak leaves: more rows than the kernels' 32-bit row offsets reach");
     unsigned blocks = (unsigned)((n_rows + 255) / 256);
     const bool pairs = keccak_pairs_enabled() && n_rows <= KECCAK_PAIR_MAX_NODES;
     ProfScope ps(pairs ? "k_keccak_leaves_pair" : "k_keccak_leaves", st, (double)n_rows * (4.0 * n_elems + 32.0), (double)n_rows * row_perms(n_elems) * KECCAK_VALU_PER_PERM / 64.0);
@@ -369,6 +380,7 @@
     VK_LAUNCH(k_keccak_leaves<PtrCols>, dim3(blocks), dim3(256), 0, st, PtrCols{cols_dev}, n_elems, n_rows, digests);
 }
 void launch_keccak_leaves_strided(hipStream_t st, const uint32_t* base, uint64_t stride, int n_elems, uint64_t n_rows, uint32_t* digests) {
+    if (n_rows > KECCAK_MAX_ROWS) throw std::invalid_argument("keccak leaves: more rows than the kernels' 32-bit row offsets reach");
     unsigned blocks = (unsigned)((n_rows + 255) / 256);
     const bool pairs = keccak_pairs_enabled() && n_rows <= KECCAK_PAIR_MAX_NODES;
     ProfScope ps(pairs ? "k_keccak_leaves_pair" : "k_keccak_leaves", st, (double)n_rows * (4.0 * n_elems + 32.0), (double)n_rows * row_perms(n_elems) * KECCAK_VALU_PER_PERM / 64.0);
@@ -379,6 +391,7 @@
     VK_LAUNCH(k_keccak_leaves<StridedCols>, dim3(blocks), dim3(256), 0, st, StridedCols{base, stride}, n_elems, n_rows, digests);
 }
 void launch_keccak_compress(hipStream_t st, const uint32_t* prev, const uint32_t* const* cols_dev, int n_elems, uint64_t n_out, uint32_t* next) {
+    if (n_out > KECCAK_MAX_ROWS) throw std::invalid_argument("keccak compress: more nodes than the kernels' 32-bit row offsets reach");
     unsigned blocks = (unsigned)((n_out + 255) / 256);
     const bool pairs = keccak_pairs_enabled() && n_out <= KECCAK_PAIR_MAX_NODES;
     ProfScope ps(pairs ? "k_keccak_compress_pair" : "k_keccak_compress", st, (double)n_out * (96.0 + 4.0 * n_elems), (double)n_out * node_perms(n_elems) * KECCAK_VALU_PER_PERM / 64.0);
diff --git a/valida_amd/csrc/kernels/ntt.hip b/valida_amd/csrc/kernels/ntt.hip
--- a/valida_amd/csrc/kernels/ntt.hip
+++ b/valida_amd/csrc/kernels/ntt.hip
@@ -104,11 +104,12 @@
     }
 }
 
-template <int R, bool DIT, int LB, int LOGT>
+template <int NT> __device__ __forceinline__ int block_threads() { return NT ? NT : (int)blockDim.x; }
+template <int R, bool DIT, int LB, int LOGT, int NT>
 __device__ __forceinline__ void ntt_round_strided(uint32_t* buf, const uint32_t* tw, int logn) {
     constexpr int G = 1 << R, T = 1 << LOGT, LD = T + 1, gs = LD << LB;
     const int n_items = (1 << (logn - R)) << LOGT;
-    for (int w = threadIdx.x; w < n_items; w += blockDim.x) {
+    auto item = [&](int w) {
         const int c = w & (T - 1), q = w >> LOGT;
         const int low = q & ((1 << LB) - 1), base = ((q >> LB) << (LB + R)) | low;
         uint32_t* p0 = buf + base * LD + c;
@@ -118,20 +119,26 @@
         butterflies<R, DIT, LB == 0>(x, tw, low, LB);
 #pragma unroll
         for (int g = 0; g < G; g++) p0[g * gs] = x[g].v;
+    };
+    if constexpr (NT != 0) {
+#pragma unroll
+        for (int w = threadIdx.x; w < n_items; w += NT) item(w);
+    } else {
+        for (int w = threadIdx.x; w < n_items; w += blockDim.x) item(w);
     }
     __syncthreads();
 }
-template <bool DIT, int K_HI, int LOGT>
+template <bool DIT, int K_HI, int LOGT, int NT = 0>
 __device__ __forceinline__ void strided_transform(uint32_t* buf, const uint32_t* tw) {
     static_assert(K_HI == 8 || K_HI == 10, "hot shapes only");
     if (DIT) {
-        ntt_round_strided<4, true, 0, LOGT>(buf, tw, K_HI);
-        ntt_round_strided<4, true, 4, LOGT>(buf, tw, K_HI);
-        if (K_HI == 10) ntt_round_strided<2, true, 8, LOGT>(buf, tw, K_HI);
+        ntt_round_strided<4, true, 0, LOGT, NT>(buf, tw, K_HI);
+        ntt_round_strided<4, true, 4, LOGT, NT>(buf, tw, K_HI);
+        if (K_HI == 10) ntt_round_strided<2, true, 8, LOGT, NT>(buf, tw, K_HI);
     } else {
-        if (K_HI == 10) ntt_round_strided<2, false, 8, LOGT>(buf, tw, K_HI);
-        ntt_round_strided<4, false, 4, LOGT>(buf, tw, K_HI);
-        ntt_round_strided<4, false, 0, LOGT>(buf, tw, K_HI);
+        if (K_HI == 10) ntt_round_strided<2, false, 8, LOGT, NT>(buf, tw, K_HI);
+        ntt_round_strided<4, false, 4, LOGT, NT>(buf, tw, K_HI);
+        ntt_round_strided<4, false, 0, LOGT, NT>(buf, tw, K_HI);
     }
 }
 #ifndef VGPU_STRIDED_FIXED
@@ -144,9 +151,15 @@
     else tile_transform<DIT, false>(buf, tw, k_hi, logT, LD);
 }
 
+template <int NT = 0>
 __device__ __forceinline__ void stage_twiddles(uint32_t* dst, const uint32_t* __restrict__ compact, int logn) {
     const int count = (1 << logn) - 1;
-    for (int i = threadIdx.x; i < count; i += blockDim.x) dst[i] = compact[i];
+    if constexpr (NT != 0) {
+#pragma unroll
+        for (int i = threadIdx.x; i < count; i += NT) dst[i] = compact[i];
+    } else {
+        for (int i = threadIdx.x; i < count; i += blockDim.x) dst[i] = compact[i];
+    }
 }
 
 __device__ __forceinline__ Fp root_pow(const DeviceTables& tb, int m, uint32_t x) { return domain_point(tb, m ? __brev(x) >> (32 - m) : 0u); }
@@ -384,11 +397,11 @@
         }
         for (; e < total; e += blockDim.x) { int c = e & (T - 1), h = e >> logT; lds[h * LD + c] = in[(uint64_t)h * n_lo + c]; }
     }
-    stage_twiddles(tw, tb.itwc, k_hi);
+    stage_twiddles<FK_HI ? 512 : 0>(tw, tb.itwc, k_hi);
     __syncthreads();
-    if constexpr (FK_HI != 0) strided_transform<false, FK_HI, FLOGT>(lds, tw);
+    if constexpr (FK_HI != 0) strided_transform<false, FK_HI, FLOGT, 512>(lds, tw);
     else tile_transform<false, false>(lds, tw, k_hi, logT, LD);
-    for (int p = threadIdx.x; p < n_hi; p += blockDim.x) {
+    for (int p = threadIdx.x; p < n_hi; p += block_threads<FK_HI ? 512 : 0>()) {
         const uint32_t ca = __brev((uint32_t)p) >> (32 - k_hi);
         const Fp base = inv_root_pow(tb, k, ca);
         Fp cur = inv_root_pow(tb, k, (uint32_t)(((uint64_t)ca * r0) & ((1ull << k) - 1)));
@@ -616,9 +629,9 @@
             lds[h * LD + c] = in[(uint64_t)pb * n_lo + c];
         }
     }
-    stage_twiddles(tw, tb.twc, k_hi);
+    stage_twiddles<FK_HI ? 512 : 0>(tw, tb.twc, k_hi);
     __syncthreads();
-    if constexpr (FK_HI != 0) strided_transform<false, FK_HI, FLOGT>(lds, tw);
+    if constexpr (FK_HI != 0) strided_transform<false, FK_HI, FLOGT, 512>(lds, tw);
     else tile_transform<false, false>(lds, tw, k_hi, logT, LD);
     const uint32_t tile = strided_tile_of_block(blockIdx.x, gridDim.x);
     if constexpr (FK_HI != 0) strided_tile_store_transposed<FK_HI, FLOGT>(out, tile, k_lo, lds);
diff --git a/valida_amd/csrc/kernels/open.hip b/valida_amd/csrc/kernels/open.hip
--- a/valida_amd/csrc/kernels/open.hip
+++ b/valida_amd/csrc/kernels/open.hip
@@ -175,7 +175,11 @@
     }
 }
 
+#ifdef __HIPCC__
 typedef int v4i __attribute__((ext_vector_type(4)));
+#else
+typedef int v4i __attribute__((vector_size(16)));
+#endif
 constexpr uint64_t MFMA_DOT_MIN_ROWS = 1024, MFMA_DOT_MAX_CHUNK = 16384;
 __host__ __device__ inline uint64_t mfma_dot_chunk_rows(uint64_t n) {
     uint64_t c = n / 2048;
@@ -288,51 +292,62 @@
 __global__ void __launch_bounds__(256) k_reduce_openings(const uint32_t* __restrict__ desc, uint64_t L, uint32_t shift, DeviceTables tb, uint32_t* __restrict__ out, int accumulate) {
     uint64_t j = (uint64_t)blockIdx.x * blockDim.x + threadIdx.x;
     if (j >= L) return;
-    const uint32_t n_mats = desc[0], n_points = desc[1], max_w = desc[2];
+    const uint32_t n_mats = desc[0], n_points = desc[1], n_pow = desc[2];
     const uint32_t* mg = desc + 3;
-    const uint32_t* apow = mg + 25 * n_points;
-    const uint32_t* md = apow + 5 * max_w;
+    const uint32_t* kp = mg + 25 * n_points;
+    const uint32_t* apow = kp + 5 * n_points;
+    const uint32_t* md = apow + 5 * n_pow;
     Ext5 S[MAX_OPEN_POINTS];
 #pragma unroll
-    for (int p = 0; p < MAX_OPEN_POINTS; p++) S[p] = Ext5::zero();
+    for (int p = 0; p < MAX_OPEN_POINTS; p++) S[p] = (uint32_t)p < n_points ? ext_from_words(kp + 5 * p) : Ext5::zero();
     for (uint32_t mi = 0; mi < n_mats; mi++) {
         const uint32_t* colp = reinterpret_cast<const uint32_t*>(((uint64_t)md[1] << 32) | md[0]);
         const uint64_t stride = ((uint64_t)md[3] << 32) | md[2];
-        const uint32_t width = md[4], npts = md[5];
+        const uint32_t width = md[4], npts = md[5] & ~REDUCE_DIRECT_FLAG;
+        const bool direct = (md[5] & REDUCE_DIRECT_FLAG) != 0 && npts == 1;
         md += 6;
-        Ext5 rr = Ext5::zero();
-        uint32_t c = 0;
-        for (; c + 16 <= width; c += 16) {
-            uint32_t v[16];
-#pragma unroll
-            for (int u = 0; u < 16; u++) v[u] = colp[(uint64_t)(c + u) * stride + j];
-#pragma unroll
-            for (int g = 0; g < 16; g += 4) {
-                const uint32_t* a0 = apow + 5 * (c + g);
+        auto weighted_row = [&](const uint32_t* pw) {
+            Ext5 rr = Ext5::zero();
+            uint32_t c = 0;
+            for (; c + 16 <= width; c += 16) {
+                uint32_t v[16];
+#pragma unroll
+                for (int u = 0; u < 16; u++) v[u] = colp[(uint64_t)(c + u) * stride + j];
+#pragma unroll
+                for (int g = 0; g < 16; g += 4) {
+                    const uint32_t* a0 = pw + 5 * (c + g);
+#pragma unroll
+                    for (int k = 0; k < 5; k++) {
+                        uint64_t t = (uint64_t)a0[k] * v[g] + (uint64_t)a0[5 + k] * v[g + 1] + (uint64_t)a0[10 + k] * v[g + 2] + (uint64_t)a0[15 + k] * v[g + 3];
+                        rr.c[k] += Fp::raw(vg::monty_reduce_wide(t));
+                    }
+                }
+            }
+            for (; c + 4 <= width; c += 4) {
+                const uint32_t v0 = colp[(uint64_t)c * stride + j], v1 = colp[(uint64_t)(c + 1) * stride + j];
+                const uint32_t v2 = colp[(uint64_t)(c + 2) * stride + j], v3 = colp[(uint64_t)(c + 3) * stride + j];
+                const uint32_t* a0 = pw + 5 * c;
 #pragma unroll
                 for (int k = 0; k < 5; k++) {
-                    uint64_t t = (uint64_t)a0[k] * v[g] + (uint64_t)a0[5 + k] * v[g + 1] + (uint64_t)a0[10 + k] * v[g + 2] + (uint64_t)a0[15 + k] * v[g + 3];
+                    uint64_t t = (uint64_t)a0[k] * v0 + (uint64_t)a0[5 + k] * v1 + (uint64_t)a0[10 + k] * v2 + (uint64_t)a0[15 + k] * v3;
                     rr.c[k] += Fp::raw(vg::monty_reduce_wide(t));
                 }
             }
-        }
-        for (; c + 4 <= width; c += 4) {
-            const uint32_t v0 = colp[(uint64_t)c * stride + j], v1 = colp[(uint64_t)(c + 1) * stride + j];
-            const uint32_t v2 = colp[(uint64_t)(c + 2) * stride + j], v3 = colp[(uint64_t)(c + 3) * stride + j];
-            const uint32_t* a0 = apow + 5 * c;
-#pragma unroll
-            for (int k = 0; k < 5; k++) {
-                uint64_t t = (uint64_t)a0[k] * v0 + (uint64_t)a0[5 + k] * v1 + (uint64_t)a0[10 + k] * v2 + (uint64_t)a0[15 + k] * v3;
-                rr.c[k] += Fp::raw(vg::monty_reduce_wide(t));
-            }
-        }
-        for (; c < width; c++) rr += ext_from_words(apow + 5 * c) * Fp::raw(colp[(uint64_t)c * stride + j]);
-        for (uint32_t q = 0; q < npts; q++, md += 11) {
-            Ext5 t = ext_from_words(md + 1) * (ext_from_words(md + 6) - rr);
-            const uint32_t slot = md[0];
-#pragma unroll
-            for (int p = 0; p < MAX_OPEN_POINTS; p++) if ((uint32_t)p == slot) S[p] += t;
-        }
+            for (; c < width; c++) rr += ext_from_words(pw + 5 * c) * Fp::raw(colp[(uint64_t)c * stride + j]);
+            return rr;
+        };
+        const uint32_t walks = direct ? npts : 1;
+        for (uint32_t q = 0; q < walks; q++) {
+            const Ext5 rr = weighted_row(direct ? apow + 5 * md[2 * q + 1] : apow);
+            const uint32_t products = direct ? 1 : npts;
+            for (uint32_t u = 0; u < products; u++) {
+                const Ext5 t = direct ? rr : ext_from_words(apow + 5 * md[2 * u + 1]) * rr;
+                const uint32_t slot = md[2 * (q + u)];
+#pragma unroll
+                for (int p = 0; p < MAX_OPEN_POINTS; p++) if ((uint32_t)p == slot) S[p] -= t;
+            }
+        }
+        md += 2 * npts;
     }
     const Fp x = Fp::raw(shift) * domain_point(tb, (uint32_t)j);
     const Fp x2 = x * x, x3 = x2 * x, x4 = x2 * x2, x5 = x4 * x;
@@ -373,24 +388,23 @@
     using V = typename RowVec<R>::T;
     const uint64_t j0 = ((uint64_t)blockIdx.x * blockDim.x + threadIdx.x) * R;
     if (j0 >= L) return;
-    const uint32_t n_mats = desc[0], n_points = desc[1], max_w = desc[2];
+    const uint32_t n_mats = desc[0], n_points = desc[1], n_pow = desc[2];
     const uint32_t* mg = desc + 3;
-    const uint32_t* apow = mg + 25 * n_points;
-    const uint32_t* md = apow + 5 * max_w;
+    const uint32_t* kp = mg + 25 * n_points;
+    const uint32_t* apow = kp + 5 * n_points;
+    const uint32_t* md = apow + 5 * n_pow;
     Ext5 S[NP][R];
 #pragma unroll
     for (int p = 0; p < NP; p++)
 #pragma unroll
-        for (int r = 0; r < R; r++) S[p][r] = Ext5::zero();
+        for (int r = 0; r < R; r++) S[p][r] = (uint32_t)p < n_points ? ext_from_words(kp + 5 * p) : Ext5::zero();
     for (uint32_t mi = 0; mi < n_mats; mi++) {
         const uint32_t* colp = reinterpret_cast<const uint32_t*>(((uint64_t)md[1] << 32) | md[0]) + j0;
         const uint64_t stride = ((uint64_t)md[3] << 32) | md[2];
-        const uint32_t width = md[4], npts = md[5];
+        const uint32_t width = md[4], npts = md[5] & ~REDUCE_DIRECT_FLAG;
+        const bool direct = (md[5] & REDUCE_DIRECT_FLAG) != 0;
         md += 6;
-        Ext5 rr[R];
-#pragma unroll
-        for (int r = 0; r < R; r++) rr[r] = Ext5::zero();
-        auto four_cols = [&](const V& v0, const V& v1, const V& v2, const V& v3, const uint32_t* a0) {
+        auto four_cols = [&](const V& v0, const V& v1, const V& v2, const V& v3, const uint32_t* a0, Ext5 (&acc)[R]) {
             uint32_t e0[R], e1[R], e2[R], e3[R];
             RowVec<R>::get(v0, e0); RowVec<R>::get(v1, e1); RowVec<R>::get(v2, e2); RowVec<R>::get(v3, e3);
 #pragma unroll
@@ -398,38 +412,73 @@
 #pragma unroll
                 for (int k = 0; k < 5; k++) {
                     const uint64_t t = (uint64_t)a0[k] * e0[r] + (uint64_t)a0[5 + k] * e1[r] + (uint64_t)a0[10 + k] * e2[r] + (uint64_t)a0[15 + k] * e3[r];
-                    rr[r].c[k] += Fp::raw(vg::monty_reduce_wide(t));
+                    acc[r].c[k] += Fp::raw(vg::monty_reduce_wide(t));
                 }
         };
-        uint32_t c = 0;
-        for (; c + 8 <= width; c += 8) {
-            V v[8];
-#pragma unroll
-            for (int u = 0; u < 8; u++) v[u] = *reinterpret_cast<const V*>(colp + (uint64_t)(c + u) * stride);
-            four_cols(v[0], v[1], v[2], v[3], apow + 5 * c);
-            four_cols(v[4], v[5], v[6], v[7], apow + 5 * (c + 4));
-        }
-        for (; c + 4 <= width; c += 4) {
-            V v[4];
-#pragma unroll
-            for (int u = 0; u < 4; u++) v[u] = *reinterpret_cast<const V*>(colp + (uint64_t)(c + u) * stride);
-            four_cols(v[0], v[1], v[2], v[3], apow + 5 * c);
-        }
-        for (; c < width; c++) {
-            uint32_t e[R];
-            RowVec<R>::get(*reinterpret_cast<const V*>(colp + (uint64_t)c * stride), e);
-            const Ext5 a = ext_from_words(apow + 5 * c);
-#pragma unroll
-            for (int r = 0; r < R; r++) rr[r] += a * Fp::raw(e[r]);
-        }
-        for (uint32_t q = 0; q < npts; q++, md += 11) {
-            const Ext5 coef = ext_from_words(md + 1), Y = ext_from_words(md + 6);
-            const uint32_t slot = md[0];
-#pragma unroll
-            for (int r = 0; r < R; r++) {
-                const Ext5 t = coef * (Y - rr[r]);
-#pragma unroll
-                for (int p = 0; p < NP; p++) if ((uint32_t)p == slot) S[p][r] += t;
+        auto weighted_rows = [&](auto dc, const uint32_t* const (&pw)[decltype(dc)::value], Ext5 (&acc)[decltype(dc)::value][R]) {
+            constexpr int D = decltype(dc)::value;
+#pragma unroll
+            for (int d = 0; d < D; d++)
+#pragma unroll
+                for (int r = 0; r < R; r++) acc[d][r] = Ext5::zero();
+            uint32_t c = 0;
+            for (; c + 8 <= width; c += 8) {
+                V v[8];
+#pragma unroll
+                for (int u = 0; u < 8; u++) v[u] = *reinterpret_cast<const V*>(colp + (uint64_t)(c + u) * stride);
+#pragma unroll
+                for (int d = 0; d < D; d++) {
+                    four_cols(v[0], v[1], v[2], v[3], pw[d] + 5 * c, acc[d]);
+                    four_cols(v[4], v[5], v[6], v[7], pw[d] + 5 * (c + 4), acc[d]);
+                }
+            }
+            for (; c + 4 <= width; c += 4) {
+                V v[4];
+#pragma unroll
+                for (int u = 0; u < 4; u++) v[u] = *reinterpret_cast<const V*>(colp + (uint64_t)(c + u) * stride);
+#pragma unroll
+                for (int d = 0; d < D; d++) four_cols(v[0], v[1], v[2], v[3], pw[d] + 5 * c, acc[d]);
+            }
+            for (; c < width; c++) {
+                uint32_t e[R];
+                RowVec<R>::get(*reinterpret_cast<const V*>(colp + (uint64_t)c * stride), e);
+#pragma unroll
+                for (int d = 0; d < D; d++) {
+                    const Ext5 a = ext_from_words(pw[d] + 5 * c);
+#pragma unroll
+                    for (int r = 0; r < R; r++) acc[d][r] += a * Fp::raw(e[r]);
+                }
+            }
+        };
+        auto take = [&](uint32_t slot, const Ext5 (&t)[R]) {
+#pragma unroll
+            for (int r = 0; r < R; r++)
+#pragma unroll
+                for (int p = 0; p < NP; p++) if ((uint32_t)p == slot) S[p][r] -= t[r];
+        };
+        if (direct && npts == 1) {
+            const uint32_t* const pw[1] = {apow + 5 * md[1]};
+            Ext5 acc[1][R];
+            weighted_rows(std::integral_constant<int, 1>{}, pw, acc);
+            take(md[0], acc[0]);
+            md += 2;
+        } else if (direct && npts == 2) {
+            const uint32_t* const pw[2] = {apow + 5 * md[1], apow + 5 * md[3]};
+            Ext5 acc[2][R];
+            weighted_rows(std::integral_constant<int, 2>{}, pw, acc);
+            take(md[0], acc[0]);
+            take(md[2], acc[1]);
+            md += 4;
+        } else {
+            const uint32_t* const pw[1] = {apow};
+            Ext5 rr[1][R];
+            weighted_rows(std::integral_constant<int, 1>{}, pw, rr);
+            for (uint32_t q = 0; q < npts; q++, md += 2) {
+                const Ext5 coef = ext_from_words(apow + 5 * md[1]);
+                Ext5 t[R];
+#pragma unroll
+                for (int r = 0; r < R; r++) t[r] = coef * rr[0][r];
+                take(md[0], t);
             }
         }
     }
```

Result: no change. 62.70 proofs/s, median of 4 (-0.1%).
